# choderalab/pymbar

Hardware: AMD Instinct MI355X
Metric: mbar_adaptive_iterations_per_sec (higher is better)
Workload: dtype f64

## Files before the change

include/mbar_hip.h:

```cpp
#ifndef MBAR_HIP_H
#define MBAR_HIP_H

#include <stdint.h>

#ifdef __cplusplus
extern "C" {
#endif

typedef struct mbar_ctx mbar_ctx;

#define MBAR_OK 0
#define MBAR_ERR_ARG (-1)
#define MBAR_ERR_HIP (-2)
#define MBAR_ERR_NODEVICE (-3)
#define MBAR_ERR_STATE (-4)
#define MBAR_ERR_COMM (-5)
#define MBAR_ERR_NUMERIC (-6)

#define MBAR_EVAL_GRAM 1u
#define MBAR_EVAL_USE_OFFSET 2u

#define MBAR_TIMER_LSE 0
#define MBAR_TIMER_GRAM 1
#define MBAR_TIMER_REDUCE 2
// ... 10 lines not shown

int mbar_ctx_create(mbar_ctx** out, int device, int64_t K, int64_t N_local);
void mbar_ctx_destroy(mbar_ctx* ctx);
int mbar_ctx_synchronize(mbar_ctx* ctx);
int mbar_cache_trim(void);
int mbar_host_digest(const void* data, int64_t nbytes, int threads, uint64_t* out2);
int mbar_host_newton_direction(const double* H, const double* g, int m, int threads, double* x);
int mbar_device_synchronize(int device);
int mbar_ctx_set_option(mbar_ctx* ctx, const char* key, int64_t value);

int mbar_ctx_upload_u(mbar_ctx* ctx, const double* u_host, int64_t ld_host, int64_t col0_host,
                      int64_t ncols, int64_t col0_dev);
int mbar_ctx_download_u(mbar_ctx* ctx, double* out, int64_t ld_out);
int mbar_ctx_upload_rows(mbar_ctx* ctx, int64_t row0, int64_t nrows, const double* rows_host, int64_t ld_host);
int mbar_ctx_copy_rows(mbar_ctx* dst, int64_t dst_row0, mbar_ctx* src, int64_t src_row0, int64_t nrows);
int mbar_ctx_row_sub(mbar_ctx* ctx, int64_t row, const double* v_host);
int mbar_ctx_rows_sub(mbar_ctx* ctx, int64_t dst_row0, int64_t src_row0, int64_t nrows, const double* v_host);
int mbar_ctx_rows_rsub(mbar_ctx* ctx, int64_t dst_row0, int64_t src_row0, int64_t nrows);
int mbar_ctx_rows_logshift(mbar_ctx* ctx, int64_t row0, int64_t nrows, double* shift_out);
int mbar_ctx_vec_logshift(mbar_ctx* ctx, const double* A, double* shift_out);
int mbar_ctx_fill_masked_rows(mbar_ctx* ctx, int64_t row0, int64_t nrows, const double* v_host, const int32_t* label_host);
int mbar_ctx_generate_harmonic(mbar_ctx* ctx, uint64_t seed, const double* O_k, const double* K_k,
                               const int64_t* N_k_global, int64_t n_global0);
int mbar_ctx_set_Nk(mbar_ctx* ctx, const double* N_k);

int mbar_ctx_set_sample_weights(mbar_ctx* ctx, const double* c_n);

int mbar_ctx_draw_bootstrap_weights(mbar_ctx* ctx, uint64_t seed, int64_t replicate, const int64_t* cumN, int64_t K_states,
                                    const int64_t* order, int64_t n_global0);
int mbar_ctx_set_bootstrap_layout(mbar_ctx* ctx, const int64_t* cumN, int64_t K_states, const int64_t* order);
int mbar_bootstrap_draws(uint64_t seed, int64_t replicate, const int64_t* cumN, int64_t K_states, const int64_t* order,
                         int64_t* rints_out);

int mbar_ctx_weights_from_vec(mbar_ctx* ctx, double power);

int mbar_comm_unique_id(void* id128);
int mbar_ctx_comm_init(mbar_ctx* ctx, const void* id128, int rank, int nranks);
typedef int (*mbar_allreduce_fn)(double* buf, int64_t count, int op, void* user);
int mbar_ctx_set_host_allreduce(mbar_ctx* ctx, mbar_allreduce_fn fn, void* user, int rank, int nranks);
int mbar_ctx_comm_destroy(mbar_ctx* ctx);

typedef struct mbar_loopback mbar_loopback;
int mbar_loopback_create(mbar_loopback** out, int nranks);
void mbar_loopback_destroy(mbar_loopback* group);
int mbar_ctx_set_loopback(mbar_ctx* ctx, mbar_loopback* group, int rank);

int mbar_eval(mbar_ctx* ctx, const double* f, int nf, unsigned flags, double* psum,
              double* sumlogden, double* gram);
int mbar_ctx_set_objective_offset(mbar_ctx* ctx, const double* f0);
int mbar_lognum(mbar_ctx* ctx, const double* f, double* lognum);
int mbar_logden(mbar_ctx* ctx, const double* f, double* out_n);
int mbar_logw(mbar_ctx* ctx, const double* f, double* out_kn, int64_t ld_out);
int mbar_w(mbar_ctx* ctx, const double* f, double* out_kn, int64_t ld_out);
int mbar_gram_w(mbar_ctx* ctx, const double* f, double* gramW, double* wsum);

int mbar_ctx_create_ext(mbar_ctx** out, mbar_ctx* base, int64_t K_rows);
int mbar_ctx_rows_sub_from(mbar_ctx* dst, int64_t dst_row0, mbar_ctx* src, int64_t src_row0, int64_t nrows, const double* v_host);
int mbar_ctx_rows_rsub_from(mbar_ctx* dst, int64_t dst_row0, mbar_ctx* src, int64_t src_row0, int64_t nrows);
int mbar_ctx_rows_obs_from(mbar_ctx* dst, int64_t dst_row0, mbar_ctx* base, int64_t state_row0, int64_t obs_row0, int64_t nrows,
                           double* shift_out, const double* min_in, double* min_out);
int mbar_lognum_ext(mbar_ctx* ext, mbar_ctx* base, const double* f_base, double* lognum_ext);
int mbar_gram_w_ext(mbar_ctx* ext, mbar_ctx* base, const double* f_base, const double* f_ext, const double* gram_base, double* gramW,
                    double* wsum);

typedef struct mbar_solve_result {
    int64_t iterations;
    int64_t nr_iter;
    int64_t sci_iter;
    int32_t success;
    int32_t gram_sweeps;
    double max_delta;
    double gnorm;
    double wall_ms;
    int32_t warm_starts;
    int32_t builds;
    int32_t light_sweeps;
    int32_t fused_unit;
} mbar_solve_result;

int mbar_solve_adaptive(mbar_ctx* ctx, double* f_inout, double tol, int64_t maxiter,
                        int64_t min_sc_iter, double gamma, int check_convergence,
                        double* history, int64_t history_rows, mbar_solve_result* result);
int mbar_ctx_last_solve_psum(mbar_ctx* ctx, double* psum);
int mbar_solve_sci(mbar_ctx* ctx, double* f_inout, double tol, int64_t maxiter, int check_convergence,
                   mbar_solve_result* result);

int mbar_ctx_timing(mbar_ctx* ctx, int which, double* total_ms, int64_t* launches);
int mbar_ctx_timing_reset(mbar_ctx* ctx);
int mbar_mfma_f64_peak(mbar_ctx* ctx, double* tflops);

typedef struct mbar_kde mbar_kde;
#define MBAR_KDE_GAUSSIAN 0
#define MBAR_KDE_TOPHAT 1
#define MBAR_KDE_EPANECHNIKOV 2
#define MBAR_KDE_EXPONENTIAL 3
#define MBAR_KDE_LINEAR 4
#define MBAR_KDE_COSINE 5
int mbar_kde_create(mbar_kde** out, int device, int kernel, int d, int64_t N, const double* x, double bandwidth);
void mbar_kde_destroy(mbar_kde* kde);
int mbar_kde_set_weights(mbar_kde* kde, int64_t C, const double* v);
int mbar_kde_eval(mbar_kde* kde, int64_t M, const double* q, double* out);
int mbar_kde_log_norm(int kernel, int d, double bandwidth, double* out);

typedef struct mbar_acf mbar_acf;
int mbar_acf_create(mbar_acf** out, int device, int64_t T, const double* a, const double* b, int64_t K, const int64_t* seg,
                    double shift_a, double shift_b);
void mbar_acf_destroy(mbar_acf* acf);
int mbar_acf_suffix_g(mbar_acf* acf, int64_t nskip, int fast, int64_t mintime, int fft, double* g, int64_t* stop, int32_t* status);
int mbar_acf_multiple_g(mbar_acf* acf, int fast, int64_t mintime, double* g, int64_t* stop, int32_t* status, int64_t ct_cap,
                        double* ct);
int mbar_acf_schedule_length(int fast, int64_t tmax, int64_t* out);
int mbar_acf_lag_sums(mbar_acf* acf, int64_t nlags, const int64_t* lags, int64_t norig, const int64_t* origins, int segments,
                      double* xab, double* xba);

#define MBAR_BAR_CHUNK 4096
typedef struct mbar_bar_state {
    double DeltaF, DeltaF_old, DeltaF_initial, UpperB, LowerB, FUpperB, FLowerB, FNew, relative_change, relative_tolerance;
    double req[2];
    double moments[4];
    int64_t method, iterated, maximum_iterations, iteration, phase, status, nreq, nzero, want_moments, moments_pending;
} mbar_bar_state;
typedef struct mbar_bar mbar_bar;
int mbar_bar_create(mbar_bar** out, int device, int64_t P, const int64_t* n_f, const double* w_f, const int64_t* n_r,
                    const double* w_r);
void mbar_bar_destroy(mbar_bar* bar);
int mbar_bar_zero(mbar_bar* bar, const double* deltaf, double* out);
int mbar_bar_solve(mbar_bar* bar, mbar_bar_state* states, int64_t* passes);
int mbar_bar_moments(mbar_bar* bar, double* out);
int mbar_bar_step_host(mbar_bar_state* state, const double* F);

typedef struct mbar_bspline mbar_bspline;
int mbar_bspline_create(mbar_bspline** out, int device, int64_t N, const double* x);
void mbar_bspline_destroy(mbar_bspline* bs);
int mbar_bspline_set_groups(mbar_bspline* bs, int G, const int* g);
int mbar_bspline_set_weights(mbar_bspline* bs, int64_t C, const double* v);
int mbar_bspline_moments(mbar_bspline* bs, int k, int nbasis, const double* t, double* out);
int mbar_bspline_kernel_ms(mbar_bspline* bs, double* ms);

#define MBAR_BATCH_MAX_K 64
#define MBAR_BATCH_CHUNK 256
typedef struct mbar_batch_state {
    double f[MBAR_BATCH_MAX_K];
    double req[2][MBAR_BATCH_MAX_K];
    double lognum[MBAR_BATCH_MAX_K];
    double psum[MBAR_BATCH_MAX_K];
    double Nk[MBAR_BATCH_MAX_K];
    double x[MBAR_BATCH_MAX_K];
    double tol, gamma, max_delta, max_diff, gnorm_sci, gnorm_nr;
    int64_t K, maxiter, min_sc_iter, iterations, nr_iter, sci_iter, choices;
    int64_t phase, status, success, nreq, gram_req, gram_w, newton_bad;
} mbar_batch_state;
typedef struct mbar_batch mbar_batch;
int mbar_batch_create(mbar_batch** out, int device, int64_t P, const int64_t* K, const int64_t* N, const double* const* u);
void mbar_batch_destroy(mbar_batch* b);
int mbar_batch_solve(mbar_batch* b, mbar_batch_state* states, int64_t* passes);
int mbar_batch_gram_w(mbar_batch* b, const double* f, const int32_t* mask, double* gram, double* wsum);
int mbar_batch_step_host(mbar_batch_state* state, const double* lognum, const double* gram);

int mbar_batch_set_replicas(mbar_batch* b, int64_t R, const int64_t* base, const int64_t* Nk);
int mbar_batch_replica_set_weights(mbar_batch* b, int64_t slot, const double* c_n);
int mbar_batch_replicas_draw(mbar_batch* b, int64_t first, int64_t count, const uint64_t* seed, const int64_t* replicate);
int mbar_batch_replicas_solve(mbar_batch* b, mbar_batch_state* states, int64_t* passes);
int mbar_batch_replicas_gram_w(mbar_batch* b, const double* f, const int32_t* mask, double* gram, double* wsum);

#define MBAR_BATCH_MAX_AUG 128
int mbar_batch_set_ext(mbar_batch* b, const int64_t* R, const double* const* e);
// ... 10 lines not shown
```

pymbar_amd/_lib.py:

```python
import ctypes as C
import os

HERE = os.path.dirname(os.path.abspath(__file__))
LIB_PATH = os.environ.get("MBAR_HIP_LIBRARY") or os.path.join(HERE, "csrc", "libmbar_hip.so")

MBAR_OK = 0
EVAL_GRAM = 1
EVAL_USE_OFFSET = 2
TIMER_LSE, TIMER_GRAM, TIMER_REDUCE, TIMER_OTHER, TIMER_FUSED, TIMER_NEWTON, TIMER_COMM = 0, 1, 2, 3, 4, 5, 6


class BackendUnavailable(RuntimeError):
    """libmbar_hip.so is missing / not loadable, or there is no gfx950 device."""


class MbarHipError(RuntimeError):

    def __init__(self, code, message):
        super().__init__(f"libmbar_hip error {code}: {message}")
        self.code = code


class BarState(C.Structure):
    _fields_ = [(n, C.c_double) for n in ("DeltaF", "DeltaF_old", "DeltaF_initial", "UpperB", "LowerB", "FUpperB", "FLowerB", "FNew",
# ... 13 lines not shown
    _fields_ = [(n, C.c_double * MBAR_BATCH_MAX_K) for n in ("f",)] + [("req", (C.c_double * MBAR_BATCH_MAX_K) * 2)] + [
        (n, C.c_double * MBAR_BATCH_MAX_K) for n in ("lognum", "psum", "Nk", "x")] + [
        (n, C.c_double) for n in ("tol", "gamma", "max_delta", "max_diff", "gnorm_sci", "gnorm_nr")] + [
        (n, C.c_int64) for n in ("K", "maxiter", "min_sc_iter", "iterations", "nr_iter", "sci_iter", "choices", "phase", "status",
                                 "success", "nreq", "gram_req", "gram_w", "newton_bad")]


class SolveResult(C.Structure):
    _fields_ = [
        ("iterations", C.c_int64),
        ("nr_iter", C.c_int64),
        ("sci_iter", C.c_int64),
        ("success", C.c_int32),
        ("gram_sweeps", C.c_int32),
        ("max_delta", C.c_double),
        ("gnorm", C.c_double),
        ("wall_ms", C.c_double),
        ("warm_starts", C.c_int32),
        ("builds", C.c_int32),
        ("light_sweeps", C.c_int32),
        ("fused_unit", C.c_int32),
    ]


ALLREDUCE_FN = C.CFUNCTYPE(C.c_int, C.POINTER(C.c_double), C.c_int64, C.c_int, C.c_void_p)

_dp = C.POINTER(C.c_double)
_ip = C.POINTER(C.c_int64)
_ctx = C.c_void_p

SIGNATURES = {
    "mbar_version": (C.c_int, []),
    "mbar_last_error": (C.c_char_p, [_ctx]),
    "mbar_device_count": (C.c_int, [C.POINTER(C.c_int)]),
    "mbar_device_info": (C.c_int, [C.c_int, C.c_char_p, C.c_int, C.POINTER(C.c_int), _ip]),
    "mbar_ctx_create": (C.c_int, [C.POINTER(_ctx), C.c_int, C.c_int64, C.c_int64]),
    "mbar_ctx_destroy": (None, [_ctx]),
    "mbar_ctx_synchronize": (C.c_int, [_ctx]),
    "mbar_device_synchronize": (C.c_int, [C.c_int]),
    "mbar_cache_trim": (C.c_int, []),
    "mbar_host_digest": (C.c_int, [C.c_void_p, C.c_int64, C.c_int, C.POINTER(C.c_uint64)]),
    "mbar_host_newton_direction": (C.c_int, [_dp, _dp, C.c_int, C.c_int, _dp]),
    "mbar_ctx_set_option": (C.c_int, [_ctx, C.c_char_p, C.c_int64]),
    "mbar_ctx_upload_u": (C.c_int, [_ctx, _dp, C.c_int64, C.c_int64, C.c_int64, C.c_int64]),
    "mbar_ctx_download_u": (C.c_int, [_ctx, _dp, C.c_int64]),
    "mbar_ctx_upload_rows": (C.c_int, [_ctx, C.c_int64, C.c_int64, _dp, C.c_int64]),
    "mbar_ctx_copy_rows": (C.c_int, [_ctx, C.c_int64, _ctx, C.c_int64, C.c_int64]),
    "mbar_ctx_row_sub": (C.c_int, [_ctx, C.c_int64, _dp]),
    "mbar_ctx_rows_sub": (C.c_int, [_ctx, C.c_int64, C.c_int64, C.c_int64, _dp]),
    "mbar_ctx_rows_rsub": (C.c_int, [_ctx, C.c_int64, C.c_int64, C.c_int64]),
    "mbar_ctx_rows_logshift": (C.c_int, [_ctx, C.c_int64, C.c_int64, _dp]),
    "mbar_ctx_vec_logshift": (C.c_int, [_ctx, _dp, _dp]),
    "mbar_ctx_fill_masked_rows": (C.c_int, [_ctx, C.c_int64, C.c_int64, _dp, C.POINTER(C.c_int32)]),
    "mbar_ctx_generate_harmonic": (C.c_int, [_ctx, C.c_uint64, _dp, _dp, _ip, C.c_int64]),
    "mbar_ctx_set_Nk": (C.c_int, [_ctx, _dp]),
    "mbar_ctx_set_sample_weights": (C.c_int, [_ctx, _dp]),
    "mbar_ctx_weights_from_vec": (C.c_int, [_ctx, C.c_double]),
    "mbar_ctx_draw_bootstrap_weights": (C.c_int, [_ctx, C.c_uint64, C.c_int64, _ip, C.c_int64, _ip, C.c_int64]),
    "mbar_ctx_set_bootstrap_layout": (C.c_int, [_ctx, _ip, C.c_int64, _ip]),
    "mbar_bootstrap_draws": (C.c_int, [C.c_uint64, C.c_int64, _ip, C.c_int64, _ip, _ip]),
    "mbar_comm_unique_id": (C.c_int, [C.c_void_p]),
    "mbar_ctx_comm_init": (C.c_int, [_ctx, C.c_void_p, C.c_int, C.c_int]),
    "mbar_ctx_set_host_allreduce": (C.c_int, [_ctx, ALLREDUCE_FN, C.c_void_p, C.c_int, C.c_int]),
    "mbar_ctx_comm_destroy": (C.c_int, [_ctx]),
    "mbar_loopback_create": (C.c_int, [C.POINTER(C.c_void_p), C.c_int]),
    "mbar_loopback_destroy": (None, [C.c_void_p]),
    "mbar_ctx_set_loopback": (C.c_int, [_ctx, C.c_void_p, C.c_int]),
    "mbar_eval": (C.c_int, [_ctx, _dp, C.c_int, C.c_uint, _dp, _dp, _dp]),
    "mbar_ctx_set_objective_offset": (C.c_int, [_ctx, _dp]),
    "mbar_lognum": (C.c_int, [_ctx, _dp, _dp]),
    "mbar_logden": (C.c_int, [_ctx, _dp, _dp]),
    "mbar_logw": (C.c_int, [_ctx, _dp, _dp, C.c_int64]),
    "mbar_w": (C.c_int, [_ctx, _dp, _dp, C.c_int64]),
    "mbar_gram_w": (C.c_int, [_ctx, _dp, _dp, _dp]),
    "mbar_ctx_create_ext": (C.c_int, [C.POINTER(_ctx), _ctx, C.c_int64]),
    "mbar_ctx_rows_sub_from": (C.c_int, [_ctx, C.c_int64, _ctx, C.c_int64, C.c_int64, _dp]),
    "mbar_ctx_rows_rsub_from": (C.c_int, [_ctx, C.c_int64, _ctx, C.c_int64, C.c_int64]),
    "mbar_ctx_rows_obs_from": (C.c_int, [_ctx, C.c_int64, _ctx, C.c_int64, C.c_int64, C.c_int64, _dp, _dp, _dp]),
    "mbar_lognum_ext": (C.c_int, [_ctx, _ctx, _dp, _dp]),
    "mbar_gram_w_ext": (C.c_int, [_ctx, _ctx, _dp, _dp, _dp, _dp, _dp]),
    "mbar_solve_adaptive": (C.c_int, [_ctx, _dp, C.c_double, C.c_int64, C.c_int64, C.c_double, C.c_int,
                                      _dp, C.c_int64, C.POINTER(SolveResult)]),
    "mbar_ctx_last_solve_psum": (C.c_int, [_ctx, _dp]),
    "mbar_solve_sci": (C.c_int, [_ctx, _dp, C.c_double, C.c_int64, C.c_int, C.POINTER(SolveResult)]),
    "mbar_ctx_timing": (C.c_int, [_ctx, C.c_int, _dp, _ip]),
    "mbar_ctx_timing_reset": (C.c_int, [_ctx]),
    "mbar_mfma_f64_peak": (C.c_int, [_ctx, _dp]),
    "mbar_kde_create": (C.c_int, [C.POINTER(C.c_void_p), C.c_int, C.c_int, C.c_int, C.c_int64, _dp, C.c_double]),
    "mbar_kde_destroy": (None, [C.c_void_p]),
    "mbar_kde_set_weights": (C.c_int, [C.c_void_p, C.c_int64, _dp]),
    "mbar_kde_eval": (C.c_int, [C.c_void_p, C.c_int64, _dp, _dp]),
    "mbar_kde_log_norm": (C.c_int, [C.c_int, C.c_int, C.c_double, _dp]),
    "mbar_acf_create": (C.c_int, [C.POINTER(C.c_void_p), C.c_int, C.c_int64, _dp, _dp, C.c_int64, _ip, C.c_double, C.c_double]),
    "mbar_acf_destroy": (None, [C.c_void_p]),
    "mbar_acf_suffix_g": (C.c_int, [C.c_void_p, C.c_int64, C.c_int, C.c_int64, C.c_int, _dp, _ip, C.POINTER(C.c_int32)]),
    "mbar_acf_multiple_g": (C.c_int, [C.c_void_p, C.c_int, C.c_int64, _dp, _ip, C.POINTER(C.c_int32), C.c_int64, _dp]),
    "mbar_acf_schedule_length": (C.c_int, [C.c_int, C.c_int64, _ip]),
    "mbar_acf_lag_sums": (C.c_int, [C.c_void_p, C.c_int64, _ip, C.c_int64, _ip, C.c_int, _dp, _dp]),
    "mbar_bar_create": (C.c_int, [C.POINTER(C.c_void_p), C.c_int, C.c_int64, _ip, _dp, _ip, _dp]),
    "mbar_bar_destroy": (None, [C.c_void_p]),
    "mbar_bar_zero": (C.c_int, [C.c_void_p, _dp, _dp]),
    "mbar_bar_solve": (C.c_int, [C.c_void_p, C.POINTER(BarState), _ip]),
    "mbar_bar_moments": (C.c_int, [C.c_void_p, _dp]),
    "mbar_bar_step_host": (C.c_int, [C.POINTER(BarState), _dp]),
    "mbar_bspline_create": (C.c_int, [C.POINTER(C.c_void_p), C.c_int, C.c_int64, _dp]),
    "mbar_bspline_destroy": (None, [C.c_void_p]),
    "mbar_bspline_set_groups": (C.c_int, [C.c_void_p, C.c_int, C.POINTER(C.c_int32)]),
    "mbar_bspline_set_weights": (C.c_int, [C.c_void_p, C.c_int64, _dp]),
    "mbar_bspline_moments": (C.c_int, [C.c_void_p, C.c_int, C.c_int, _dp, _dp]),
    "mbar_bspline_kernel_ms": (C.c_int, [C.c_void_p, _dp]),
    "mbar_batch_create": (C.c_int, [C.POINTER(C.c_void_p), C.c_int, C.c_int64, _ip, _ip, C.POINTER(_dp)]),
    "mbar_batch_destroy": (None, [C.c_void_p]),
    "mbar_batch_solve": (C.c_int, [C.c_void_p, C.POINTER(BatchState), _ip]),
    "mbar_batch_gram_w": (C.c_int, [C.c_void_p, _dp, C.POINTER(C.c_int32), _dp, _dp]),
    "mbar_batch_step_host": (C.c_int, [C.POINTER(BatchState), _dp, _dp]),
    "mbar_batch_set_replicas": (C.c_int, [C.c_void_p, C.c_int64, _ip, _ip]),
    "mbar_batch_replica_set_weights": (C.c_int, [C.c_void_p, C.c_int64, _dp]),
    "mbar_batch_replicas_draw": (C.c_int, [C.c_void_p, C.c_int64, C.c_int64, C.POINTER(C.c_uint64), _ip]),
    "mbar_batch_replicas_solve": (C.c_int, [C.c_void_p, C.POINTER(BatchState), _ip]),
    "mbar_batch_replicas_gram_w": (C.c_int, [C.c_void_p, _dp, C.POINTER(C.c_int32), _dp, _dp]),
    "mbar_batch_set_ext": (C.c_int, [C.c_void_p, _ip, C.POINTER(_dp)]),
    "mbar_batch_ext_lognum": (C.c_int, [C.c_void_p, _dp, C.POINTER(C.c_int32), _dp]),
    "mbar_batch_ext_gram": (C.c_int, [C.c_void_p, _dp, _dp, C.POINTER(C.c_int32), C.c_int64, _dp, _dp]),
}

_lib = None


def load_library():
    global _lib
    if _lib is not None:
        return _lib
    if not os.path.exists(LIB_PATH):
        raise BackendUnavailable(
            f"{LIB_PATH} not found: build it with `python -c 'import __graft_entry__ as g; g.build()'` "
            "(hipcc --offload-arch=gfx950).  pymbar_amd has no CPU fallback.")
    try:
        lib = C.CDLL(LIB_PATH)
    except OSError as exc:
        raise BackendUnavailable(f"cannot load {LIB_PATH}: {exc}") from exc
    for name, (restype, argtypes) in SIGNATURES.items():
        fn = getattr(lib, name)
        fn.restype = restype
        fn.argtypes = argtypes
    _lib = lib
    return lib


def last_error(ctx=None):
    msg = load_library().mbar_last_error(ctx)
    return msg.decode("utf-8", "replace") if msg else ""


def check(code, ctx=None):
    if code != MBAR_OK:
        raise MbarHipError(code, last_error(ctx))


def host_digest(a, threads=0):
    out = (C.c_uint64 * 2)()
    check(load_library().mbar_host_digest(C.c_void_p(a.ctypes.data), a.nbytes, int(threads), out))
    return bytes(out)


def bootstrap_draws(seed, replicate, cumN, order=None):
    import numpy as np
# ... 77 lines not shown
```

pymbar_amd/csrc/mbar_capi.cpp:

```cpp
#include "mbar_ctx.h"

using namespace mbar;
using namespace mbar::host;

namespace mbar {
namespace host {

int fail(mbar_ctx* c, int code, const std::string& msg) {
    if (c) c->error = msg;
    g_last_error = msg;
    return code;
}
hipEvent_t get_event(mbar_ctx* c) {
    if (!c->pool.empty()) {
        hipEvent_t e = c->pool.back();
        c->pool.pop_back();
        return e;
    }
    hipEvent_t e;
    if (hipEventCreate(&e) != hipSuccess) return nullptr;
    return e;
}
void flush_timers(mbar_ctx* c) {
    for (auto& tp : c->pending) {
// ... 26 lines not shown
    }
    return MBAR_OK;
}
int ensure(mbar_ctx* c, double** p, size_t* have, size_t want) {
    if (*have >= want) return MBAR_OK;
    {
        int rc = drop_graphs(c);
        if (rc) return rc;
    }
    if (*p) HIPCHK(c, cache_free(*p));
    *p = nullptr;
    *have = 0;
    HIPCHK(c, cache_malloc((void**)p, want * sizeof(double)));
    *have = want;
    return MBAR_OK;
}
int refresh_poison(mbar_ctx* c) {
    if (c->u_checked) return MBAR_OK;
    c->ld0_valid = false;
    int* dflags = reinterpret_cast<int*>(d_delta(c) + 255);
    HIPCHK(c, hipMemsetAsync(dflags, 0, sizeof(int), c->stream));
    HIPCHK(c, launch_check_u(c->stream, c->u, c->ld, c->N, c->K, dflags));
    int h = 0;
    HIPCHK(c, hipMemcpyAsync(&h, dflags, sizeof(int), hipMemcpyDeviceToHost, c->stream));
    HIPCHK(c, hipStreamSynchronize(c->stream));
    if (c->nranks > 1) {
        double v[2] = {(h & 3) ? 1.0 : 0.0, (h & 4) ? 1.0 : 0.0};
        int rc = allreduce_host(c, v, 2, 1);
        if (rc) return rc;
        h = (v[0] > 0.0 ? 1 : 0) | (v[1] > 0.0 ? 4 : 0);
    }
    c->u_poison = (h & 3) != 0;
    c->u_posinf = (h & 4) != 0;
    c->u_checked = true;
    return MBAR_OK;
}
bool f_is_finite(const mbar_ctx* c, const double* f, int nf) {
    for (int i = 0; i < nf; ++i)
        for (int64_t k = 0; k < c->K; ++k)
            if (c->Nk[k] > 0.0 && !std::isfinite(f[(size_t)i * c->K + k])) return false;
    return true;
}

bool wide_pitch(const mbar_ctx* c) { return (uint64_t)c->ld * 56u + 128u >= (1ull << 32); }
int lse_variant_for(const mbar_ctx* c) {
    if (wide_pitch(c)) return 0;
    int v = 0;
    if (c->opt_small && c->Kp <= 32 && c->ld % 64 == 0) v |= 0x10;
    if (c->opt_wide && c->Kp > 128) v |= 0x20;
    return v;
}
bool use_fast(const mbar_ctx* c) { return c->K <= MAX_FAST_K && !c->opt_force_generic; }

void build_aden(const mbar_ctx* c, const double* f, double* out, int64_t rows) {
    const double ninf = -std::numeric_limits<double>::infinity();
    for (int64_t k = 0; k < rows; ++k) out[k] = (k < c->K && c->Nk[k] > 0.0) ? f[k] + c->lnNk[k] : ninf;
}

bool split_sweep_ok(const mbar_ctx* c, int64_t rows) {
    return !use_fast(c) && !c->opt_force_generic && !wide_pitch(c) && rows <= 1024 && rows % 64 == 0 && c->opt_wide;
}

int run_lse(mbar_ctx* c, int nf, int64_t rows, double* ld0, double* ld1, bool use_offset) {
    const double* dn = use_offset ? c->dn : nullptr;
    if (use_fast(c)) {
        const int nb = (int)(rows / 16);
        const int64_t ntiles = (c->N + TS - 1) / TS;
        LaunchGeom g = lse_geometry(nb, nf, c->num_cu, ntiles, c->opt_grid, lse_variant_for(c));
        g.balanced = c->opt_small_balanced ? 1 : 0;
        const size_t rec = (size_t)nf * rows;
        int rc = ensure(c, &c->part, &c->part_doubles, (size_t)g.nwaves * (rec + nf));
        if (rc) return rc;
        rc = ensure(c, &c->scratch, &c->scratch_doubles, ((size_t)g.nwaves / 32 + 1) * (rec + nf));
        if (rc) return rc;
        double* psum_part = c->part;
        double* obj_part = c->part + (size_t)g.nwaves * rec;
        {
            ScopedTimer t(c, MBAR_TIMER_LSE);
            HIPCHK(c, launch_lse(c->stream, nb, nf, g, c->u, c->ld, c->N, d_aden(c), c->cw, ld0,
                                 ld1, dn, psum_part, obj_part));
        }
        {
            ScopedTimer t(c, MBAR_TIMER_REDUCE);
            HIPCHK(c, launch_reduce2(c->stream, psum_part, (int64_t)rec, obj_part, nf, g.nwaves, c->scratch, c->red, c->red + rec));
        }
        return MBAR_OK;
    }
    if (split_sweep_ok(c, rows)) {
        int blocks = 0;
        int rc = ensure(c, &c->part, &c->part_doubles, (size_t)c->num_cu * nf * (rows + 1));
        if (rc) return rc;
        rc = ensure(c, &c->scratch, &c->scratch_doubles, (size_t)(c->num_cu / 32 + 2) * nf * (rows + 1));
        if (rc) return rc;
        double* obj_part = c->part + (size_t)c->num_cu * nf * rows;
        {
            ScopedTimer t(c, MBAR_TIMER_LSE);
            HIPCHK(c, launch_lse_split(c->stream, c->num_cu, nf, c->u, c->ld, c->N, rows, d_aden(c), c->cw, ld0, nf == 2 ? ld1 : nullptr, dn,
                                       c->part, obj_part, &blocks));
        }
        ScopedTimer t(c, MBAR_TIMER_REDUCE);
        HIPCHK(c, launch_reduce(c->stream, c->part, blocks, (int64_t)nf * rows, c->scratch, c->red));
        HIPCHK(c, launch_reduce(c->stream, obj_part, blocks, nf, c->scratch, c->red + (size_t)nf * rows));
        return MBAR_OK;
    }
    for (int i = 0; i < nf; ++i) {
        int blocks = 0, cblocks = 0;
        int rc = ensure(c, &c->part, &c->part_doubles, (size_t)c->num_cu * 8 + (size_t)512 * c->K);
        if (rc) return rc;
        rc = ensure(c, &c->scratch, &c->scratch_doubles, (size_t)64 * (c->K + 8));
        if (rc) return rc;
        double* ldst = i == 0 ? ld0 : ld1;
        if (!ldst) ldst = c->logden[i];
        {
            ScopedTimer t(c, MBAR_TIMER_LSE);
            HIPCHK(c, launch_lse_generic(c->stream, c->num_cu, c->u, c->ld, c->N, c->K, d_aden(c) + i * rows, c->cw,
                                         ldst, dn, c->part, &blocks));
        }
        {
            ScopedTimer t(c, MBAR_TIMER_REDUCE);
            HIPCHK(c, launch_reduce(c->stream, c->part, blocks, 1, c->scratch, c->red + nf * rows + i));
        }
        {
            ScopedTimer t(c, MBAR_TIMER_LSE);
            HIPCHK(c, launch_colsum_generic(c->stream, c->num_cu, c->u, c->ld, c->N, c->K, d_aden(c) + i * rows, c->cw,
                                            ldst, c->part, &cblocks));
        }
        {
            ScopedTimer t(c, MBAR_TIMER_REDUCE);
            HIPCHK(c, hipMemsetAsync(c->red + i * rows, 0, rows * sizeof(double), c->stream));
            HIPCHK(c, launch_reduce(c->stream, c->part, cblocks, c->K, c->scratch, c->red + i * rows));
        }
    }
    return MBAR_OK;
}

GramPlan gram_plan(int64_t Kp, bool quad) {
    GramPlan p;
    if (Kp <= 128 || quad) {
        int nb = (int)(Kp / 16);
        p.items.push_back({true, 0, 0, nb, nb, nb * (nb + 1) / 2, 0});
        p.total_blocks = (size_t)nb * (nb + 1) / 2;
        return p;
    }
    struct Panel { int64_t r0; int nb; };
    std::vector<Panel> panels;
    for (int64_t r = 0; r < Kp;) {
        const int nb = Kp - r >= 128 ? 8 : (int)((Kp - r) / 16);
        panels.push_back({r, nb});
        r += 16 * nb;
    }
    size_t off = 0;
    for (const auto& a : panels) {
        const int nblk = a.nb * (a.nb + 1) / 2;
        p.items.push_back({true, a.r0, a.r0, a.nb, a.nb, nblk, off});
        off += nblk;
    }
    for (size_t ia = 0; ia < panels.size(); ++ia)
        for (size_t ib = ia + 1; ib < panels.size(); ++ib) {
            const Panel &a = panels[ia], &b = panels[ib];
            if (b.nb == 8) {
                for (int h = 0; h < 2; ++h) {
                    p.items.push_back({false, a.r0 + 64 * h, b.r0, 4, 8, 32, off});
                    off += 32;
                }
            } else if (b.nb == 4) {
                p.items.push_back({false, b.r0, a.r0, 4, 8, 32, off});
                off += 32;
// ... 422 lines not shown
void mbar_ctx_destroy(mbar_ctx* c) {
    if (!c) return;
    (void)hipSetDevice(c->device);
    if (c->stream) (void)hipStreamSynchronize(c->stream);
    flush_timers(c);
    for (auto e : c->pool) (void)hipEventDestroy(e);
    if (c->comm && g_rccl.CommDestroy) g_rccl.CommDestroy(c->comm);
    if (c->u_alloc) (void)cache_free(c->u_alloc);
    else if (c->u) (void)cache_free(c->u);
    if (c->logden[0]) (void)cache_free(c->logden[0]);
    if (c->ad) (void)cache_free(c->ad);
    if (c->P) (void)cache_free(c->P);
    if (c->pm_vec) (void)cache_free(c->pm_vec);
    if (c->pm_ld0) (void)cache_free(c->pm_ld0);
    if (c->part_g) (void)cache_free(c->part_g);
    if (c->cwsq) (void)cache_free(c->cwsq);
    if (c->chol) (void)cache_free(c->chol);
    if (c->ad_ints) (void)cache_free(c->ad_ints);
    if (c->h_ctl) (void)cache_host_free(c->h_ctl);
    if (c->ad_graph) (void)hipGraphExecDestroy(c->ad_graph);
    if (c->dn) (void)cache_free(c->dn);
    if (c->cw) (void)cache_free(c->cw);
    if (c->lden_eff) (void)cache_free(c->lden_eff);
    if (c->small) (void)cache_free(c->small);
    if (c->part) (void)cache_free(c->part);
    if (c->scratch) (void)cache_free(c->scratch);
    if (c->red) (void)cache_free(c->red);
    if (c->hred) (void)cache_host_free(c->hred);
    if (c->lognum_part) (void)cache_free(c->lognum_part);
    if (c->f_hist) (void)cache_free(c->f_hist);
    if (c->hstage) (void)cache_host_free(c->hstage);
    if (c->vec_tmp) (void)cache_free(c->vec_tmp);
    if (c->boot_idx) (void)cache_free(c->boot_idx);
    if (c->stamps) (void)hipFree(c->stamps);
    if (c->sci_graph) (void)hipGraphExecDestroy(c->sci_graph);
    if (c->stream) {
        std::lock_guard<std::mutex> lock(g_dev_mu);
        auto& pool = g_stream_pool[c->device];
        if (pool.size() < 8)
            pool.push_back(c->stream);
        else
            (void)hipStreamDestroy(c->stream);
    }
    delete c;
    if (g_live_contexts.fetch_sub(1) == 1) g_mem.trim_to(g_mem.idle_limit());
}

int mbar_ctx_synchronize(mbar_ctx* c) {
    if (!c) return fail(nullptr, MBAR_ERR_ARG, "ctx is NULL");
    HIPCHK(c, hipSetDevice(c->device));
    return sync_stream(c);
}

int mbar_device_synchronize(int device) {
    hipError_t e = hipSetDevice(device);
    if (e == hipSuccess) e = hipDeviceSynchronize();
    if (e != hipSuccess) return fail(nullptr, MBAR_ERR_HIP, std::string("hipDeviceSynchronize: ") + hipGetErrorString(e));
    return MBAR_OK;
}

int mbar_ctx_set_option(mbar_ctx* c, const char* key, int64_t value) {
    if (!c || !key) return fail(c, MBAR_ERR_ARG, "NULL argument");
    const std::string k(key);
    if (k == "grid_blocks") c->opt_grid = value;
    else if (k == "force_generic") c->opt_force_generic = value;
    else if (k == "small_k_kernel") c->opt_small = value;
    else if (k == "wide_k_kernel") c->opt_wide = value;
    else if (k == "check_finite") c->opt_check_finite = value;
    else if (k == "timing") c->opt_timing = value;
    else if (k == "graph") c->opt_graph = value;
    else if (k == "sci_batch") c->opt_sci_batch = value < 1 ? 1 : (value > 256 ? 256 : value);
    else if (k == "device_loop") c->opt_device_loop = value;
    else if (k == "pmode") c->opt_pmode = value;
    else if (k == "fused") c->opt_fused = value;
    else if (k == "gram_quad") c->opt_quad = value;
    else if (k == "device_loop_wide") c->opt_device_loop_wide = value;
    else if (k == "pcache") c->opt_pcache = value;
    else if (k == "merge_select") c->opt_merge_select = value;
    else if (k == "light_last") c->opt_light_last = value;
    else if (k == "fused_general") {
        c->opt_fused_general = value ? 1 : 0;
        (void)drop_graphs(c);
    }
    else if (k == "debug_download_p") c->opt_debug_download_p = value;
    else if (k == "direct_results") c->opt_direct_results = value;
    else if (k == "sci_merged") c->opt_sci_merged = value;
    else if (k == "host_pmode") c->opt_host_pmode = value;
    else if (k == "rect_waves") c->opt_rect_waves = value == 8 ? 8 : 4;
    else if (k == "newton_ldlt") {
        c->opt_newton_ldlt = value ? 1 : 0;
        (void)drop_graphs(c);
    }
    else if (k == "sci_pingpong") {
        c->opt_sci_pingpong = value;
        (void)drop_graphs(c);
    }
    else if (k == "small_balanced") {
        c->opt_small_balanced = value;
        (void)drop_graphs(c);
    }
    else if (k == "wide_pmode") c->opt_wide_pmode = value;
    else if (k == "quad_trim") {
        c->opt_quad_trim = value;
        c->P_valid = false;
    }
    else if (k == "adapt_batch") c->opt_adapt_batch = value < 1 ? 1 : (value > 64 ? 64 : value);
    else return fail(c, MBAR_ERR_ARG, "unknown option: " + k);
    return MBAR_OK;
}

int mbar_ctx_upload_u(mbar_ctx* c, const double* u_host, int64_t ld_host, int64_t col0_host, int64_t ncols,
                      int64_t col0_dev) {
    if (!c || !u_host) return fail(c, MBAR_ERR_ARG, "NULL argument");
    if (ncols < 0 || col0_dev < 0 || col0_dev + ncols > c->N || col0_host < 0 || col0_host + ncols > ld_host)
        return fail(c, MBAR_ERR_ARG, "column range out of bounds");
    if (ncols == 0) return MBAR_OK;
    HIPCHK(c, hipSetDevice(c->device));
    HIPCHK(c, hipMemcpy2DAsync(c->u + col0_dev, (size_t)c->ld * sizeof(double), u_host + col0_host,
                               (size_t)ld_host * sizeof(double), (size_t)ncols * sizeof(double), (size_t)c->K,
                               hipMemcpyHostToDevice, c->stream));
    c->u_checked = false;
    c->P_valid = false;
    c->last_psum.clear();
    return sync_stream(c);
}

int mbar_ctx_upload_rows(mbar_ctx* c, int64_t row0, int64_t nrows, const double* rows_host, int64_t ld_host) {
    if (!c || !rows_host) return fail(c, MBAR_ERR_ARG, "NULL argument");
    if (row0 < 0 || nrows < 0 || row0 + nrows > c->K || ld_host < c->N) return fail(c, MBAR_ERR_ARG, "row range out of bounds");
    if (nrows == 0) return MBAR_OK;
    HIPCHK(c, hipSetDevice(c->device));
    HIPCHK(c, hipMemcpy2DAsync(c->u + row0 * c->ld, (size_t)c->ld * sizeof(double), rows_host,
                               (size_t)ld_host * sizeof(double), (size_t)c->N * sizeof(double), (size_t)nrows,
                               hipMemcpyHostToDevice, c->stream));
    c->u_checked = false;
    c->P_valid = false;
    c->last_psum.clear();
    return sync_stream(c);
}

int mbar_ctx_copy_rows(mbar_ctx* dst, int64_t dst_row0, mbar_ctx* src, int64_t src_row0, int64_t nrows) {
    if (!dst || !src) return fail(dst, MBAR_ERR_ARG, "NULL argument");
    if (dst->device != src->device || dst->N != src->N) return fail(dst, MBAR_ERR_ARG, "contexts must share device and N_local");
    if (nrows < 0 || dst_row0 < 0 || src_row0 < 0 || dst_row0 + nrows > dst->K || src_row0 + nrows > src->K)
        return fail(dst, MBAR_ERR_ARG, "row range out of bounds");
    if (nrows == 0) return MBAR_OK;
    HIPCHK(dst, hipSetDevice(dst->device));
    HIPCHK(dst, hipStreamSynchronize(src->stream));
    if (dst->ld == src->ld)
        HIPCHK(dst, hipMemcpyAsync(dst->u + dst_row0 * dst->ld, src->u + src_row0 * src->ld, (size_t)nrows * dst->ld * sizeof(double),
                                   hipMemcpyDeviceToDevice, dst->stream));
    else
        HIPCHK(dst, hipMemcpy2DAsync(dst->u + dst_row0 * dst->ld, (size_t)dst->ld * sizeof(double), src->u + src_row0 * src->ld,
                                     (size_t)src->ld * sizeof(double), (size_t)dst->N * sizeof(double), (size_t)nrows,
                                     hipMemcpyDeviceToDevice, dst->stream));
    dst->u_checked = false;
    dst->P_valid = false;
    dst->last_psum.clear();
    return sync_stream(dst);
}

int mbar_ctx_row_sub(mbar_ctx* c, int64_t row, const double* v_host) {
    if (!c) return fail(c, MBAR_ERR_ARG, "NULL argument");
    if (row < 0 || row >= c->K) return fail(c, MBAR_ERR_ARG, "row out of range");
    if (!v_host && !c->vec_tmp) return fail(c, MBAR_ERR_STATE, "mbar_ctx_row_sub: no vector has been uploaded yet");
    HIPCHK(c, hipSetDevice(c->device));
// ... 837 lines not shown
```

pymbar_amd/csrc/mbar_ctx.h:

```cpp
#pragma once
#include "../../include/mbar_hip.h"
#include "mbar_internal.h"

#include <dlfcn.h>
#include <sched.h>
#include <unistd.h>
#include <rccl/rccl.h>

#include <algorithm>
#include <chrono>
#include <condition_variable>
#include <cmath>
#include <cstdio>
#include <cstdlib>
#include <cstring>
#include <functional>
#include <limits>
#include <map>
#include <memory>
#include <mutex>
#include <string>
#include <atomic>
#include <thread>
#include <unordered_map>
// ... 184 lines not shown


}
}
using mbar::host::TimerPair;

struct mbar_loopback {
    int nranks = 0, device = -1;
    std::mutex mu;
    std::condition_variable cv;
    int arrived = 0;
    uint64_t gen = 0;
    bool broken = false;
    std::vector<const double*> src;
    std::vector<int64_t> cnt;
    std::vector<int> op;
    std::vector<hipEvent_t> ready, done;
    std::vector<double*> tmp;
    std::vector<size_t> tmp_doubles;
    std::vector<int> attached;
};

struct mbar_ctx {
    int device = 0;
    int num_cu = 256;
    hipStream_t stream = nullptr;
    int64_t K = 0, Kp = 0, N = 0, ld = 0;
    bool have_Nk = false;
    bool u_checked = false, u_poison = false;
    std::vector<double> ld0_f;
    bool ld0_valid = false;
    bool u_posinf = true;
    std::vector<double> Nk, lnNk;
    std::vector<int> sampled;
    double* u = nullptr;
    double* u_alloc = nullptr;
    mbar_ctx* ext_base = nullptr;
    double* logden[3] = {nullptr, nullptr, nullptr};
    double* dn = nullptr;
    double* cw = nullptr;
    double* lden_eff = nullptr;
    bool weighted = false;
    double* small = nullptr;
    double* part = nullptr;
    size_t part_doubles = 0;
    double* scratch = nullptr;
    size_t scratch_doubles = 0;
    double* red = nullptr;
    size_t red_doubles = 0;
    double* hred = nullptr;
    double* hstage = nullptr;
    double* lognum_part = nullptr;
    size_t lognum_part_doubles = 0;
    double* f_hist = nullptr;
    double* vec_tmp = nullptr;
    int64_t* boot_idx = nullptr;
    size_t boot_idx_words = 0;
    uint64_t boot_layout_digest[2] = {0, 0};
    int64_t boot_states = 0, boot_total = 0;
    bool boot_has_order = false;
    bool vec_holds_logshift = false;
    hipGraphExec_t sci_graph = nullptr;
    int64_t sci_graph_batch = 0, sci_graph_sig = 0;
    double sci_graph_tol = 0.0;
    double* ad = nullptr;
    int64_t ad_hist_cap = 0;
    int* ad_ints = nullptr;
    int* h_ctl = nullptr;
    hipGraphExec_t ad_graph = nullptr;
    int64_t ad_graph_batch = 0, ad_graph_sig = 0;
    double* P = nullptr;
    bool P_failed = false;
    double* pm_vec = nullptr;
    double* pm_ld0 = nullptr;
    double* part_g = nullptr;
    size_t part_g_doubles = 0;
    double* cwsq = nullptr;
    double* chol = nullptr;
    long long* stamps = nullptr;
    std::vector<double> last_psum;
    bool P_valid = false;
    std::vector<double> P_a0;
    int64_t opt_grid = 0, opt_force_generic = 0, opt_check_finite = 1, opt_sci_batch = 16, opt_timing = 0, opt_graph = 1, opt_small = 1, opt_wide = 1;
    int64_t opt_device_loop = 1, opt_adapt_batch = 8, opt_pmode = 1, opt_fused = 1, opt_quad = 1, opt_device_loop_wide = 1, opt_pcache = 1, opt_merge_select = 1, opt_sci_merged = 1, opt_wide_pmode = 1, opt_quad_trim = 1, opt_light_last = 1, opt_direct_results = 1, opt_debug_download_p = 0, opt_fused_general = 0;
    int64_t opt_small_balanced = 1, opt_sci_pingpong = 1, opt_host_pmode = 2, opt_rect_waves = 8, opt_newton_ldlt = 1;

    ncclComm_t comm = nullptr;
    mbar_loopback* loop = nullptr;
    mbar_allreduce_fn host_reduce = nullptr;
    void* host_reduce_user = nullptr;
    int rank = 0, nranks = 1;
    std::vector<TimerPair> pending;
    std::vector<hipEvent_t> pool;
    double t_ms[MBAR_TIMER_COUNT] = {0, 0, 0, 0, 0};
    int64_t t_n[MBAR_TIMER_COUNT] = {0, 0, 0, 0, 0};
    std::string error;
};


namespace mbar {
namespace host {

int fail(mbar_ctx* c, int code, const std::string& msg);
#define HIPCHK(ctx, expr)                                                                        \
    do {                                                                                         \
        hipError_t _e = (expr);                                                                  \
        if (_e != hipSuccess)                                                                    \
            return fail(ctx, MBAR_ERR_HIP, std::string(#expr) + ": " + hipGetErrorString(_e));   \
    } while (0)
inline int bad_arg(const std::string& msg) { return fail(nullptr, MBAR_ERR_ARG, msg); }


template <typename T>
struct DevBuf {
    T* p = nullptr;
    size_t n = 0;
    DevBuf() = default;
    DevBuf(const DevBuf&) = delete;
    DevBuf& operator=(const DevBuf&) = delete;
    DevBuf(DevBuf&& o) noexcept : p(o.p), n(o.n) {
        o.p = nullptr;
        o.n = 0;
    }
    DevBuf& operator=(DevBuf&& o) noexcept {
        std::swap(p, o.p);
        std::swap(n, o.n);
        return *this;
    }
    ~DevBuf() { reset(); }
    operator T*() const { return p; }
    void reset() {
        if (p) (void)cache_free(p);
        p = nullptr;
        n = 0;
    }
    auto grow(size_t want) -> hipError_t {
        if (n >= want) return hipSuccess;
        if (p) {
            hipError_t e = cache_free(p);
            if (e != hipSuccess) return e;
        }
        p = nullptr;
        n = 0;
        hipError_t e = cache_malloc((void**)&p, want * sizeof(T));
        if (e == hipSuccess) n = want;
        return e;
    }
    auto upload(const T* src, size_t count) -> hipError_t {
        hipError_t e = grow(count);
        return e != hipSuccess ? e : hipMemcpy(p, src, count * sizeof(T), hipMemcpyHostToDevice);
    }
};

int open_device(int device, DevInfo* out);

struct Handle {
    int device = 0;
    hipStream_t stream = nullptr;
    Handle() { g_live_contexts.fetch_add(1); }
    Handle(const Handle&) = delete;
    Handle& operator=(const Handle&) = delete;
    ~Handle() {
        if (stream) (void)hipStreamDestroy(stream);
        if (g_live_contexts.fetch_sub(1) == 1) g_mem.trim_to(g_mem.idle_limit());
    }
};

// ... 199 lines not shown
```

pymbar_amd/csrc/mbar_device.h:

```cpp
#ifndef MBAR_DEVICE_H
#define MBAR_DEVICE_H
#include "mbar_internal.h"

#include <hip/hip_ext.h>
#include <math.h>
#include <type_traits>

namespace mbar {

typedef double v4d __attribute__((ext_vector_type(4)));

template <int CTRL>
__device__ __forceinline__ double dpp_move(double x) {
    int lo = __double2loint(x), hi = __double2hiint(x);
    lo = __builtin_amdgcn_update_dpp(0, lo, CTRL, 0xF, 0xF, true);
    hi = __builtin_amdgcn_update_dpp(0, hi, CTRL, 0xF, 0xF, true);
    return __hiloint2double(hi, lo);
}
__device__ __forceinline__ double row16_max(double x) {
    x = fmax(x, dpp_move<0xB1>(x));
    x = fmax(x, dpp_move<0x4E>(x));
    x = fmax(x, dpp_move<0x141>(x));
    x = fmax(x, dpp_move<0x140>(x));
    return x;
// ... 434 lines not shown
}
template <bool DMA>
__device__ __forceinline__ void stage_piece(const double* __restrict__ ubase , uint32_t voff,
                                            char* dst , int lane) {
    uint64_t ub = reinterpret_cast<uint64_t>(ubase);
    asm("" : "+s"(ub));
    asm("" : "+v"(voff));
    const char* src = reinterpret_cast<const char*>(ub) + voff;
    if constexpr (DMA) {
        __builtin_amdgcn_global_load_lds((const __attribute__((address_space(1))) void*)src,
                                         (__attribute__((address_space(3))) void*)dst, 16, 0, MBAR_DMA_AUX);
    } else {
        *reinterpret_cast<double2*>(dst + lane * 16) = *reinterpret_cast<const double2*>(src);
    }
}
template <int ROWS, bool DMA, int J0, int JSTEP, typename RowMap, typename SO>
__device__ __forceinline__ void stage_tile(const double* __restrict__ u, int64_t ld, int64_t n0, char* dst, int lane,
                                           const SO& so, RowMap rowmap) {
    constexpr int NDMA = ROWS / 8;
#pragma unroll
    for (int j = J0; j < NDMA; j += JSTEP)
        stage_piece<DMA>(u + rowmap(8 * j) * ld + rowmap.cols(j, n0), so.off[j & 1], dst + j * 1024, lane);
}

template <bool DMA>
__device__ __forceinline__ void stage_vec16(const double* __restrict__ v, int64_t n0, char* dst, int lane) {
    if (lane < 8) stage_piece<DMA>(v + n0, (uint32_t)(lane * 16), dst, lane);
}

__device__ __forceinline__ void settle(double& x) { asm volatile("" : "+v"(x)); }

__device__ __forceinline__ double load_untracked(const double* p) {
    double v;
    asm volatile("global_load_dwordx2 %0, %1, off" : "=v"(v) : "v"(p) : "memory");
    return v;
}
template <int N>
__device__ __forceinline__ void wait_vm_for(double& a, double& b, double& c, double& d, double& e, double (&r)[16]) {
    asm volatile("s_waitcnt vmcnt(%21)"
                 : "+v"(a), "+v"(b), "+v"(c), "+v"(d), "+v"(e), "+v"(r[0]), "+v"(r[1]), "+v"(r[2]), "+v"(r[3]), "+v"(r[4]), "+v"(r[5]),
                   "+v"(r[6]), "+v"(r[7]), "+v"(r[8]), "+v"(r[9]), "+v"(r[10]), "+v"(r[11]), "+v"(r[12]), "+v"(r[13]), "+v"(r[14]), "+v"(r[15])
                 : "n"(N)
                 : "memory");
}
__device__ __forceinline__ void lds_barrier() { asm volatile("s_waitcnt lgkmcnt(0)\n\ts_barrier" ::: "memory"); }
template <int N>
__device__ __forceinline__ void wait_vm() {
    asm volatile("s_waitcnt vmcnt(%0)" ::"n"(N) : "memory");
}

struct RowIdentity {
    int64_t row0;
    uint32_t live = 0xffffffffu;
    __device__ __forceinline__ int64_t operator()(int tr) const { return row0 + tr; }
    __device__ __forceinline__ int64_t cols(int j, int64_t n0) const { return ((live >> j) & 1u) ? n0 : 0; }
};
struct RowTwoPanels {
    int64_t row_i0, row_j0;
    int split;
    uint32_t live = 0xffffffffu;
    __device__ __forceinline__ int64_t operator()(int tr) const {
        return tr < split ? row_i0 + tr : row_j0 + (tr - split);
    }
    __device__ __forceinline__ int64_t cols(int j, int64_t n0) const { return ((live >> j) & 1u) ? n0 : 0; }
};
template <int NB>
__device__ __forceinline__ uint32_t live_piece_mask(const double (&a)[NB], double dead) {
    uint32_t m = 0;
#pragma unroll
    for (int I = 0; I < NB; ++I) {
        const unsigned long long b = __ballot(a[I] != dead);
        m |= ((b & 0xffull) ? 1u : 0u) << (2 * I);
        m |= ((b & 0xff00ull) ? 1u : 0u) << (2 * I + 1);
    }
    return m;
}

constexpr int lse_waves(int nb) { return nb <= 2 ? 16 : (nb <= 4 ? 8 : (nb <= 8 ? 4 : 2)); }
constexpr int TSS = 64;
constexpr int GRAM_AGPR_BLOCKS = 31;
constexpr double GRAM_NEG_HUGE = -2.9e303, LOGDEN_HUGE = 1e300;
constexpr int FUSED_PSUM1_FROM_GRAM_NB = 8;

static inline int blocks_per_cu_for(size_t lds_bytes) {
    int b = (int)((160 * 1024) / lds_bytes);
    if (b < 1) b = 1;
    if (b > 4) b = 4;
    return b;
}

static inline bool stage_offsets_wide(int64_t ld) { return (uint64_t)ld * 56u + 128u >= (1ull << 32); }

hipError_t launch_fused_quad(hipStream_t s, int nbt, const LaunchGeom& g, const double* P, int64_t ld, int64_t N, const double* cmul,
                             const double* cw, const double* wsq, double* rinv0, double* gp, double* pp, const LoopCtl& lc);

}
#endif
```

pymbar_amd/csrc/mbar_internal.h:

```cpp
#pragma once
#include <hip/hip_runtime.h>
#include <stdint.h>

#include "../../include/mbar_hip.h"

namespace mbar {

constexpr int TS = 16;
constexpr int GROUPS = 4;
constexpr int MAX_FAST_K = 256;
constexpr int PANEL = 64;

inline int64_t padded_K(int64_t K) {
    if (K <= 128) return (K + 15) / 16 * 16;
    return (K + PANEL - 1) / PANEL * PANEL;
}
inline int lse_nb_for(int64_t Kp) {
    static const int nbs[] = {1, 2, 3, 4, 5, 6, 7, 8, 12, 16};
    int need = (int)(Kp / 16);
    for (int nb : nbs) if (nb >= need) return nb;
    return 0;
}

#if defined(__HIPCC__)
#define MBAR_HD __host__ __device__
#else
#define MBAR_HD
#endif
MBAR_HD inline uint64_t bootstrap_mix64(uint64_t z) {
    z = (z ^ (z >> 30)) * 0xBF58476D1CE4E5B9ull;
    z = (z ^ (z >> 27)) * 0x94D049BB133111EBull;
    return z ^ (z >> 31);
}
MBAR_HD inline int64_t bootstrap_draw(uint64_t seed, uint64_t replicate, uint64_t slot, uint64_t n) {
    const uint64_t key = bootstrap_mix64(seed + 0x9E3779B97F4A7C15ull * (replicate + 1));
    const uint64_t z = bootstrap_mix64(bootstrap_mix64(key ^ (slot * 0xD1342543DE82EF95ull)) + slot);
    return (int64_t)(((unsigned __int128)z * (unsigned __int128)n) >> 64);
}

enum : int {
    CTL_SLOT = 0,
    CTL_DONE = 1,
    CTL_ITER = 2,
    CTL_SCI = 3,
    CTL_NR = 4,
    CTL_REASON = 5,
    CTL_NEEDGRAM = 6,
    CTL_GRAMSWEEPS = 7,
    CTL_SPEC = 8,
    CTL_LIGHT = 9,
    CTL_LIGHTS = 10,
    CTL_WORDS = 12
};
struct LoopCtl {
    const int* ctl = nullptr;
    int64_t slot_stride = 0;
    hipEvent_t ev_start = nullptr, ev_stop = nullptr;
    bool unclamped = false;
    bool pmode = false;
    bool cond_needgram = false;
    bool light_only = false;
};

struct LaunchGeom {
    int blocks;
    int waves;
    int nwaves;
    int psum_records;
    int variant;
    size_t lds_bytes;
    int live_blocks = 0;
    int balanced = 0;
};

LaunchGeom lse_geometry(int nb, int nf, int num_cu, int64_t ntiles, int64_t grid_override, int variant);
hipError_t launch_lse(hipStream_t s, int nb, int nf, const LaunchGeom& g,
                      const double* u, int64_t ld, int64_t N, const double* aden ,
                      const double* cw, double* logden0, double* logden1, const double* dn,
                      double* psum_part, double* obj_part, const LoopCtl& lc = LoopCtl());

LaunchGeom gram_geometry(int tile_rows, bool diag, int num_cu, int64_t ntiles, int64_t grid_override);
hipError_t launch_row_sub(hipStream_t s, double* row, const double* v, int64_t n);
hipError_t launch_rows_sub(hipStream_t s, double* dst, const double* src, int64_t ld, int64_t nrows, const double* v, int64_t n);
hipError_t launch_rows_obs(hipStream_t s, double* dst, const double* obs, const double* state, int64_t ld, int64_t nrows, int64_t n,
                           double* part, double* shift_out, bool have_min = false);
hipError_t launch_rows_rsub(hipStream_t s, double* dst, const double* src, int64_t ld, int64_t nrows, int64_t n);
hipError_t launch_rows_logshift(hipStream_t s, double* base, int64_t ld, int64_t nrows, int64_t n, double* part, double* shift_out);
hipError_t launch_fill_masked_rows(hipStream_t s, double* rows, int64_t ld, int64_t n, int64_t nrows, const double* v,
                                   const int* label);
hipError_t launch_gram_diag(hipStream_t s, int nb, const LaunchGeom& g, const double* u,
                            int64_t ld, int64_t N, const double* anum ,
                            const double* logden, int64_t row0, double* gram_part, double* psum_part,
                            const LoopCtl& lc = LoopCtl());
hipError_t launch_gram_thin(hipStream_t s, const LaunchGeom& g, const double* u, int64_t ld, int64_t N, const double* ai,
                            const double* aj, const double* logden, int64_t ri, int64_t rj, double* gp);
hipError_t launch_gram_off(hipStream_t s, int nbj , const LaunchGeom& g, const double* u, int64_t ld,
                           int64_t N, const double* anum_i, const double* anum_j, const double* logden,
                           int64_t row_i0, int64_t row_j0, double* gram_part, bool pmode = false);

LaunchGeom gram_quad_geometry(int nbt, int num_cu, int64_t ntiles, int64_t grid_override);
hipError_t launch_gram_rect(hipStream_t s, int nbi, const LaunchGeom& g, const double* P, int64_t ld, int64_t N, int64_t ri, int64_t rj,
                            const double* rinv, double* gram_part);
hipError_t launch_gram_quad(hipStream_t s, int nbt, const LaunchGeom& g, const double* u, int64_t ld, int64_t N,
                            const double* anum, const double* logden, double* gram_part, const LoopCtl& lc = LoopCtl(),
                            double* Pout = nullptr);
hipError_t launch_gram_quad_split(hipStream_t s, int nbt, const LaunchGeom& g, const double* u, int64_t ld, int64_t N, const double* anum,
                                  const double* logden, double* gram_part, int64_t split_rows, int64_t row_j0);

hipError_t launch_lse_split(hipStream_t s, int num_cu, int nf, const double* u, int64_t ld, int64_t N, int64_t rows, const double* aden,
                            const double* cw, double* logden, double* logden1, const double* dn, double* psum_part, double* obj_part,
                            int* blocks_out, const double* ld_anchor = nullptr );
hipError_t launch_lse_generic(hipStream_t s, int num_cu, const double* u, int64_t ld, int64_t N, int64_t K,
                              const double* aden, const double* cw, double* logden, const double* dn,
                              double* obj_part , int* blocks_out);
hipError_t launch_colsum_generic(hipStream_t s, int num_cu, const double* u, int64_t ld, int64_t N, int64_t K,
                                 const double* anum, const double* cw, const double* logden,
                                 double* psum_part , int* blocks_out);
hipError_t launch_shift_logden(hipStream_t s, const double* logden, const double* cw, double alpha, int64_t N,
                               double* out, const LoopCtl& lc = LoopCtl());

hipError_t launch_reduce(hipStream_t s, const double* part, int64_t nparts, int64_t count,
                         double* scratch, double* out);
hipError_t launch_lognum(hipStream_t s, const double* u, int64_t ld, int64_t N, int64_t K,
                         const double* anum, const double* logden,
                         double* pmax , double* psum , int64_t nchunks);
int64_t lognum_chunks(int64_t N, int64_t K);
hipError_t launch_lognum_merge(hipStream_t s, const double* pmax, const double* psum, int64_t K,
                               int64_t nchunks, double* out_max , double* out_sum );
hipError_t launch_logw(hipStream_t s, const double* u, int64_t ld, int64_t N, int64_t K,
                       const double* f, const double* logden, double* out, int64_t ld_out, bool exponentiate = false);
hipError_t launch_check_u(hipStream_t s, const double* u, int64_t ld, int64_t N, int64_t K, int* flags);
hipError_t launch_generate_harmonic(hipStream_t s, double* u, int64_t ld, int64_t N, int64_t K,
                                    uint64_t seed, const double* O_k, const double* K_k,
                                    const int64_t* cumN , int64_t n_global0);
hipError_t launch_sci_update(hipStream_t s, const double* part, int64_t nparts, int64_t rows, const double* Nk,
                             const double* lnNk, int64_t K, int64_t Kp, int first_state, double tol, double* f,
                             double* aden, double* f_hist, double* delta_out);
struct SciLoopArgs {
    const double* Nk;
    const double* lnNk;
    int K;
    int first;
    double tol;
    double* state;
    double* rec;
    int64_t nrec;
    double* f_hist;
    double* delta_out;
    int parity;
    uint32_t live;
    int balanced;
    int pingpong;
    long long* stamps;
};
hipError_t launch_sci_small(hipStream_t s, int nb, const LaunchGeom& g, const double* u, int64_t ld, int64_t N, const double* cw,
                            const SciLoopArgs& q);
hipError_t launch_bootstrap_counts(hipStream_t s, uint64_t seed, int64_t replicate, const int64_t* cum, int64_t K, int64_t total,
                                   const int64_t* order, int64_t n0, int64_t N, double* cw);
hipError_t launch_weights_from_log(hipStream_t s, const double* v, double p, int64_t n, double* cw, double* cwsq, int* overflow);
hipError_t launch_reduce_level1(hipStream_t s, const double* part, int64_t nparts, int64_t count, double* out,
                                int64_t* nchunks);
hipError_t launch_mfma_peak(hipStream_t s, int blocks, int iters, double* sink);
hipError_t launch_reduce2(hipStream_t s, const double* partA, int64_t countA, const double* partB, int64_t countB,
                          int64_t nparts, double* scratch, double* outA, double* outB);

struct LoopSrc {
    const double* p[8];
    int n;
};
hipError_t launch_loop_reduce(hipStream_t s, const LoopSrc& src, int64_t count, int op , double* out);

struct AdaptArgs {
    const double* gram_red;
    const double* lse_red;
    double* f;
    double* psum;
    double* cand;
    double* ratio;
    double* aden;
    double* anum;
    const double* Nk;
    const double* lnNk;
    const int* sampled;
    int m, K, Kp;
    int* ctl;
    const double* prm;
    double* state;
    double* hist;
    int64_t hist_cap;
    int pmode;
    const double* a0;
    double* ccur;
    int fused;
    double* cgram;
    int light_ok;
    long long* stamps;
    int newton_ldlt;
};
LaunchGeom psweep_geometry(int nb, int num_cu, int64_t ntiles, int64_t grid_override);
hipError_t launch_psweep(hipStream_t s, int nb, int nf, const LaunchGeom& g, const double* P, int64_t ld, int64_t N,
                         const double* cmul, const double* cw, double* rinv0, double* rinv1, double* psum_part,
                         const LoopCtl& lc = LoopCtl());
LaunchGeom fused_geometry(int nb, int num_cu, int64_t ntiles, int64_t grid_override, bool unit = false);
hipError_t launch_fused(hipStream_t s, int nb, const LaunchGeom& g, const double* P, int64_t ld, int64_t N, const double* cmul,
                        const double* cw, const double* wsq, bool unit, double* rinv_base, double* gram_part, double* psum_part,
                        const LoopCtl& lc);
LaunchGeom build_sweep_geometry(int nb, int num_cu, int64_t ntiles, int64_t grid_override);
hipError_t launch_build_sweep(hipStream_t s, int nb, const LaunchGeom& g, const double* u, int64_t ld, int64_t N,
                              const double* aden, const double* cw, double* P, double* rinv_slot, double* psum_part);
LaunchGeom build_gram_geometry(int nb, int num_cu, int64_t ntiles, int64_t grid_override);
hipError_t launch_build_gram(hipStream_t s, int nb, const LaunchGeom& g, const double* u, int64_t ld, int64_t N,
                             const double* aden, const double* wsq, bool general, double* P, double* rinv_slot, double* gram_part);

hipError_t launch_make_p(hipStream_t s, int num_cu, const double* u, int64_t ld, int64_t N, int64_t rows, const double* aden,
                         const double* logden, double* P);
hipError_t launch_fill(hipStream_t s, double* v, double value, int64_t n);
hipError_t launch_zero(hipStream_t s, void* p, size_t bytes);
hipError_t launch_sqrt_vec(hipStream_t s, double* dst, const double* src, int64_t n);
hipError_t launch_rinv_from_logden(hipStream_t s, const double* ld0, const double* ldv, const double* cw, bool weighted, int64_t N,
                                   double* out);
hipError_t launch_rinv_weighted(hipStream_t s, const double* rinv, const double* cw, int64_t N, double* out,
                                const LoopCtl& lc = LoopCtl());
hipError_t launch_newton(hipStream_t s, const AdaptArgs& a);
constexpr size_t NEWTON_CHOL_WORK = (size_t)256 * 256 + 8;
hipError_t launch_newton_chol(hipStream_t s, const AdaptArgs& a, double* work);
hipError_t launch_select(hipStream_t s, const AdaptArgs& a);
hipError_t launch_select_newton(hipStream_t s, const AdaptArgs& a);
hipError_t launch_ctl_resume(hipStream_t s, int* ctl);


enum : int { KDE_GAUSSIAN = 0, KDE_TOPHAT = 1, KDE_EPANECHNIKOV = 2, KDE_EXPONENTIAL = 3, KDE_LINEAR = 4, KDE_COSINE = 5 };
constexpr int KDE_MAX_D = 8;
constexpr int KDE_TILE = 64;
constexpr int KDE_MAX_CB = 32;
struct KdeLaunch {
    int kernel, d, cb;
    const double* X;
    int64_t ldx;
    const double* V;
    const double* Q;
    int64_t ldq, M;
    double coef;
    double h, inv_h, inv_h2;
    int64_t qblocks, nchunks, chunk;
    double* part;
};
size_t kde_lds_bytes(int kernel, int d, int cb);
hipError_t launch_kde(hipStream_t s, const KdeLaunch& a);
hipError_t launch_kde_combine(hipStream_t s, const KdeLaunch& a, int cv, const double* logW, double lognorm, double* out, int* flag);
hipError_t launch_kde_exact(hipStream_t s, const KdeLaunch& a, int64_t N, int64_t npairs, const int64_t* pq, const double* logW,
                            double lognorm, double* out);

constexpr int BSP_MAX_K = 7;
constexpr int BSP_MAX_BASIS = 1024;
constexpr int BSP_MAX_GROUPS = 1024;
constexpr int BSP_MAX_CB = 32;
constexpr int BSP_SLAB_ENTRIES = 768;
struct BsplineLaunch {
    int k, nbasis, cb;
    const double* X;
    const int* G;
    const double* V;
    int64_t N;
    const double* t;
    int64_t nchunks, chunk;
    int cells, tile_cells, ntiles;
    double* part;
};
size_t bspline_lds_bytes(int k, int nbasis, int tile_cells, int cb);
hipError_t launch_bspline(hipStream_t s, const BsplineLaunch& a);
hipError_t launch_bspline_combine(hipStream_t s, const BsplineLaunch& a, double* out);

constexpr int ACF_WG = 256;
constexpr int ACF_R = 8;
constexpr int ACF_TILE = ACF_WG * ACF_R;
constexpr int ACF_MAX_LAGS = 64;
enum : int { ACF_AUTO = 0, ACF_CROSS = 1, ACF_PLAIN = 2 };
enum : int { ACF_RULE_SUFFIX = 0, ACF_RULE_MULTIPLE = 1 };
enum : int { ACF_RUNNING = 0, ACF_STOPPED = 1, ACF_ZERO_VARIANCE = 2, ACF_END = 3 };
struct AcfLaunch {
    int kind, nacc;
    const double2* A;
    const double2* B;
    const int* rem;
    int64_t T, ldx, ntiles;
    int nl;
    int64_t lag[ACF_MAX_LAGS];
    int64_t inc[ACF_MAX_LAGS];
    double den[ACF_MAX_LAGS];
    int64_t kbase;
    int64_t tile_lo, atile_hi;
    double2* tot;
    double2* off;
// ... 394 lines not shown
```

pymbar_amd/csrc/mbar_k_fused.hip:

```cpp
#include "mbar_device.h"

namespace mbar {

template <int NB>
__host__ __device__ constexpr int fused_steps_done(int I) {
    if (I < 0) return 0;
    if (I >= NB - 2) return 2 * NB;
    if (NB < 4) return 2 * (I + 1) < 2 * NB ? 2 * (I + 1) : 2 * NB;
    const int r1 = (NB + 1) / 2 - 1;
    if (I <= r1) return 2 * (I + 1) < NB ? 2 * (I + 1) : NB;
    const int rows = NB - 2 - r1;
    return NB + (NB * (I - r1) + rows - 1) / rows;
}
template <int NB, bool WIDE, bool UNIT>
__global__ void __launch_bounds__(256, 1)
k_fused(const double* __restrict__ P, int64_t ld, int64_t N, int64_t ntiles, const double* __restrict__ cmul,
        const double* __restrict__ cw, const double* __restrict__ wsq, double* __restrict__ rinv0,
        double* __restrict__ rinv1, double* __restrict__ gram_part, double* __restrict__ psum_part,
        const int* __restrict__ ctl, int64_t slot_stride) {
    extern __shared__ __attribute__((aligned(16))) char smem[];
    if (ctl) {
        if (ctl[CTL_DONE] != 0 || ctl[CTL_LIGHT] != 0) return;
        const int s = ctl[CTL_SLOT];
        rinv1 = rinv0 + (int64_t)((s + 2) % 3) * slot_stride;
        rinv0 = rinv0 + (int64_t)((s + 1) % 3) * slot_stride;
    }
    constexpr int ROWS = NB * 16;
    constexpr int NDMA = ROWS / 8 + (UNIT ? 0 : 1);
    constexpr int U_BYTES = ROWS * TS * 8;
    constexpr int TILE_BYTES = U_BYTES + (UNIT ? 0 : 1024);
    constexpr int NBLK = NB * (NB + 1) / 2;
    constexpr bool PINNED = NBLK > GRAM_AGPR_BLOCKS;
    constexpr bool ACC1 = NB < FUSED_PSUM1_FROM_GRAM_NB;
    const int lane = threadIdx.x & 63;
    const int wave = __builtin_amdgcn_readfirstlane(threadIdx.x >> 6);
    const int nwv = blockDim.x >> 6;
    const int ks = lane & 15, ns = lane >> 4;
    char* buf = smem + wave * (2 * TILE_BYTES);
    const int64_t gw = (int64_t)blockIdx.x * nwv + wave;
    const int64_t W = (int64_t)gridDim.x * nwv;
    RowIdentity rows{0};
    const StageOffsetsT<WIDE> so = make_stage_offsets<WIDE>(ld, lane);

    double acc[2][NB];
#pragma unroll
    for (int f = 0; f < 2; ++f)
#pragma unroll
        for (int I = 0; I < NB; ++I) acc[f][I] = 0.0;
    {
        double cany[NB];
#pragma unroll
        for (int I = 0; I < NB; ++I) cany[I] = fabs(cmul[16 * I + ks]) + fabs(cmul[ROWS + 16 * I + ks]);
        if constexpr (NB <= 2) rows.live = live_piece_mask<NB>(cany, 0.0);
    }
    constexpr int NSTEP = ROWS / 4;
    double cb[UNIT ? NSTEP : 1];
    if constexpr (UNIT) {
#pragma unroll
        for (int st = 0; st < NSTEP; ++st) {
            const double cv = cmul[(lane & 1) * ROWS + 4 * st + (lane >> 4)];
            cb[st] = (lane & 3) < 2 ? cv : 0.0;
            asm volatile("" : "+v"(cb[st]));
        }
    } else {
        double* ctab = reinterpret_cast<double*>(smem + nwv * (2 * TILE_BYTES));
        for (int e = threadIdx.x; e < NSTEP * 16; e += blockDim.x) ctab[e] = (e & 3) < 2 ? cmul[(e & 3) * ROWS + (e >> 2)] : 0.0;
        __syncthreads();
    }
    int apos[4];
#pragma unroll
    for (int q = 0; q < 4; ++q) apos[q] = ns * (TS * 8) + (((lane & 15) + (ns & 2) + 4 * q) & 15) * 8;
    v4d G[NBLK];
#pragma unroll
    for (int b = 0; b < NBLK; ++b) G[b] = v4d{0.0, 0.0, 0.0, 0.0};

    const int rd_base = ks * (TS * 8);
    int pos[GROUPS];
#pragma unroll
    for (int g = 0; g < GROUPS; ++g) pos[g] = ((4 * g + ns + (ks & 14)) & 15) * 8;
    const int sq = ns + 4 * ((lane >> 2) & 3);
    const int fq = lane & 3;

    const char* wsrc = reinterpret_cast<const char*>(((lane >> 3) & 1) ? wsq : cw) + (lane & 7) * 16;
    auto stage_w = [&](int64_t tile, char* dst) {
        __builtin_amdgcn_global_load_lds((const __attribute__((address_space(1))) void*)(wsrc + tile * (TS * 8)),
                                         (__attribute__((address_space(3))) void*)(dst + U_BYTES), 16, 0, 0);
    };
    auto stage = [&](int64_t tile, char* dst) {
        stage_tile<ROWS, true, 0, 1>(P, ld, tile * TS, dst, lane, so, rows);
        if constexpr (!UNIT) stage_w(tile, dst);
    };
    auto read_group = [&](const char* tb, int g, double (&x)[NB], double& wg, double& swg) {
        if constexpr (!UNIT) {
            wg = *reinterpret_cast<const double*>(tb + U_BYTES + (4 * g + ns) * 8);
            swg = *reinterpret_cast<const double*>(tb + U_BYTES + TS * 8 + (4 * g + ns) * 8);
        }
#pragma unroll
// ... 90 lines not shown
#pragma unroll
                    for (int q = 0; q < B1; ++q) read_step(nbuf, (g - 2) * 2 * NB + q, opa[q], opb[q]);
                }
            };
            if constexpr (!PINNED) {
                request_next();
                request_steps();
            }
            auto mfma = [&](int b, double x, double y) {
                if constexpr (PINNED) {
                    if (b < GRAM_AGPR_BLOCKS)
                        asm volatile("v_mfma_f64_16x16x4_f64 %0, %1, %2, %0" : "+a"(G[b]) : "v"(x), "v"(y));
                    else
                        asm volatile("v_mfma_f64_16x16x4_f64 %0, %1, %2, %0" : "+v"(G[b]) : "v"(x), "v"(y));
                } else {
                    G[b] = __builtin_amdgcn_mfma_f64_16x16x4f64(x, y, G[b], 0, 0, 0);
                }
            };
            if constexpr (PINNED) {
                __builtin_amdgcn_sched_barrier(0);
                asm volatile("s_nop 7");
            }
            constexpr int NM = NBLK;
            int b = 0, nm = 0;
#pragma unroll
            for (int I = 0; I < NB; ++I) {
                if (NB == 1 && g >= 2) {
                    mfma4(sacc[2 * (g & 1)], opa[0], opb[0], true);
                    mfma4(sacc[2 * (g & 1) + 1], opa[1], opb[1], true);
                }
#pragma unroll
                for (int J = I; J < NB; ++J) {
                    mfma(b, p[I], p[J]);
                    if constexpr (PINNED) {
                        if (nm == 0 || nm == 1) {
                            __builtin_amdgcn_sched_barrier(0);
                            if (nm == 0) request_next(); else request_steps();
                            __builtin_amdgcn_sched_barrier(0);
                        }
                    }
                    if (g == GROUPS - 1) {
#pragma unroll
                        for (int j = nm * NDMA / NM; j < (nm + 1) * NDMA / NM; ++j) {
                            if constexpr (PINNED) __builtin_amdgcn_sched_barrier(0);
                            if (j < ROWS / 8)
                                stage_piece<true>(P + rows(8 * j) * ld + rows.cols(j, tstage * TS), so.off[j & 1], cbuf + j * 1024, lane);
                            else if constexpr (!UNIT)
                                stage_w(tstage, cbuf);
                            if constexpr (PINNED) __builtin_amdgcn_sched_barrier(0);
                        }
                    }
                    ++b;
                    ++nm;
                }
                if (g >= 2 && NB > 1 && I < NB - 1) {
#pragma unroll
                    for (int q = fused_steps_done<NB>(I - 1); q < fused_steps_done<NB>(I); ++q)
                        mfma4(sacc[q & 3], opa[q % B1], opb[q % B1], g == 2 && q < 4);
                    if (B1 < 2 * NB && fused_steps_done<NB>(I - 1) < B1 && fused_steps_done<NB>(I) >= B1) {
#pragma unroll
                        for (int q = 0; q < B1; ++q) read_step(nbuf, (g - 2) * 2 * NB + B1 + q, opa[q], opb[q]);
                    }
                }
            }
            if constexpr (PINNED) __builtin_amdgcn_sched_barrier(0);
        }
        if constexpr (PINNED)
            asm volatile("s_nop 7\n\ts_nop 7" : "+v"(sacc[0]), "+v"(sacc[1]), "+v"(sacc[2]), "+v"(sacc[3]));
        rcur = recip_fast(fmax((sacc[0] + sacc[1]) + (sacc[2] + sacc[3]), 1e-300));
        store_rinv(tn, rcur);
        cur ^= 1;
    }
    if constexpr (PINNED) asm volatile("s_nop 15\n\ts_nop 15" ::: "memory");
#pragma unroll
    for (int f = 0; f < 2; ++f) {
#pragma unroll
        for (int I = 0; I < NB; ++I) {
            double v = acc[f][I];
            v += __shfl_xor(v, 16);
            v += __shfl_xor(v, 32);
            if (lane < 16) psum_part[(gw * 2 + f) * ROWS + 16 * I + lane] = v;
        }
    }
    {
        int b = 0;
#pragma unroll
        for (int I = 0; I < NB; ++I)
#pragma unroll
            for (int J = I; J < NB; ++J, ++b) {
#pragma unroll
                for (int r = 0; r < 4; ++r) {
#if defined(MBAR_GRAM_STORE_NT)
                    __builtin_nontemporal_store(G[b][r], &gram_part[((gw * NBLK + b) * 4 + r) * 64 + lane]);
#else
                    gram_part[((gw * NBLK + b) * 4 + r) * 64 + lane] = G[b][r];
#endif
                }
            }
    }
}



LaunchGeom fused_geometry(int nb, int num_cu, int64_t ntiles, int64_t grid_override, bool unit) {
    LaunchGeom g;
    g.waves = 4;
    g.variant = 1;
    if (nb > 8) {
        g.variant = 6;
        g.lds_bytes = (size_t)2 * ((size_t)nb * 16 * TS * 8 + 4 * 1024) + 1024;
        int64_t capq = grid_override > 0 ? grid_override : num_cu;
        int64_t wantq = ntiles < 1 ? 1 : ntiles;
        g.blocks = (int)(wantq < capq ? wantq : capq);
        g.nwaves = g.blocks;
        g.psum_records = g.nwaves;
        return g;
    }
    const size_t tile = (size_t)nb * 16 * TS * 8 + 1024;
    const size_t lds_general = (size_t)4 * 2 * tile + (size_t)nb * 512;
    g.lds_bytes = unit ? (size_t)4 * 2 * (tile - 1024) : lds_general;
    int64_t want = (ntiles + 3) / 4;
    int64_t cap = num_cu;
    if (nb <= 5) {
        static const int occ[6] = {1, 4, 4, 3, 2, 2};
        const int by_lds = blocks_per_cu_for(lds_general);
        cap = (int64_t)num_cu * (by_lds < occ[nb] ? by_lds : occ[nb]);
        int64_t by_work = (ntiles + 127) / 128;
        if (by_work < num_cu) by_work = num_cu;
        if (cap > by_work) cap = by_work;
    }
    if (grid_override > 0) cap = grid_override;
    if (want < 1) want = 1;
    g.blocks = (int)(want < cap ? want : cap);
    g.nwaves = g.blocks * 4;
    g.psum_records = g.nwaves;
    return g;
}
template <int NB>
static hipError_t launch_fused_nb(hipStream_t s, const LaunchGeom& g, const double* P, int64_t ld, int64_t N, const double* cmul,
                                  const double* cw, const double* wsq, bool unit, double* rinv0, double* gp, double* pp, const LoopCtl& lc) {
    auto go = [&](auto kern) -> hipError_t {
        if (g.lds_bytes > 64 * 1024) {
            hipError_t e = hipFuncSetAttribute(reinterpret_cast<const void*>(kern),
                                               hipFuncAttributeMaxDynamicSharedMemorySize, (int)g.lds_bytes);
            if (e != hipSuccess) return e;
        }
        const int64_t ntiles = (N + TS - 1) / TS;
        double* r1 = nullptr;
        if (lc.ev_start && lc.ev_stop)
            hipExtLaunchKernelGGL(kern, dim3(g.blocks), dim3(256), g.lds_bytes, s, lc.ev_start, lc.ev_stop, 0, P, ld, N, ntiles, cmul,
                                  cw, wsq, rinv0, r1, gp, pp, lc.ctl, lc.slot_stride);
        else
            hipLaunchKernelGGL(kern, dim3(g.blocks), dim3(256), g.lds_bytes, s, P, ld, N, ntiles, cmul, cw, wsq, rinv0, r1, gp, pp,
                               lc.ctl, lc.slot_stride);
        return hipGetLastError();
    };
    if (unit) return stage_offsets_wide(ld) ? go(k_fused<NB, true, true>) : go(k_fused<NB, false, true>);
    return stage_offsets_wide(ld) ? go(k_fused<NB, true, false>) : go(k_fused<NB, false, false>);
}
hipError_t launch_fused(hipStream_t s, int nb, const LaunchGeom& g, const double* P, int64_t ld, int64_t N, const double* cmul,
                        const double* cw, const double* wsq, bool unit, double* rinv_base, double* gram_part, double* psum_part,
                        const LoopCtl& lc) {
    if (!lc.ctl) return hipErrorInvalidValue;
    if (nb == 12 || nb == 16) return launch_fused_quad(s, nb, g, P, ld, N, cmul, cw, wsq, rinv_base, gram_part, psum_part, lc);
    switch (nb) {
#define MBAR_CASE(NB_) \
    case NB_: return launch_fused_nb<NB_>(s, g, P, ld, N, cmul, cw, wsq, unit, rinv_base, gram_part, psum_part, lc);
        MBAR_CASE(1) MBAR_CASE(2) MBAR_CASE(3) MBAR_CASE(4) MBAR_CASE(5) MBAR_CASE(6) MBAR_CASE(7) MBAR_CASE(8)
#undef MBAR_CASE
        default: return hipErrorInvalidValue;
    }
}

}
```

pymbar_amd/csrc/mbar_k_pmode.hip:

```cpp
#include "mbar_device.h"

namespace mbar {

__global__ void __launch_bounds__(256)
k_rinv_weighted(const double* __restrict__ rinv, const double* __restrict__ cw, int64_t N, double* __restrict__ out,
                const int* __restrict__ ctl, int64_t slot_stride) {
    if (ctl) {
        if (ctl[CTL_DONE] != 0) return;
        rinv += (int64_t)ctl[CTL_SLOT] * slot_stride;
    }
    for (int64_t n = (int64_t)blockIdx.x * blockDim.x + threadIdx.x; n < N; n += (int64_t)gridDim.x * blockDim.x)
        out[n] = rinv[n] * sqrt(cw[n]);
}

__global__ void __launch_bounds__(256)
k_rinv_from_logden(const double* __restrict__ ld0, const double* __restrict__ ldv, const double* __restrict__ cw, int weighted,
                   int64_t N, double* __restrict__ out) {
    for (int64_t n = (int64_t)blockIdx.x * blockDim.x + threadIdx.x; n < N; n += (int64_t)gridDim.x * blockDim.x) {
        double r = exp(ld0[n] - ldv[n]);
        if (weighted) r *= sqrt(cw[n]);
        out[n] = r;
    }
}
hipError_t launch_rinv_from_logden(hipStream_t s, const double* ld0, const double* ldv, const double* cw, bool weighted, int64_t N,
// ... 54 lines not shown
k_build_sweep(const double* __restrict__ u, int64_t ld, int64_t N, int64_t ntiles, const double* __restrict__ aden,
              const double* __restrict__ cw, double* __restrict__ P, double* __restrict__ rinv_slot,
              double* __restrict__ psum_part) {
    extern __shared__ __attribute__((aligned(16))) char smem[];
    constexpr int ROWS = NB * 16;
    constexpr int NDMA = ROWS / 8;
    constexpr int U_BYTES = ROWS * TS * 8;
    constexpr int TILE_BYTES = U_BYTES + TS * 8;
    const int lane = threadIdx.x & 63;
    const int wave = __builtin_amdgcn_readfirstlane(threadIdx.x >> 6);
    const int nwv = blockDim.x >> 6;
    const int ks = lane & 15, ns = lane >> 4;
    exp_table_init(smem);
    __syncthreads();
    char* buf = smem + EXP_TABLE_BYTES + wave * (2 * TILE_BYTES);
    const int64_t gw = (int64_t)blockIdx.x * nwv + wave;
    const int64_t W = (int64_t)gridDim.x * nwv;
    RowIdentity rows{0};
    const StageOffsetsT<WIDE> so = make_stage_offsets<WIDE>(ld, lane);

    double a[NB], acc[NB];
#pragma unroll
    for (int I = 0; I < NB; ++I) {
        a[I] = aden[16 * I + ks];
        acc[I] = 0.0;
    }
#pragma unroll
    for (int I = 0; I < NB; ++I) settle(a[I]);
    rows.live = live_piece_mask<NB>(a, -INFINITY);
    const int rd_base = ks * (TS * 8);
    int pos[GROUPS];
#pragma unroll
    for (int g = 0; g < GROUPS; ++g) pos[g] = rd_base + ((4 * g + ns + (ks & 14)) & 15) * 8;

    int64_t t = gw;
    int cur = 0;
    if (t < ntiles) {
        stage_tile<ROWS, true, 0, 1>(u, ld, t * TS, buf, lane, so, rows);
        stage_vec16<true>(cw, t * TS, buf + U_BYTES, lane);
    }
    for (; t < ntiles; t += W) {
        char* cbuf = buf + cur * TILE_BYTES;
        const char* wslot = cbuf + U_BYTES;
        const int64_t tn = t + W;
        if (tn < ntiles) {
            char* nbuf = buf + (cur ^ 1) * TILE_BYTES;
            stage_tile<ROWS, true, 0, 1>(u, ld, tn * TS, nbuf, lane, so, rows);
            stage_vec16<true>(cw, tn * TS, nbuf + U_BYTES, lane);
            if (t != gw)
                wait_vm<2 * (NDMA + 1)>();
            else
                wait_vm<NDMA + 1>();
        } else {
            wait_vm<0>();
        }
        double w[GROUPS];
#pragma unroll
        for (int g = 0; g < GROUPS; ++g) w[g] = *reinterpret_cast<const double*>(wslot + (4 * g + ns) * 8);
        build_two_groups<NB>(cbuf, pos[0], pos[1], a, acc, w[0], w[1]);
        build_two_groups<NB>(cbuf, pos[2], pos[3], a, acc, w[2], w[3]);
        __builtin_amdgcn_fence(__ATOMIC_RELEASE, "wavefront");
        __builtin_amdgcn_wave_barrier();
#pragma unroll
        for (int j = 0; j < NDMA; ++j) {
            const double2 v = *reinterpret_cast<const double2*>(cbuf + j * 1024 + lane * 16);
            char* dst = reinterpret_cast<char*>(P + (int64_t)(8 * j) * ld + t * TS) + so.off[j & 1];
            store_p16(dst, v);
        }
        {
            const int64_t n = t * TS + lane;
            if (lane < TS && n < N) rinv_slot[n] = 1.0;
        }
        cur ^= 1;
    }
#pragma unroll
    for (int I = 0; I < NB; ++I) {
        double v = acc[I];
        v += __shfl_xor(v, 16);
        v += __shfl_xor(v, 32);
        if (lane < 16) psum_part[gw * ROWS + 16 * I + lane] = v;
    }
}

template <int NB, bool WIDE, bool GENERAL>
__global__ void __launch_bounds__(256, 1)
k_build_gram(const double* __restrict__ u, int64_t ld, int64_t N, int64_t ntiles, const double* __restrict__ aden,
             const double* __restrict__ wsq, double* __restrict__ P, double* __restrict__ rinv_slot, double* __restrict__ gram_part) {
    extern __shared__ __attribute__((aligned(16))) char smem[];
    constexpr int ROWS = NB * 16;
    constexpr int NDMA = ROWS / 8;
    constexpr int U_BYTES = ROWS * TS * 8;
    constexpr int TILE_BYTES = U_BYTES + TS * 8;
    constexpr int NBLK = NB * (NB + 1) / 2;
    constexpr bool PINNED = NBLK > GRAM_AGPR_BLOCKS;
    const int lane = threadIdx.x & 63;
    const int wave = __builtin_amdgcn_readfirstlane(threadIdx.x >> 6);
    const int nwv = blockDim.x >> 6;
    const int ks = lane & 15, ns = lane >> 4;
    exp_table_init(smem);
    __syncthreads();
    char* buf = smem + EXP_TABLE_BYTES + wave * (2 * TILE_BYTES);
    const int64_t gw = (int64_t)blockIdx.x * nwv + wave;
    const int64_t W = (int64_t)gridDim.x * nwv;
    RowIdentity rows{0};
    const StageOffsetsT<WIDE> so = make_stage_offsets<WIDE>(ld, lane);

    double aL[NB];
    {
        double a[NB];
#pragma unroll
        for (int I = 0; I < NB; ++I) a[I] = aden[16 * I + ks];
        if constexpr (NB <= 2) rows.live = live_piece_mask<NB>(a, -INFINITY);
#pragma unroll
        for (int I = 0; I < NB; ++I) aL[I] = a[I] > -INFINITY ? a[I] * LOG2E_S : -1.0e9;
    }
#pragma unroll
    for (int I = 0; I < NB; ++I) settle(aL[I]);
    v4d G[NBLK];
#pragma unroll
    for (int b = 0; b < NBLK; ++b) G[b] = v4d{0.0, 0.0, 0.0, 0.0};
    const int rd_base = ks * (TS * 8);
    int pos[GROUPS];
#pragma unroll
    for (int g = 0; g < GROUPS; ++g) pos[g] = rd_base + ((4 * g + ns + (ks & 14)) & 15) * 8;

    auto stage = [&](int64_t tile, char* dst) {
        stage_tile<ROWS, true, 0, 1>(u, ld, tile * TS, dst, lane, so, rows);
        stage_vec16<true>(wsq, tile * TS, dst + U_BYTES, lane);
    };
    int64_t t = gw;
    int cur = 0;
    if (t < ntiles) stage(t, buf);
    for (; t < ntiles; t += W) {
        char* cbuf = buf + cur * TILE_BYTES;
        const int64_t tn = t + W;
        if (tn < ntiles) {
            stage(tn, buf + (cur ^ 1) * TILE_BYTES);
            if (t != gw)
                wait_vm<2 * (NDMA + 1)>();
            else
                wait_vm<NDMA + 1>();
        } else {
            wait_vm<0>();
        }
        const int nvalid = (int)(N - t * TS < TS ? N - t * TS : TS);
        auto mfma = [&](int b, double xx, double yy) {
            if constexpr (PINNED) {
                if (b < GRAM_AGPR_BLOCKS)
                    asm("v_mfma_f64_16x16x4_f64 %0, %1, %2, %0" : "+a"(G[b]) : "v"(xx), "v"(yy));
                else
                    asm("v_mfma_f64_16x16x4_f64 %0, %1, %2, %0" : "+v"(G[b]) : "v"(xx), "v"(yy));
            } else {
                G[b] = __builtin_amdgcn_mfma_f64_16x16x4f64(xx, yy, G[b], 0, 0, 0);
            }
        };
#pragma unroll
        for (int g = 0; g < GROUPS; g += 2) {
            double x0[NB], x1[NB];
#pragma unroll
            for (int I = 0; I < NB; ++I) {
                x0[I] = *reinterpret_cast<const double*>(cbuf + I * (16 * TS * 8) + pos[g]);
                x1[I] = *reinterpret_cast<const double*>(cbuf + I * (16 * TS * 8) + pos[g + 1]);
            }
            __builtin_amdgcn_sched_barrier(0);
#pragma unroll
            for (int I = 0; I < NB; ++I) {
                x0[I] = fma(x0[I], -LOG2E_S, aL[I]);
                x1[I] = fma(x1[I], -LOG2E_S, aL[I]);
            }
            double m0 = tree_max<NB>(x0), m1 = tree_max<NB>(x1);
            row16_max2(m0, m1);
#pragma unroll
            for (int I = 0; I < NB; ++I) {
                x0[I] = m0 - x0[I];
                x1[I] = m1 - x1[I];
            }
            exp2s_neg_batch2<NB, GENERAL>(x0, x1);
            double s0 = tree_sum<NB>(x0), s1 = tree_sum<NB>(x1);
            row16_sum2(s0, s1);
            double ri0 = recip_fast(s0), ri1 = recip_fast(s1);
            if (4 * g + ns >= nvalid) ri0 = 0.0;
            if (4 * g + 4 + ns >= nvalid) ri1 = 0.0;
            double p0[NB], p1[NB];
            if constexpr (GENERAL) {
                const double sw0 = *reinterpret_cast<const double*>(cbuf + U_BYTES + (4 * g + ns) * 8);
                const double sw1 = *reinterpret_cast<const double*>(cbuf + U_BYTES + (4 * g + 4 + ns) * 8);
#pragma unroll
                for (int I = 0; I < NB; ++I) {
                    x0[I] *= ri0;
                    x1[I] *= ri1;
                    *reinterpret_cast<double*>(cbuf + I * (16 * TS * 8) + pos[g]) = x0[I];
                    *reinterpret_cast<double*>(cbuf + I * (16 * TS * 8) + pos[g + 1]) = x1[I];
                    p0[I] = x0[I] * sw0;
                    p1[I] = x1[I] * sw1;
                }
            } else {
#pragma unroll
                for (int I = 0; I < NB; ++I) {
                    p0[I] = x0[I] * ri0;
                    p1[I] = x1[I] * ri1;
                    *reinterpret_cast<double*>(cbuf + I * (16 * TS * 8) + pos[g]) = p0[I];
                    *reinterpret_cast<double*>(cbuf + I * (16 * TS * 8) + pos[g + 1]) = p1[I];
                }
            }
            if constexpr (PINNED) {
                __builtin_amdgcn_sched_barrier(0);
                asm volatile("s_nop 7");
            }
            {
                int b = 0;
#pragma unroll
                for (int I = 0; I < NB; ++I)
#pragma unroll
                    for (int J = I; J < NB; ++J) mfma(b++, p0[I], p0[J]);
            }
            {
                int b = 0;
#pragma unroll
                for (int I = 0; I < NB; ++I)
#pragma unroll
                    for (int J = I; J < NB; ++J) mfma(b++, p1[I], p1[J]);
            }
            if constexpr (PINNED) __builtin_amdgcn_sched_barrier(0);
        }
        __builtin_amdgcn_fence(__ATOMIC_RELEASE, "wavefront");
        __builtin_amdgcn_wave_barrier();
#pragma unroll
        for (int j = 0; j < NDMA; ++j) {
            const double2 v = *reinterpret_cast<const double2*>(cbuf + j * 1024 + lane * 16);
            char* dst = reinterpret_cast<char*>(P + (int64_t)(8 * j) * ld + t * TS) + so.off[j & 1];
            store_p16(dst, v);
        }
        {
            const int64_t n = t * TS + lane;
            if (lane < TS && n < N) rinv_slot[n] = 1.0;
        }
        cur ^= 1;
    }
    if constexpr (PINNED) asm volatile("s_nop 15\n\ts_nop 15" ::: "memory");
#pragma unroll
    for (int b = 0; b < NBLK; ++b)
#pragma unroll
        for (int r = 0; r < 4; ++r) gram_part[((gw * NBLK + b) * 4 + r) * 64 + lane] = G[b][r];
}

template <int NB, int NF>
__device__ __forceinline__ void psweep_two_groups(const char* cbuf, int rd0, int rd1, const double (&c)[NF][NB],
                                                  double (&acc)[NF][NB], double w0, double w1, double (&r0)[NF],
                                                  double (&r1)[NF]) {
    double x0[NB], x1[NB];
#pragma unroll
    for (int I = 0; I < NB; ++I) {
        x0[I] = *reinterpret_cast<const double*>(cbuf + I * (16 * TS * 8) + rd0);
        x1[I] = *reinterpret_cast<const double*>(cbuf + I * (16 * TS * 8) + rd1);
    }
    __builtin_amdgcn_sched_barrier(0);
#pragma unroll
    for (int f = 0; f < NF; ++f) {
        double s0 = dot_sum<NB>(x0, c[f]), s1 = dot_sum<NB>(x1, c[f]);
        row16_sum2(s0, s1);
        r0[f] = recip_fast(fmax(s0, 1e-300));
        r1[f] = recip_fast(fmax(s1, 1e-300));
        const double q0 = w0 * r0[f], q1 = w1 * r1[f];
#pragma unroll
        for (int I = 0; I < NB; ++I) acc[f][I] = fma(x1[I], q1, fma(x0[I], q0, acc[f][I]));
    }
}

template <int NB, int NF, bool WIDE>
__global__ void __launch_bounds__(64 * lse_waves(NB))
k_psweep(const double* __restrict__ P, int64_t ld, int64_t N, int64_t ntiles, const double* __restrict__ cmul,
         const double* __restrict__ cw, double* __restrict__ rinv0, double* __restrict__ rinv1,
         double* __restrict__ psum_part, const int* __restrict__ ctl, int64_t slot_stride, int light_only) {
    extern __shared__ __attribute__((aligned(16))) char smem[];
    if (ctl) {
        if (ctl[CTL_DONE] != 0) return;
        if (light_only && ctl[CTL_LIGHT] == 0) return;
        const int s = ctl[CTL_SLOT];
        rinv1 = rinv0 + (int64_t)((s + 2) % 3) * slot_stride;
        rinv0 = rinv0 + (int64_t)((s + 1) % 3) * slot_stride;
    }
    constexpr int ROWS = NB * 16;
    constexpr int U_BYTES = ROWS * TS * 8;
    constexpr int TILE_BYTES = U_BYTES + TS * 8;
    const int lane = threadIdx.x & 63;
    const int wave = __builtin_amdgcn_readfirstlane(threadIdx.x >> 6);
    const int nwv = blockDim.x >> 6;
    const int ks = lane & 15, ns = lane >> 4;
    char* buf = smem + wave * (2 * TILE_BYTES);
    const int64_t gw = (int64_t)blockIdx.x * nwv + wave;
    const int64_t W = (int64_t)gridDim.x * nwv;
    RowIdentity rows{0};
    const StageOffsetsT<WIDE> so = make_stage_offsets<WIDE>(ld, lane);

    double c[NF][NB], acc[NF][NB];
#pragma unroll
    for (int f = 0; f < NF; ++f)
#pragma unroll
        for (int I = 0; I < NB; ++I) {
            c[f][I] = cmul[f * ROWS + 16 * I + ks];
            acc[f][I] = 0.0;
        }
#pragma unroll
    for (int f = 0; f < NF; ++f)
#pragma unroll
        for (int I = 0; I < NB; ++I) settle(c[f][I]);
    {
        double cany[NB];
#pragma unroll
        for (int I = 0; I < NB; ++I) cany[I] = NF == 2 ? fabs(c[0][I]) + fabs(c[NF - 1][I]) : c[0][I];
        rows.live = live_piece_mask<NB>(cany, 0.0);
    }
    const int rd_base = ks * (TS * 8);
    int pos[GROUPS];
#pragma unroll
    for (int g = 0; g < GROUPS; ++g) pos[g] = rd_base + ((4 * g + ns + (ks & 14)) & 15) * 8;
    const int gq = ks & 3;
    const int fq = (NF == 2 && (ks & 4)) ? 1 : 0;

    int64_t t = gw;
    int cur = 0;
    if (t < ntiles) {
        stage_tile<ROWS, true, 0, 1>(P, ld, t * TS, buf, lane, so, rows);
        stage_vec16<true>(cw, t * TS, buf + U_BYTES, lane);
    }
    for (; t < ntiles; t += W) {
// ... 55 lines not shown
    int64_t want = (ntiles + g.waves - 1) / g.waves;
    int64_t cap = (int64_t)num_cu * blocks_per_cu_for(g.lds_bytes);
    if (grid_override > 0) cap = grid_override;
    if (want < 1) want = 1;
    g.blocks = (int)(want < cap ? want : cap);
    g.nwaves = g.blocks * g.waves;
    g.psum_records = g.nwaves;
    return g;
}

template <int NB>
static hipError_t launch_psweep_nb(hipStream_t s, int nf, const LaunchGeom& g, const double* P, int64_t ld, int64_t N,
                                   const double* cmul, const double* cw, double* rinv0, double* rinv1, double* pp,
                                   const LoopCtl& lc) {
    auto go = [&](auto kern) -> hipError_t {
        if (g.lds_bytes > 64 * 1024) {
            hipError_t e = hipFuncSetAttribute(reinterpret_cast<const void*>(kern),
                                               hipFuncAttributeMaxDynamicSharedMemorySize, (int)g.lds_bytes);
            if (e != hipSuccess) return e;
        }
        const int64_t ntiles = (N + TS - 1) / TS;
        if (lc.ev_start && lc.ev_stop)
            hipExtLaunchKernelGGL(kern, dim3(g.blocks), dim3(g.waves * 64), g.lds_bytes, s, lc.ev_start, lc.ev_stop, 0, P, ld, N,
                                  ntiles, cmul, cw, rinv0, rinv1, pp, lc.ctl, lc.slot_stride, lc.light_only ? 1 : 0);
        else
            hipLaunchKernelGGL(kern, dim3(g.blocks), dim3(g.waves * 64), g.lds_bytes, s, P, ld, N, ntiles, cmul, cw, rinv0,
                               rinv1, pp, lc.ctl, lc.slot_stride, lc.light_only ? 1 : 0);
        return hipGetLastError();
    };
    const bool wide = stage_offsets_wide(ld);
    if (nf == 1) return wide ? go(k_psweep<NB, 1, true>) : go(k_psweep<NB, 1, false>);
    return wide ? go(k_psweep<NB, 2, true>) : go(k_psweep<NB, 2, false>);
}

hipError_t launch_psweep(hipStream_t s, int nb, int nf, const LaunchGeom& g, const double* P, int64_t ld, int64_t N,
                         const double* cmul, const double* cw, double* rinv0, double* rinv1, double* pp, const LoopCtl& lc) {
    switch (nb) {
#define MBAR_CASE(NB_) \
    case NB_: return launch_psweep_nb<NB_>(s, nf, g, P, ld, N, cmul, cw, rinv0, rinv1, pp, lc);
        MBAR_CASE(1) MBAR_CASE(2) MBAR_CASE(3) MBAR_CASE(4) MBAR_CASE(5) MBAR_CASE(6) MBAR_CASE(7) MBAR_CASE(8)
#undef MBAR_CASE
        default: return hipErrorInvalidValue;
    }
}

hipError_t launch_rinv_weighted(hipStream_t s, const double* rinv, const double* cw, int64_t N, double* out,
                                const LoopCtl& lc) {
    int64_t bx = (N + 255) / 256;
    if (bx > 2048) bx = 2048;
    if (bx < 1) bx = 1;
    hipLaunchKernelGGL(k_rinv_weighted, dim3((unsigned)bx), dim3(256), 0, s, rinv, cw, N, out, lc.ctl, lc.slot_stride);
    return hipGetLastError();
}

template <int NB>
static hipError_t launch_build_sweep_nb(hipStream_t s, const LaunchGeom& g, const double* u, int64_t ld, int64_t N,
                                        const double* aden, const double* cw, double* P, double* rinv_slot, double* pp) {
    auto go = [&](auto kern) -> hipError_t {
        if (g.lds_bytes > 64 * 1024) {
            hipError_t e = hipFuncSetAttribute(reinterpret_cast<const void*>(kern),
                                               hipFuncAttributeMaxDynamicSharedMemorySize, (int)g.lds_bytes);
            if (e != hipSuccess) return e;
        }
        const int64_t ntiles = (N + TS - 1) / TS;
        hipLaunchKernelGGL(kern, dim3(g.blocks), dim3(g.waves * 64), g.lds_bytes, s, u, ld, N, ntiles, aden, cw, P, rinv_slot, pp);
        return hipGetLastError();
    };
    return stage_offsets_wide(ld) ? go(k_build_sweep<NB, true>) : go(k_build_sweep<NB, false>);
}
LaunchGeom build_sweep_geometry(int nb, int num_cu, int64_t ntiles, int64_t grid_override) {
    return lse_geometry(nb, 1, num_cu, ntiles, grid_override, 1);
}
hipError_t launch_build_sweep(hipStream_t s, int nb, const LaunchGeom& g, const double* u, int64_t ld, int64_t N,
                              const double* aden, const double* cw, double* P, double* rinv_slot, double* pp) {
    switch (nb) {
#define MBAR_CASE(NB_) \
    case NB_: return launch_build_sweep_nb<NB_>(s, g, u, ld, N, aden, cw, P, rinv_slot, pp);
        MBAR_CASE(1) MBAR_CASE(2) MBAR_CASE(3) MBAR_CASE(4) MBAR_CASE(5) MBAR_CASE(6) MBAR_CASE(7) MBAR_CASE(8)
#undef MBAR_CASE
        default: return hipErrorInvalidValue;
    }
}

LaunchGeom build_gram_geometry(int nb, int num_cu, int64_t ntiles, int64_t grid_override) {
    LaunchGeom g = fused_geometry(nb, num_cu, ntiles, grid_override);
    g.lds_bytes = (size_t)4 * 2 * ((size_t)nb * 16 * TS * 8 + TS * 8) + EXP_TABLE_BYTES;
    return g;
}
template <int NB>
static hipError_t launch_build_gram_nb(hipStream_t s, const LaunchGeom& g, const double* u, int64_t ld, int64_t N,
                                       const double* aden, const double* wsq, bool general, double* P, double* rinv_slot, double* gp) {
    auto go = [&](auto kern) -> hipError_t {
        if (g.lds_bytes > 64 * 1024) {
            hipError_t e = hipFuncSetAttribute(reinterpret_cast<const void*>(kern),
                                               hipFuncAttributeMaxDynamicSharedMemorySize, (int)g.lds_bytes);
            if (e != hipSuccess) return e;
        }
        const int64_t ntiles = (N + TS - 1) / TS;
        hipLaunchKernelGGL(kern, dim3(g.blocks), dim3(256), g.lds_bytes, s, u, ld, N, ntiles, aden, wsq, P, rinv_slot, gp);
        return hipGetLastError();
    };
    if (general) return stage_offsets_wide(ld) ? go(k_build_gram<NB, true, true>) : go(k_build_gram<NB, false, true>);
    return stage_offsets_wide(ld) ? go(k_build_gram<NB, true, false>) : go(k_build_gram<NB, false, false>);
}
hipError_t launch_build_gram(hipStream_t s, int nb, const LaunchGeom& g, const double* u, int64_t ld, int64_t N,
                             const double* aden, const double* wsq, bool general, double* P, double* rinv_slot, double* gram_part) {
    switch (nb) {
#define MBAR_CASE(NB_) \
    case NB_: return launch_build_gram_nb<NB_>(s, g, u, ld, N, aden, wsq, general, P, rinv_slot, gram_part);
        MBAR_CASE(1) MBAR_CASE(2) MBAR_CASE(3) MBAR_CASE(4) MBAR_CASE(5) MBAR_CASE(6) MBAR_CASE(7) MBAR_CASE(8)
#undef MBAR_CASE
        default: return hipErrorInvalidValue;
    }
}

}
```

pymbar_amd/csrc/mbar_k_solver.hip:

```cpp
#include "mbar_device.h"

namespace mbar {

__global__ void __launch_bounds__(256)
k_reduce(const double* __restrict__ part, int64_t nparts, int64_t count, int64_t chunk,
         double* __restrict__ out) {
    const int64_t i = (int64_t)blockIdx.x * blockDim.x + threadIdx.x;
    if (i >= count) return;
    const int64_t p0 = (int64_t)blockIdx.y * chunk;
    const int64_t p1 = p0 + chunk < nparts ? p0 + chunk : nparts;
    double s = 0.0;
#pragma unroll 8
    for (int64_t p = p0; p < p1; ++p) s += part[p * count + i];
    out[(int64_t)blockIdx.y * count + i] = s;
}

constexpr int LN_ROWS = 8;
constexpr int LN_TILE = 64;
template <bool MASKED>
__device__ __forceinline__ void lognum_tile(const double* __restrict__ u, int64_t ld, int64_t N, int64_t K, int64_t k0,
                                            int64_t n, const double* __restrict__ logden, const double (&a)[LN_ROWS],
                                            double (&m)[LN_ROWS], double (&s)[LN_ROWS]) {
    const bool ok = !MASKED || n < N;
    const int64_t nn = ok ? n : 0;
    double v[LN_ROWS];
#pragma unroll
    for (int i = 0; i < LN_ROWS; ++i) v[i] = (k0 + i < K) ? u[(k0 + i) * ld + nn] : 0.0;
    const double nl = -logden[nn];
#pragma unroll
    for (int i = 0; i < LN_ROWS; ++i) {
        double x = (a[i] + nl) - v[i];
        if (MASKED && !ok) x = -INFINITY;
        const double d = x - m[i];
        const double e = exp2s_fast(-fabs(d) * LOG2E_S);
        s[i] = d > 0.0 ? fma(s[i], e, 1.0) : s[i] + e;
        m[i] = fmax(m[i], x);
    }
}
__global__ void __launch_bounds__(256)
k_lognum(const double* __restrict__ u, int64_t ld, int64_t N, int64_t K,
         const double* __restrict__ anum, const double* __restrict__ logden,
         double* __restrict__ pmax, double* __restrict__ psum, int64_t nchunks, int64_t tiles_per_chunk) {
    extern __shared__ __attribute__((aligned(16))) char smem[];
    exp_table_init(smem);
    __syncthreads();
    const int wave = threadIdx.x >> 6, lane = threadIdx.x & 63;
    const int64_t nsb = (K + LN_ROWS - 1) / LN_ROWS;
    const int64_t w = (int64_t)blockIdx.x * 4 + wave;
    const int64_t c = w / nsb, k0 = (w % nsb) * LN_ROWS;
    if (c >= nchunks) return;
    double a[LN_ROWS], m[LN_ROWS], s[LN_ROWS];
#pragma unroll
    for (int i = 0; i < LN_ROWS; ++i) {
        a[i] = (k0 + i < K) ? anum[k0 + i] : 0.0;
        m[i] = -INFINITY;
        s[i] = 0.0;
    }
    const int64_t ntiles = (N + LN_TILE - 1) / LN_TILE;
    const int64_t t0 = c * tiles_per_chunk;
    int64_t t1 = t0 + tiles_per_chunk;
    if (t1 > ntiles) t1 = ntiles;
    const int64_t tfull = (t1 * LN_TILE <= N) ? t1 : t1 - 1;
    int64_t t = t0;
    for (; t + 1 < tfull; t += 2) {
        lognum_tile<false>(u, ld, N, K, k0, t * LN_TILE + lane, logden, a, m, s);
        lognum_tile<false>(u, ld, N, K, k0, (t + 1) * LN_TILE + lane, logden, a, m, s);
    }
    for (; t < tfull; ++t) lognum_tile<false>(u, ld, N, K, k0, t * LN_TILE + lane, logden, a, m, s);
    for (; t < t1; ++t) lognum_tile<true>(u, ld, N, K, k0, t * LN_TILE + lane, logden, a, m, s);
#pragma unroll
    for (int i = 0; i < LN_ROWS; ++i) {
        const double mw = wave_max(m[i]);
        const double sc = (m[i] > -INFINITY) ? s[i] * exp(m[i] - mw) : 0.0;
        const double sw = wave_sum(sc);
        if (lane == 0 && k0 + i < K) {
            pmax[(k0 + i) * nchunks + c] = mw;
            psum[(k0 + i) * nchunks + c] = sw;
        }
    }
}

__global__ void __launch_bounds__(256)
k_lognum_merge(const double* __restrict__ pmax, const double* __restrict__ psum, int64_t nchunks,
               double* __restrict__ out_max, double* __restrict__ out_sum) {
    __shared__ double red[8];
    const int64_t k = blockIdx.x;
// ... 136 lines not shown
            if (k < K && q.Nk[k] > 0.0) {
                const double fo = q.f[k];
                const double fn = fo - log(psum[k] / q.Nk[k]) - f0new;
                q.f[k] = fn;
                q.f_hist[k] = fn;
                q.aden[k] = fn + q.lnNk[k];
                if (k != q.first) {
                    const double div = fabs(fn) < small ? 1.0 : fabs(fn);
                    const double d = fabs(fn - fo) / div;
                    dmax = (d > dmax || d != d) ? d : dmax;
                }
            } else {
                q.aden[k] = -INFINITY;
                q.f_hist[k] = k < K ? q.f[k] : 0.0;
            }
        }
    double m = dmax;
#pragma unroll
    for (int sft = 32; sft >= 1; sft >>= 1) {
        const double o = __shfl_xor(m, sft);
        m = (o > m || o != o) ? o : m;
    }
    if (act && (tid & 63) == 0) red[tid >> 6] = m;
    __syncthreads();
    if (tid == 0) {
        double r = red[0];
        for (int w = 1; w < 4; ++w) r = (red[w] > r || red[w] != red[w]) ? red[w] : r;
        *q.delta_out = r;
    }
}

__global__ void __launch_bounds__(256)
k_sci_update(const double* __restrict__ part, int64_t nparts, int64_t rows, SciArgs q) {
    __shared__ double red[5];
    extern __shared__ double psum[];
    sci_update_block(part, nparts, rows, q, psum, red);
}

__global__ void k_mfma_peak(int iters, double* sink) {
    v4d c[4];
#pragma unroll
    for (int i = 0; i < 4; ++i) c[i] = v4d{0.0, 0.0, 0.0, 0.0};
    const double a = 1.0 + threadIdx.x * 1e-9, b = 1.0 - threadIdx.x * 1e-9;
    for (int it = 0; it < iters; ++it) {
#pragma unroll
        for (int i = 0; i < 4; ++i) c[i] = __builtin_amdgcn_mfma_f64_16x16x4f64(a, b, c[i], 0, 0, 0);
    }
    double v = 0.0;
#pragma unroll
    for (int i = 0; i < 4; ++i) v += c[i][0] + c[i][3];
    if (v == 12345.678) sink[threadIdx.x] = v;
}


__global__ void __launch_bounds__(256)
k_make_p(const double* __restrict__ u, int64_t ld, int64_t N, int64_t rows, const double* __restrict__ aden,
         const double* __restrict__ logden, double* __restrict__ P) {
    const int64_t per_row = ld / 2;
    const int64_t total = rows * per_row;
    for (int64_t e = (int64_t)blockIdx.x * blockDim.x + threadIdx.x; e < total; e += (int64_t)gridDim.x * blockDim.x) {
        const int64_t k = e / per_row, n = (e - k * per_row) * 2;
        const double a = aden[k];
        const double2 uv = *reinterpret_cast<const double2*>(u + k * ld + n);
        double2 pv;
        pv.x = (n < N) ? exp(a - uv.x - logden[n]) : 0.0;
        pv.y = (n + 1 < N) ? exp(a - uv.y - logden[n + 1]) : 0.0;
        if (!(pv.x >= 0x1p-1022)) pv.x = 0.0;
        if (!(pv.y >= 0x1p-1022)) pv.y = 0.0;
        *reinterpret_cast<double2*>(P + k * ld + n) = pv;
    }
}
__global__ void __launch_bounds__(256) k_fill(double* __restrict__ v, double value, int64_t n) {
    for (int64_t i = (int64_t)blockIdx.x * blockDim.x + threadIdx.x; i < n; i += (int64_t)gridDim.x * blockDim.x) v[i] = value;
}
__global__ void __launch_bounds__(256) k_zero16(uint4* __restrict__ p, size_t n16) {
    const uint4 z = make_uint4(0u, 0u, 0u, 0u);
    for (size_t i = (size_t)blockIdx.x * blockDim.x + threadIdx.x; i < n16; i += (size_t)gridDim.x * blockDim.x) p[i] = z;
}
__global__ void __launch_bounds__(256) k_sqrt_vec(double* __restrict__ dst, const double* __restrict__ src, int64_t n) {
    for (int64_t i = (int64_t)blockIdx.x * blockDim.x + threadIdx.x; i < n; i += (int64_t)gridDim.x * blockDim.x) dst[i] = sqrt(src[i]);
}


__global__ void __launch_bounds__(256)
k_reduce2(const double* __restrict__ partA, int64_t countA, const double* __restrict__ partB, int64_t countB,
          int64_t nparts, int64_t chunk, double* __restrict__ outA, double* __restrict__ outB) {
    const int64_t gxA = (countA + 255) / 256;
    const bool isB = (int64_t)blockIdx.x >= gxA;
    const double* part = isB ? partB : partA;
    const int64_t count = isB ? countB : countA;
    double* out = isB ? outB : outA;
    const int64_t i = ((int64_t)blockIdx.x - (isB ? gxA : 0)) * blockDim.x + threadIdx.x;
    if (i >= count) return;
    const int64_t p0 = (int64_t)blockIdx.y * chunk;
    const int64_t p1 = p0 + chunk < nparts ? p0 + chunk : nparts;
    double s = 0.0;
#pragma unroll 8
    for (int64_t p = p0; p < p1; ++p) s += part[p * count + i];
    out[(int64_t)blockIdx.y * count + i] = s;
}


__device__ __forceinline__ double gram_elem(const double* __restrict__ g, int nb, int ki, int kj) {
    if (ki > kj) {
        const int t = ki;
        ki = kj;
        kj = t;
    }
    const int I = ki >> 4, J = kj >> 4;
    const int b = I * nb - (I * (I - 1)) / 2 + (J - I);
    return g[(int64_t)b * 256 + (ki & 15) * 16 + (kj & 15)];
}

__device__ __forceinline__ double block256_sum(double v, double* red ) {
    v = wave_sum(v);
    __syncthreads();
    if ((threadIdx.x & 63) == 0) red[threadIdx.x >> 6] = v;
    __syncthreads();
    return (red[0] + red[1]) + (red[2] + red[3]);
}
__device__ __forceinline__ double block256_max(double v, double* red ) {
    v = wave_max(v);
    __syncthreads();
    if ((threadIdx.x & 63) == 0) red[threadIdx.x >> 6] = v;
    __syncthreads();
    return fmax(fmax(red[0], red[1]), fmax(red[2], red[3]));
}

template <int NT>
__device__ __forceinline__ void newton_tail(const AdaptArgs& q, const double* xs, bool bad, const double* s_f, const double* s_ps,
                                            const double* s_nk, const double* s_ln, const double* s_a0, const int* smp,
                                            const int* pos, int tid) {
    const double gamma = q.prm[0];
    const int first = smp[0];
    const double shift = s_f[first] - log(s_ps[first] / s_nk[first]);
    int flags = bad ? 1 : 0;
    const bool swap = q.fused && q.ctl[CTL_SCI] < (int)q.prm[2];
    const int o_sci = swap ? q.Kp : 0, o_nr = swap ? 0 : q.Kp;
    if (tid == 0) q.ctl[CTL_SPEC] = swap ? 0 : 1;
    const double tol = q.prm[1], tol_small = tol < 1e-8 ? tol : 1e-8, tol_diff = sqrt(tol);
    for (int k = tid; k < q.Kp; k += NT) {
        const bool sampled = k < q.K && s_nk[k] > 0.0;
        const double fk = s_f[k];
        double fs = fk, fn = fk, a0 = -INFINITY, rt = 1.0;
        if (sampled) {
            fn = fk - gamma * xs[pos[k]];
            fs = (fk - log(s_ps[k] / s_nk[k])) - shift;
            a0 = fs + s_ln[k];
            const double a1 = fn + s_ln[k];
            if (q.pmode) {
                const double d0 = a0 - s_a0[k], d1 = a1 - s_a0[k];
                if (!(fabs(d0) < 250.0) || !(fabs(d1) < 250.0)) flags |= 2;
                a0 = exp(d0);
                rt = exp(d1);
            } else {
                const double d = a1 - a0;
                rt = exp(d);
                if (!(fabs(d) < 300.0)) flags |= 2;
            }
            if (!isfinite(fs) || !isfinite(fn)) flags |= 4;
            if (k != first) {
                const double ds = fabs(fs) < tol_small ? 1.0 : fabs(fs), dn = fabs(fn) < tol_small ? 1.0 : fabs(fn);
                const double gap = fabs(fs - fn);
                if (!(fabs(fs - fk) / ds < tol) || !(fabs(fn - fk) / dn < tol) || !(gap / ds < tol_diff) || !(gap / dn < tol_diff)) flags |= 8;
            }
        } else if (q.pmode) {
            a0 = 0.0;
            rt = 0.0;
        }
        q.cand[k] = fs;
        q.cand[q.Kp + k] = fn;
        q.ratio[k] = rt;
        q.aden[o_sci + k] = a0;
        q.aden[o_nr + k] = rt;
    }
    {
        __shared__ int s_flags;
        if (tid == 0) s_flags = 0;
        __syncthreads();
        if (flags) atomicOr(&s_flags, flags);
        __syncthreads();
        flags = s_flags;
// ... 757 lines not shown
                }
            }
#pragma unroll
            for (int b = 0; b < 4; ++b) {
                if (4 * w2 + b < nb) {
#pragma unroll
                    for (int r = 0; r < 16; ++r) xv = fma(wt[b][r], readlane_f64(xv, 16 * b + r), xv);
                }
            }
            s_x[64 * w2 + lane] = xv;
        }
        __syncthreads();
    }
    if (tid == 0) {
        s_x[0] = 0.0;
        s_x[first] = 0.0;
    }
    __syncthreads();
    bool bad = false;
    if (tid < 128 && tid < q.Kp && s_live[tid]) {
        const double pvv = s_pv[tid];
        bad = !(pvv > piv_thr) || !isfinite(pvv);
    }
    if (st && tid == 0) st[4] = clock64();
    newton_tail<256>(q, s_x, bad, s_f, s_ps, s_nk, s_ln, s_a0, s_first, s_pos, tid);
}
template <int NB>
__global__ void __launch_bounds__(256) __attribute__((amdgpu_waves_per_eu(2, 2)))
k_newton_ldlt(AdaptArgs q) {
    extern __shared__ __attribute__((aligned(16))) double select_dyn_lds[];
    newton_body_ldlt<NB>(q, select_dyn_lds, nullptr);
}

template <int R>
__global__ void __launch_bounds__(256)
k_select_newton(AdaptArgs q, int gram_in_lds) {
    extern __shared__ __attribute__((aligned(16))) double select_dyn_lds[];
    long long* st = q.stamps ? q.stamps + 16 * (q.ctl[CTL_ITER] & 63) : nullptr;
    if (st && threadIdx.x == 0) st[0] = clock64();
    select_body(q, gram_in_lds ? select_dyn_lds : nullptr);
    __syncthreads();
    if (st && threadIdx.x == 0) st[1] = clock64();
    newton_body<16, R>(q, st);
    if (st && threadIdx.x == 0) st[5] = clock64();
}
template <int NB>
__global__ void __launch_bounds__(256) __attribute__((amdgpu_waves_per_eu(2, 2)))
k_select_newton_ldlt(AdaptArgs q, int gram_in_lds) {
    extern __shared__ __attribute__((aligned(16))) double select_dyn_lds[];
    long long* st = q.stamps ? q.stamps + 16 * (q.ctl[CTL_ITER] & 63) : nullptr;
    if (st && threadIdx.x == 0) st[0] = clock64();
    select_body(q, gram_in_lds ? select_dyn_lds : nullptr, st);
    __syncthreads();
    if (st && threadIdx.x == 0) st[1] = clock64();
    newton_body_ldlt<NB>(q, select_dyn_lds, gram_in_lds ? select_dyn_lds : nullptr, st);
    if (st && threadIdx.x == 0) st[5] = clock64();
}

__global__ void __launch_bounds__(256)
k_loop_reduce(LoopSrc src, int64_t count, int op, double* __restrict__ out) {
    const int64_t i = (int64_t)blockIdx.x * blockDim.x + threadIdx.x;
    if (i >= count) return;
    double v = src.p[0][i];
    for (int r = 1; r < src.n; ++r) v = op == 0 ? v + src.p[r][i] : fmax(v, src.p[r][i]);
    out[i] = v;
}

__global__ void k_ctl_resume(int* ctl) {
    if (threadIdx.x == 0 && ctl[CTL_DONE] == 3) {
        ctl[CTL_DONE] = 0;
        ctl[CTL_NEEDGRAM] = 0;
    }
}



hipError_t launch_reduce(hipStream_t s, const double* part, int64_t nparts, int64_t count, double* scratch,
                         double* out) {
    const unsigned gx = (unsigned)((count + 255) / 256);
    if (nparts <= 32) {
        hipLaunchKernelGGL(k_reduce, dim3(gx, 1), dim3(256), 0, s, part, nparts, count, nparts, out);
        return hipGetLastError();
    }
    const int64_t chunk = 32;
    const int64_t n1 = (nparts + chunk - 1) / chunk;
    hipLaunchKernelGGL(k_reduce, dim3(gx, (unsigned)n1), dim3(256), 0, s, part, nparts, count, chunk, scratch);
    hipLaunchKernelGGL(k_reduce, dim3(gx, 1), dim3(256), 0, s, (const double*)scratch, n1, count, n1, out);
    return hipGetLastError();
}

static int64_t lognum_tiles_per_chunk(int64_t N, int64_t K) {
    const int64_t ntiles = (N + LN_TILE - 1) / LN_TILE;
    const int64_t nsb = (K + LN_ROWS - 1) / LN_ROWS;
    int64_t target = 16384 / nsb;
    if (target < 1) target = 1;
    int64_t tpc = (ntiles + target - 1) / target;
    return tpc < 1 ? 1 : tpc;
}
int64_t lognum_chunks(int64_t N, int64_t K) {
    const int64_t ntiles = (N + LN_TILE - 1) / LN_TILE;
    const int64_t tpc = lognum_tiles_per_chunk(N, K);
    const int64_t n = (ntiles + tpc - 1) / tpc;
    return n < 1 ? 1 : n;
}

hipError_t launch_lognum(hipStream_t s, const double* u, int64_t ld, int64_t N, int64_t K, const double* anum,
                         const double* logden, double* pmax, double* psum, int64_t nchunks) {
    const int64_t nsb = (K + LN_ROWS - 1) / LN_ROWS;
    const int64_t waves = nsb * nchunks;
    hipLaunchKernelGGL(k_lognum, dim3((unsigned)((waves + 3) / 4)), dim3(256), EXP_TABLE_BYTES, s, u, ld, N, K, anum, logden, pmax,
                       psum, nchunks, lognum_tiles_per_chunk(N, K));
    return hipGetLastError();
}

hipError_t launch_lognum_merge(hipStream_t s, const double* pmax, const double* psum, int64_t K, int64_t nchunks,
                               double* out_max, double* out_sum) {
    hipLaunchKernelGGL(k_lognum_merge, dim3((unsigned)K), dim3(256), 0, s, pmax, psum, nchunks, out_max, out_sum);
    return hipGetLastError();
}

hipError_t launch_logw(hipStream_t s, const double* u, int64_t ld, int64_t N, int64_t K, const double* f,
                       const double* logden, double* out, int64_t ld_out, bool exponentiate) {
    int64_t bx = (N + 255) / 256;
    if (bx > 2048) bx = 2048;
    if (bx < 1) bx = 1;
    if (exponentiate)
        hipLaunchKernelGGL(k_logw<true>, dim3((unsigned)bx, (unsigned)K), dim3(256), 0, s, u, ld, N, f, logden, out, ld_out);
    else
        hipLaunchKernelGGL(k_logw<false>, dim3((unsigned)bx, (unsigned)K), dim3(256), 0, s, u, ld, N, f, logden, out, ld_out);
    return hipGetLastError();
}

hipError_t launch_check_u(hipStream_t s, const double* u, int64_t ld, int64_t N, int64_t K, int* flags) {
    int64_t bx = (N + 255) / 256;
    if (bx > 1024) bx = 1024;
    if (bx < 1) bx = 1;
    hipLaunchKernelGGL(k_check_u, dim3((unsigned)bx, (unsigned)K), dim3(256), 0, s, u, ld, N, flags);
    return hipGetLastError();
}

hipError_t launch_shift_logden(hipStream_t s, const double* logden, const double* cw, double alpha, int64_t N,
                               double* out, const LoopCtl& lc) {
    int64_t bx = (N + 255) / 256;
    if (bx > 2048) bx = 2048;
    if (bx < 1) bx = 1;
    hipLaunchKernelGGL(k_shift_logden, dim3((unsigned)bx), dim3(256), 0, s, logden, cw, alpha, N, out, lc.ctl, lc.slot_stride);
    return hipGetLastError();
}

hipError_t launch_generate_harmonic(hipStream_t s, double* u, int64_t ld, int64_t N, int64_t K, uint64_t seed,
                                    const double* O_k, const double* K_k, const int64_t* cumN,
                                    int64_t n_global0) {
    int64_t bx = (N + 255) / 256;
    if (bx > 4096) bx = 4096;
    if (bx < 1) bx = 1;
    hipLaunchKernelGGL(k_generate_harmonic, dim3((unsigned)bx), dim3(256), 0, s, u, ld, N, K, seed, O_k, K_k, cumN,
                       n_global0);
    return hipGetLastError();
}

__global__ void __launch_bounds__(256)
k_fill_masked_rows(double* __restrict__ rows, int64_t ld, int64_t n, const double* __restrict__ v,
                   const int* __restrict__ label) {
    const int i = blockIdx.y;
    double* row = rows + (int64_t)i * ld;
    for (int64_t k = (int64_t)blockIdx.x * blockDim.x + threadIdx.x; k < n; k += (int64_t)gridDim.x * blockDim.x)
        row[k] = label[k] == i ? v[k] : INFINITY;
// ... 44 lines not shown
    __shared__ double red[4];
    for (int64_t r = blockIdx.y; r < nrows; r += gridDim.y) {
        double m = INFINITY;
        for (int i = threadIdx.x; i < nparts; i += blockDim.x) m = fmin(m, part[r * nparts + i]);
        m = -block256_max(-m, red);
        const double shift = m - fabs(8.881784197001252e-16 * m);
        if (blockIdx.x == 0 && threadIdx.x == 0) shift_out[r] = shift;
        for (int64_t i = (int64_t)blockIdx.x * blockDim.x + threadIdx.x; i < n; i += (int64_t)gridDim.x * blockDim.x)
            base[r * ld + i] = log(base[r * ld + i] - shift);
        __syncthreads();
    }
}
hipError_t launch_rows_logshift(hipStream_t s, double* base, int64_t ld, int64_t nrows, int64_t n, double* part, double* shift_out) {
    const int64_t want = (n + 2047) / 2048;
    const unsigned gx = (unsigned)(want < 256 ? (want < 1 ? 1 : want) : 256);
    const unsigned gy = (unsigned)(nrows < 1024 ? (nrows < 1 ? 1 : nrows) : 1024);
    hipLaunchKernelGGL(k_rows_min_partial, dim3(gx, gy), dim3(256), 0, s, base, ld, nrows, n, part);
    hipLaunchKernelGGL(k_rows_logshift, dim3(gx, gy), dim3(256), 0, s, base, ld, nrows, n, part, (int)gx, shift_out);
    return hipGetLastError();
}
__global__ void __launch_bounds__(256) k_rows_obs(double* __restrict__ dst, const double* __restrict__ obs, const double* __restrict__ state,
                                                  int64_t ld, int64_t nrows, int64_t n, const double* __restrict__ part, int nparts,
                                                  double* __restrict__ shift_out) {
    __shared__ double red[4];
    for (int64_t r = blockIdx.y; r < nrows; r += gridDim.y) {
        double m = INFINITY;
        for (int i = threadIdx.x; i < nparts; i += blockDim.x) m = fmin(m, part[r * nparts + i]);
        m = -block256_max(-m, red);
        const double shift = m - fabs(8.881784197001252e-16 * m);
        if (blockIdx.x == 0 && threadIdx.x == 0) shift_out[r] = shift;
        for (int64_t i = (int64_t)blockIdx.x * blockDim.x + threadIdx.x; i < n; i += (int64_t)gridDim.x * blockDim.x)
            dst[r * ld + i] = state[r * ld + i] - log(obs[r * ld + i] - shift);
        __syncthreads();
    }
}
hipError_t launch_rows_obs(hipStream_t s, double* dst, const double* obs, const double* state, int64_t ld, int64_t nrows, int64_t n,
                           double* part, double* shift_out, bool have_min) {
    const int64_t want = (n + 2047) / 2048;
    const unsigned gx = (unsigned)(want < 256 ? (want < 1 ? 1 : want) : 256);
    const unsigned gy = (unsigned)(nrows < 1024 ? (nrows < 1 ? 1 : nrows) : 1024);
    if (!have_min) hipLaunchKernelGGL(k_rows_min_partial, dim3(gx, gy), dim3(256), 0, s, obs, ld, nrows, n, part);
    hipLaunchKernelGGL(k_rows_obs, dim3(gx, gy), dim3(256), 0, s, dst, obs, state, ld, nrows, n, (const double*)part, have_min ? 1 : (int)gx,
                       shift_out);
    return hipGetLastError();
}
hipError_t launch_rows_rsub(hipStream_t s, double* dst, const double* src, int64_t ld, int64_t nrows, int64_t n) {
    const int64_t want = (n + 255) / 256;
    const unsigned gx = (unsigned)(want < 2048 ? (want < 1 ? 1 : want) : 2048);
    const unsigned gy = (unsigned)(nrows < 1024 ? (nrows < 1 ? 1 : nrows) : 1024);
    hipLaunchKernelGGL(k_rows_rsub, dim3(gx, gy), dim3(256), 0, s, dst, src, ld, nrows, n);
    return hipGetLastError();
}
hipError_t launch_rows_sub(hipStream_t s, double* dst, const double* src, int64_t ld, int64_t nrows, const double* v, int64_t n) {
    const int64_t want = (n + 255) / 256;
    const unsigned gx = (unsigned)(want < 2048 ? (want < 1 ? 1 : want) : 2048);
    const unsigned gy = (unsigned)(nrows < 1024 ? (nrows < 1 ? 1 : nrows) : 1024);
    hipLaunchKernelGGL(k_rows_sub, dim3(gx, gy), dim3(256), 0, s, dst, src, ld, nrows, v, n);
    return hipGetLastError();
}

hipError_t launch_sci_update(hipStream_t s, const double* part, int64_t nparts, int64_t rows, const double* Nk,
                             const double* lnNk, int64_t K, int64_t Kp, int first_state, double tol, double* f,
                             double* aden, double* f_hist, double* delta_out) {
    const SciArgs q{Nk, lnNk, K, Kp, first_state, tol, f, aden, f_hist, delta_out};
    hipLaunchKernelGGL(k_sci_update, dim3(1), dim3(256), (size_t)(Kp + 256) * sizeof(double), s, part, nparts, rows, q);
    return hipGetLastError();
}

hipError_t launch_reduce_level1(hipStream_t s, const double* part, int64_t nparts, int64_t count, double* out,
                                int64_t* nchunks) {
    const int64_t chunk = 32;
    const int64_t n1 = (nparts + chunk - 1) / chunk;
    const unsigned gx = (unsigned)((count + 255) / 256);
    hipLaunchKernelGGL(k_reduce, dim3(gx, (unsigned)n1), dim3(256), 0, s, part, nparts, count, chunk, out);
    *nchunks = n1;
    return hipGetLastError();
}

hipError_t launch_mfma_peak(hipStream_t s, int blocks, int iters, double* sink) {
    hipLaunchKernelGGL(k_mfma_peak, dim3(blocks), dim3(256), 0, s, iters, sink);
    return hipGetLastError();
}

hipError_t launch_reduce2(hipStream_t s, const double* partA, int64_t countA, const double* partB, int64_t countB,
                          int64_t nparts, double* scratch, double* outA, double* outB) {
    const unsigned gx = (unsigned)((countA + 255) / 256 + (countB + 255) / 256);
    if (nparts <= 32) {
        hipLaunchKernelGGL(k_reduce2, dim3(gx, 1), dim3(256), 0, s, partA, countA, partB, countB, nparts, nparts, outA, outB);
        return hipGetLastError();
    }
    const int64_t chunk = 32;
    const int64_t n1 = (nparts + chunk - 1) / chunk;
    double* sA = scratch;
    double* sB = scratch + n1 * countA;
    hipLaunchKernelGGL(k_reduce2, dim3(gx, (unsigned)n1), dim3(256), 0, s, partA, countA, partB, countB, nparts, chunk, sA, sB);
    hipLaunchKernelGGL(k_reduce2, dim3(gx, 1), dim3(256), 0, s, (const double*)sA, countA, (const double*)sB, countB, n1, n1,
                       outA, outB);
    return hipGetLastError();
}

hipError_t launch_newton(hipStream_t s, const AdaptArgs& a) {
    const int M = a.m - 1;
    if (M > 127 || a.Kp > 128) return hipErrorInvalidValue;
    if (a.newton_ldlt) {
        const size_t lds = (size_t)LDLT_LDS_DOUBLES * sizeof(double);
        auto go = [&](auto kern) -> hipError_t {
            hipError_t e = hipFuncSetAttribute(reinterpret_cast<const void*>(kern), hipFuncAttributeMaxDynamicSharedMemorySize, (int)lds);
            if (e != hipSuccess) return e;
            hipLaunchKernelGGL(kern, dim3(1), dim3(256), lds, s, a);
            return hipGetLastError();
        };
        return a.Kp <= 64 ? go(k_newton_ldlt<4>) : go(k_newton_ldlt<8>);
    }
    if (M <= 31)
        hipLaunchKernelGGL((k_newton<8, 4>), dim3(1), dim3(64), 0, s, a);
    else if (M <= 63)
        hipLaunchKernelGGL((k_newton<16, 4>), dim3(1), dim3(256), 0, s, a);
    else
        hipLaunchKernelGGL((k_newton<16, 8>), dim3(1), dim3(256), 0, s, a);
    return hipGetLastError();
}

hipError_t launch_loop_reduce(hipStream_t s, const LoopSrc& src, int64_t count, int op, double* out) {
    if (count < 1 || src.n < 1 || src.n > 8) return hipErrorInvalidValue;
    hipLaunchKernelGGL(k_loop_reduce, dim3((unsigned)((count + 255) / 256)), dim3(256), 0, s, src, count, op, out);
    return hipGetLastError();
}

hipError_t launch_newton_chol(hipStream_t s, const AdaptArgs& a, double* work) {
    const int M = a.m - 1;
    if (M < 0 || M > CHOL_NP - 1 || a.Kp > 256) return hipErrorInvalidValue;
    double* Aw = work;
    double* thr = work + (size_t)CHOL_NP * CHOL_NP;
    hipLaunchKernelGGL(k_chol_setup, dim3(CHOL_NP / 16, CHOL_NP / 16), dim3(256), 0, s, a, Aw, thr);
    for (int j0 = 0; j0 < M; j0 += CB) {
        hipLaunchKernelGGL(k_chol_panel, dim3(1), dim3(256), 0, s, a, Aw, (const double*)thr, j0);
        const int rows_below = M + 1 - (j0 + CB);
        if (rows_below > 0) {
            const int nt = (rows_below + CB - 1) / CB;
            hipLaunchKernelGGL(k_chol_update, dim3((unsigned)(nt * (nt + 1) / 2)), dim3(256), 0, s, a, Aw, j0);
        }
    }
    hipLaunchKernelGGL(k_chol_finish, dim3(1), dim3(256), 0, s, a, (const double*)Aw);
    return hipGetLastError();
}

hipError_t launch_ctl_resume(hipStream_t s, int* ctl) {
    hipLaunchKernelGGL(k_ctl_resume, dim3(1), dim3(64), 0, s, ctl);
    return hipGetLastError();
}

hipError_t launch_select_newton(hipStream_t s, const AdaptArgs& a) {
    const int M = a.m - 1;
    if (M > 127 || a.Kp > 128) return hipErrorInvalidValue;
    const int stage = (a.fused && a.Kp == 128) ? 1 : 0;
    const size_t lds = a.newton_ldlt ? (size_t)LDLT_LDS_DOUBLES * sizeof(double) : stage ? (size_t)SELECT_GRAM_LDS_DOUBLES * sizeof(double) : 0;
    auto go = [&](auto kern) -> hipError_t {
        if (lds > 48 * 1024) {
            hipError_t e = hipFuncSetAttribute(reinterpret_cast<const void*>(kern), hipFuncAttributeMaxDynamicSharedMemorySize, (int)lds);
            if (e != hipSuccess) return e;
        }
        hipLaunchKernelGGL(kern, dim3(1), dim3(256), lds, s, a, stage);
        return hipGetLastError();
    };
    if (a.newton_ldlt) return a.Kp <= 64 ? go(k_select_newton_ldlt<4>) : go(k_select_newton_ldlt<8>);
    if (M <= 63) return go(k_select_newton<4>);
    return go(k_select_newton<8>);
}

hipError_t launch_select(hipStream_t s, const AdaptArgs& a) {
    if (a.Kp > 256) return hipErrorInvalidValue;
    const int stage = (a.fused && a.Kp == 128) ? 1 : 0;
    const size_t lds = stage ? (size_t)SELECT_GRAM_LDS_DOUBLES * sizeof(double) : 0;
    if (lds > 48 * 1024) {
        hipError_t e = hipFuncSetAttribute(reinterpret_cast<const void*>(k_select), hipFuncAttributeMaxDynamicSharedMemorySize, (int)lds);
        if (e != hipSuccess) return e;
    }
    hipLaunchKernelGGL(k_select, dim3(1), dim3(256), lds, s, a, stage);
    return hipGetLastError();
// ... 71 lines not shown
```

pymbar_amd/csrc/mbar_loops.cpp:

```cpp
#include "mbar_ctx.h"

using namespace mbar;
using namespace mbar::host;

namespace mbar {
namespace host {

int adaptive_host_loop(mbar_ctx* c, std::vector<double>& f, double tol, int64_t maxiter, int64_t min_sc_iter, double gamma,
                       int check_convergence, double* history, int64_t history_rows, mbar_solve_result& res,
                       std::vector<double>& psum, double& max_delta) {
    const int64_t K = c->K;
    const int m = (int)c->sampled.size();
    const int first = c->sampled[0];
    std::vector<double> f_old(K), cand(2 * (size_t)K), psum2(2 * (size_t)K);
    std::vector<double> H((size_t)m * m), g(m), x;
    std::vector<int> pos((size_t)K, -1);
    for (int i = 0; i < m; ++i) pos[(size_t)c->sampled[i]] = i;
    psum.assign(K, 0.0);
    int cur = 0;
    int rc = eval_core(c, f.data(), 1, 0, c->logden[cur], nullptr, psum.data(), nullptr, nullptr);
    if (rc) return rc;
    bool done = false;
    const GramPlan plan = plan_for(c);
    const bool dbg = std::getenv("MBAR_DEBUG_TIMING") != nullptr;
// ... 267 lines not shown
    int rc = allreduce_host(c, &v, 1, 1);
    if (rc) return rc;
    ok = !(v > 0.0);
    return MBAR_OK;
}

template <class Enqueue>
int capture_batch(mbar_ctx* c, hipGraphExec_t* exec, int64_t batch, Enqueue&& enqueue) {
    hipGraph_t graph = nullptr;
    HIPCHK(c, hipStreamBeginCapture(c->stream, hipStreamCaptureModeThreadLocal));
    int crc = MBAR_OK;
    for (int64_t b = 0; b < batch && crc == MBAR_OK; ++b) crc = enqueue(b);
    hipError_t ee = hipStreamEndCapture(c->stream, &graph);
    if (crc) return crc;
    if (ee != hipSuccess) return fail(c, MBAR_ERR_HIP, std::string("hipStreamEndCapture: ") + hipGetErrorString(ee));
    ee = hipGraphInstantiate(exec, graph, nullptr, nullptr, 0);
    (void)hipGraphDestroy(graph);
    if (ee != hipSuccess) return fail(c, MBAR_ERR_HIP, std::string("hipGraphInstantiate: ") + hipGetErrorString(ee));
    return MBAR_OK;
}

struct DeviceLoopPlan {
    int m = 0, nb = 0;
    bool wide = false;
    bool pmode = false;
    bool fused = false;
    bool light = false;
    bool unit = false;
    bool merged = false;
    bool warm = false;
    bool use_graph = false;
    LaunchGeom gg, gl, gp, gb;
    size_t rec_g = 0, rec_l = 0, off_gram = 0;
    LoopCtl lc_slot, lc_flat;
    int64_t batch = 0, graph_sig = 0;
    std::vector<double> an0, cm0;
};

int plan_device_loop(mbar_ctx* c, const std::vector<double>& f, int check_convergence, const double* history, int64_t history_rows,
                     DeviceLoopPlan& p) {
    const int64_t Kp = c->Kp;
    const int64_t ntiles = (c->N + TS - 1) / TS;
    const int nb = p.nb = (int)(Kp / 16);
    p.m = (int)c->sampled.size();
    const bool wide = p.wide = Kp > 128;
    bool pmode = c->opt_pmode && !c->P_failed && (!wide || (c->opt_wide_pmode && c->opt_fused));
    int arc = ensure_ad(c, history ? history_rows : 0);
    if (!arc && wide && !c->chol && cache_malloc((void**)&c->chol, NEWTON_CHOL_WORK * sizeof(double)) != hipSuccess)
        arc = fail(c, MBAR_ERR_HIP, "allocation of the Newton workspace failed");
    if (!arc && pmode && !c->P) {
        arc = drop_graphs(c);
        if (!arc) {
            if (cache_malloc((void**)&c->P, (size_t)Kp * c->ld * sizeof(double)) != hipSuccess) {
                (void)hipGetLastError();
                c->P = nullptr;
                c->P_failed = true;
                pmode = false;
            } else if (launch_zero(c->stream, c->P, (size_t)Kp * c->ld * sizeof(double)) != hipSuccess) {
                arc = fail(c, MBAR_ERR_HIP, "zero fill of P failed");
            }
        }
    }
    {
        bool p_ok = pmode;
        int rc = agree_all_ok(c, p_ok);
        if (rc) return rc;
        if (pmode && !p_ok) {
            pmode = false;
            c->error = "resident probability matrix does not fit on every rank: classic sweeps";
        }
    }
    p.pmode = pmode;
    if (!arc && pmode && !c->pm_vec && cache_malloc((void**)&c->pm_vec, (size_t)3 * Kp * sizeof(double)) != hipSuccess)
        arc = fail(c, MBAR_ERR_HIP, "allocation of the P-mode vectors failed");
    const bool fused = p.fused = pmode && c->opt_fused;
    p.merged = fused && !wide && c->opt_merge_select;
    bool light = fused && check_convergence && c->opt_light_last != 0 &&
                 (c->opt_light_last >= 2 || (nb >= 5 && (double)Kp * (double)c->N >= 5.0e7));
    LaunchGeom& gg = p.gg;
    LaunchGeom& gl = p.gl;
    LaunchGeom& gp = p.gp;
    gg = wide ? gram_quad_geometry(nb, c->num_cu, ntiles, c->opt_grid) : gram_geometry(nb * 16, true, c->num_cu, ntiles, c->opt_grid);
    p.unit = !c->weighted && !c->opt_fused_general;
    gl = fused ? fused_geometry(nb, c->num_cu, ntiles, c->opt_grid, p.unit)
         : pmode ? psweep_geometry(nb, c->num_cu, ntiles, c->opt_grid)
                 : lse_geometry(nb, 2, c->num_cu, ntiles, c->opt_grid, lse_variant_for(c));
    if (wide) gg.live_blocks = gl.live_blocks = quad_live_blocks(c);
    if (fused) {
        gg.blocks = gl.blocks;
        gg.nwaves = gl.nwaves;
    }
    gp = psweep_geometry(wide ? 8 : nb, c->num_cu, ntiles, 0);
    if (light && !wide && gl.nwaves % gp.waves != 0) light = false;
    if (light && !wide) {
        gp.blocks = gl.nwaves / gp.waves;
        gp.nwaves = gp.psum_records = gl.nwaves;
    }
    {
        bool l_ok = light;
        int rcl = agree_all_ok(c, l_ok);
        if (rcl) return rcl;
        light = light && l_ok;
    }
    p.light = light;
    const LaunchGeom& gb = p.gb = fused ? build_gram_geometry(nb, c->num_cu, ntiles, c->opt_grid)
                                        : build_sweep_geometry(nb, c->num_cu, ntiles, c->opt_grid);
    const size_t rec_g = p.rec_g = (size_t)nb * (nb + 1) / 2 * 256;
    const size_t rec_l = p.rec_l = (size_t)2 * Kp;
    const size_t off_gram = p.off_gram = rec_l + 2;
    if (!arc) arc = ensure_red(c, off_gram + rec_g);
    if (!arc)
        arc = ensure(c, &c->part, &c->part_doubles,
                     std::max(std::max((size_t)gg.nwaves * rec_g, (size_t)gl.nwaves * (rec_l + 2)), (size_t)gb.nwaves * Kp));
    if (!arc)
        arc = ensure(c, &c->scratch, &c->scratch_doubles,
                     std::max(((size_t)std::max(gg.nwaves, gl.nwaves) / 32 + 1) * (rec_g + rec_l + 2), ((size_t)gb.nwaves / 32 + 1) * (Kp + rec_g)));
    if (!arc && c->weighted && !c->lden_eff) arc = fail(c, MBAR_ERR_STATE, "weighted context without its logden buffer");
    if (!arc && fused) arc = ensure(c, &c->part_g, &c->part_g_doubles, (size_t)gl.nwaves * rec_g);
    {
        bool ok = arc == MBAR_OK;
        const std::string local_err = c->error;
        int rc = agree_all_ok(c, ok);
        if (rc) return rc;
        if (arc) return arc;
        if (!ok) return fail(c, MBAR_ERR_STATE, "a peer rank could not allocate its solver buffers");
        c->error = local_err;
    }
    p.lc_slot.ctl = p.lc_flat.ctl = c->ad_ints;
    p.lc_slot.slot_stride = c->ld;
    p.lc_slot.unclamped = p.lc_flat.unclamped = c->u_checked && !c->u_posinf;
    p.lc_slot.pmode = p.lc_flat.pmode = pmode;
    p.batch = c->opt_adapt_batch;
    p.use_graph = c->opt_graph && !stream_transport(c);
    p.graph_sig = ((int64_t)gg.blocks << 40) ^ ((int64_t)gl.blocks << 20) ^ ((int64_t)p.m << 12) ^ (pmode ? 128 : 0) ^ (fused ? 256 : 0) ^
                  (c->weighted ? 64 : 0) ^ (p.lc_slot.unclamped ? 512 : 0) ^ (p.merged ? 1024 : 0) ^ (light ? 2048 : 0) ^ (int64_t)nb;
    p.an0.assign((size_t)Kp, 0.0);
    p.cm0.assign((size_t)Kp, 0.0);
    build_aden(c, f.data(), p.an0.data(), Kp);
    bool warm = fused && c->opt_pcache && c->P_valid && (int64_t)c->P_a0.size() == Kp;
    for (int64_t k = 0; warm && k < Kp; ++k) {
        const bool live = !std::isinf(p.an0[k]), was = !std::isinf(c->P_a0[k]);
        if (live != was) warm = false;
        else if (live) {
            const double d = p.an0[k] - c->P_a0[k];
            if (!(std::fabs(d) < 200.0)) warm = false;
            p.cm0[k] = std::exp(d);
        }
    }
    int rc = agree_all_ok(c, warm);
    if (rc) return rc;
    p.warm = warm;
    return MBAR_OK;
}


int start_classic(mbar_ctx* c, const DeviceLoopPlan&, const std::vector<double>& f, std::vector<double>& psum, mbar_solve_result&) {
    return eval_core(c, f.data(), 1, 0, c->logden[0], nullptr, psum.data(), nullptr, nullptr);
}

int start_warm(mbar_ctx* c, const DeviceLoopPlan& p, const std::vector<double>&, std::vector<double>& psum, mbar_solve_result& res) {
    const int64_t K = c->K, Kp = c->Kp;
    std::vector<int> z((size_t)CTL_WORDS, 0);
    HIPCHK(c, hipMemcpyAsync(c->ad_ints, z.data(), z.size() * sizeof(int), hipMemcpyHostToDevice, c->stream));
    std::copy(p.cm0.begin(), p.cm0.end(), c->hstage);
    std::copy(p.cm0.begin(), p.cm0.end(), c->hstage + Kp);
    HIPCHK(c, hipMemcpyAsync(d_aden(c), c->hstage, (size_t)2 * Kp * sizeof(double), hipMemcpyHostToDevice, c->stream));
    HIPCHK(c, hipMemsetAsync(c->red, 0, p.off_gram * sizeof(double), c->stream));
    {
        ScopedTimer t(c, MBAR_TIMER_OTHER);
        HIPCHK(c, launch_fused(c->stream, p.nb, p.gl, c->P, c->ld, c->N, d_aden(c), c->cw, c->weighted ? c->cwsq : c->cw, p.unit,
                               c->logden[0], c->part_g, c->part, p.lc_slot));
    }
    HIPCHK(c, launch_reduce2(c->stream, c->part, (int64_t)p.rec_l, c->part_g, (int64_t)p.rec_g, p.gl.nwaves, c->scratch, c->red,
                             c->red + p.off_gram));
    int rc = allreduce_dev(c, c->red, (int64_t)(p.off_gram + p.rec_g), 0);
    if (rc) return rc;
    HIPCHK(c, hipMemcpyAsync(c->hred, c->red, (size_t)Kp * sizeof(double), hipMemcpyDeviceToHost, c->stream));
    rc = sync_stream(c);
    if (rc) return rc;
    for (int64_t k = 0; k < K; ++k) psum[k] = c->hred[k] * p.cm0[k];
    res.warm_starts += 1;
    return MBAR_OK;
}

int start_build_wide(mbar_ctx* c, const DeviceLoopPlan& p, const std::vector<double>& f, std::vector<double>& psum, mbar_solve_result& res) {
    c->P_valid = false;
    int rc = eval_core(c, f.data(), 1, 0, c->logden[1], nullptr, psum.data(), nullptr, nullptr);
    if (rc) return rc;
    if (!c->weighted) {
        ScopedTimer t(c, MBAR_TIMER_OTHER);
        HIPCHK(c, launch_gram_quad(c->stream, p.nb, p.gg, c->u, c->ld, c->N, d_aden(c), c->logden[1], c->part_g, LoopCtl(), c->P));
        HIPCHK(c, launch_reduce(c->stream, c->part_g, p.gg.nwaves, (int64_t)p.rec_g, c->scratch, c->red + p.off_gram));
        rc = allreduce_dev(c, c->red + p.off_gram, (int64_t)p.rec_g, 0);
        if (rc) return rc;
        HIPCHK(c, launch_fill(c->stream, c->logden[0], 1.0, c->ld));
    } else {
        {
            ScopedTimer t(c, MBAR_TIMER_OTHER);
            HIPCHK(c, launch_make_p(c->stream, c->num_cu, c->u, c->ld, c->N, c->Kp, d_aden(c), c->logden[1], c->P));
            HIPCHK(c, launch_fill(c->stream, c->logden[0], 1.0, c->ld));
        }
        HIPCHK(c, launch_rinv_weighted(c->stream, c->logden[0], c->cw, c->N, c->lden_eff));
        LoopCtl lp;
        lp.pmode = true;
        {
            ScopedTimer t(c, MBAR_TIMER_GRAM);
            HIPCHK(c, launch_gram_quad(c->stream, p.nb, p.gg, c->P, c->ld, c->N, d_anum(c), c->lden_eff, c->part_g, lp));
        }
        HIPCHK(c, launch_reduce(c->stream, c->part_g, p.gg.nwaves, (int64_t)p.rec_g, c->scratch, c->red + p.off_gram));
        rc = allreduce_dev(c, c->red + p.off_gram, (int64_t)p.rec_g, 0);
        if (rc) return rc;
    }
    rc = sync_stream(c);
    if (rc) return rc;
    c->P_a0 = p.an0;
    c->P_valid = true;
    res.builds += 1;
    return MBAR_OK;
}

int reduce_to_host(mbar_ctx* c, const double* part, int64_t nrec, int64_t len, size_t off) {
    HIPCHK(c, launch_reduce(c->stream, part, nrec, len, c->scratch, c->red + off));
    int rc = allreduce_dev(c, c->red + off, len, 0);
    if (rc) return rc;
    HIPCHK(c, hipMemcpyAsync(c->hred + off, c->red + off, (size_t)len * sizeof(double), hipMemcpyDeviceToHost, c->stream));
    return sync_stream(c);
}

int start_build_narrow(mbar_ctx* c, const DeviceLoopPlan& p, const std::vector<double>& f, std::vector<double>& psum, mbar_solve_result& res) {
    const int64_t K = c->K, Kp = c->Kp;
    c->P_valid = false;
    build_aden(c, f.data(), c->hstage, Kp);
    HIPCHK(c, hipMemcpyAsync(d_aden(c), c->hstage, (size_t)Kp * sizeof(double), hipMemcpyHostToDevice, c->stream));
    HIPCHK(c, hipMemsetAsync(c->red, 0, p.off_gram * sizeof(double), c->stream));
    {
        ScopedTimer t(c, MBAR_TIMER_OTHER);
        if (p.fused)
            HIPCHK(c, launch_build_gram(c->stream, p.nb, p.gb, c->u, c->ld, c->N, d_aden(c), c->weighted ? c->cwsq : c->cw,
                                        c->weighted || !p.lc_slot.unclamped, c->P, c->logden[0], c->part_g));
        else
            HIPCHK(c, launch_build_sweep(c->stream, p.nb, p.gb, c->u, c->ld, c->N, d_aden(c), c->cw, c->P, c->logden[0], c->part));
    }
    if (p.fused) {
        int rc = reduce_to_host(c, c->part_g, p.gb.nwaves, (int64_t)p.rec_g, p.off_gram);
        if (rc) return rc;
        gram_row_sums(c->hred + p.off_gram, p.nb, K, psum.data());
    } else {
        int rc = reduce_to_host(c, c->part, p.gb.nwaves, Kp, 0);
        if (rc) return rc;
        for (int64_t k = 0; k < K; ++k) psum[k] = c->hred[k];
    }
    c->P_a0 = p.an0;
    c->P_valid = true;
    res.builds += 1;
    return MBAR_OK;
}

int upload_state(mbar_ctx* c, const DeviceLoopPlan& p, const std::vector<double>& f, const std::vector<double>& psum, double tol,
                 int64_t min_sc_iter, double gamma, int check_convergence, const mbar_solve_result& res) {
    const int64_t K = c->K, Kp = c->Kp;
    std::vector<double> h(ad_off_hist(c), 0.0);
    for (int64_t k = 0; k < K; ++k) {
        h[ad_off_f() + k] = f[k];
        h[ad_off_psum(c) + k] = psum[k];
    }
    h[ad_off_prm(c) + 0] = gamma;
    h[ad_off_prm(c) + 1] = tol;
    h[ad_off_prm(c) + 2] = (double)std::min<int64_t>(min_sc_iter, 1 << 30);
    h[ad_off_prm(c) + 3] = check_convergence ? 1.0 : 0.0;
    h[ad_off_state(c)] = std::numeric_limits<double>::quiet_NaN();
    std::vector<int> hi((size_t)CTL_WORDS + Kp, 0);
    hi[CTL_NEEDGRAM] = p.fused ? 0 : 1;
    hi[CTL_GRAMSWEEPS] = 0;
    hi[CTL_SPEC] = 1;
    hi[CTL_SLOT] = p.warm ? 1 : 0;
    hi[CTL_ITER] = (int)res.iterations;
    hi[CTL_SCI] = (int)res.sci_iter;
    hi[CTL_NR] = (int)res.nr_iter;
    for (int i = 0; i < p.m; ++i) hi[CTL_WORDS + i] = c->sampled[i];
    HIPCHK(c, hipMemcpyAsync(c->ad, h.data(), h.size() * sizeof(double), hipMemcpyHostToDevice, c->stream));
    HIPCHK(c, hipMemcpyAsync(c->ad_ints, hi.data(), hi.size() * sizeof(int), hipMemcpyHostToDevice, c->stream));
    HIPCHK(c, hipMemcpyAsync(d_anum(c), p.an0.data(), p.an0.size() * sizeof(double), hipMemcpyHostToDevice, c->stream));
    std::vector<double> pv;
    if (p.pmode) {
        pv.assign((size_t)3 * Kp, 1.0);
        std::copy(c->P_a0.begin(), c->P_a0.end(), pv.begin());
        for (int64_t k = 0; k < Kp; ++k) {
            if (p.warm) pv[(size_t)Kp + k] = pv[(size_t)2 * Kp + k] = p.cm0[k];
            if (!(k < K && c->Nk[k] > 0.0)) pv[(size_t)Kp + k] = pv[(size_t)2 * Kp + k] = 0.0;
        }
        HIPCHK(c, hipMemcpyAsync(c->pm_vec, pv.data(), pv.size() * sizeof(double), hipMemcpyHostToDevice, c->stream));
    }
    HIPCHK(c, hipStreamSynchronize(c->stream));
    return MBAR_OK;
}

int make_adapt_args(mbar_ctx* c, const DeviceLoopPlan& p, AdaptArgs& q) {
    const int64_t Kp = c->Kp;
    q.gram_red = c->red + p.off_gram;
    q.lse_red = c->red;
    q.f = c->ad + ad_off_f();
    q.psum = c->ad + ad_off_psum(c);
    q.cand = c->ad + ad_off_cand(c);
    q.ratio = c->ad + ad_off_ratio(c);
    q.aden = d_aden(c);
    q.anum = d_anum(c);
    q.Nk = d_Nk(c);
    q.lnNk = d_lnNk(c);
    q.sampled = c->ad_ints + CTL_WORDS;
    q.m = p.m;
    q.K = (int)c->K;
    q.Kp = (int)Kp;
    q.ctl = c->ad_ints;
    q.prm = c->ad + ad_off_prm(c);
    q.state = c->ad + ad_off_state(c);
    q.hist = c->ad + ad_off_hist(c);
    q.hist_cap = c->ad_hist_cap;
    q.pmode = p.pmode ? 1 : 0;
    q.a0 = c->pm_vec;
    q.ccur = p.pmode ? c->pm_vec + Kp : nullptr;
    q.fused = p.fused ? 1 : 0;
    q.cgram = p.fused ? c->pm_vec + 2 * Kp : nullptr;
    q.light_ok = p.light ? 1 : 0;
    q.newton_ldlt = c->opt_newton_ldlt ? 1 : 0;
    if (const char* e = std::getenv("MBAR_NEWTON_LDLT")) q.newton_ldlt = std::atoi(e) != 0 ? 1 : 0;
    q.stamps = nullptr;
    if (std::getenv("MBAR_DEBUG_STAMPS")) {
// ... 37 lines not shown
    mbar_ctx* c;
    const DeviceLoopPlan& p;
    AdaptArgs q;
    double* gram_part;
    bool need_newton = true;
    int64_t it, it_start;
    int32_t gram_sweeps = 0;
    bool converged = false, handed_back = false;

    DeviceLoop(mbar_ctx* c_, const DeviceLoopPlan& p_, int64_t it0)
        : c(c_), p(p_), gram_part(p_.fused ? c_->part_g : c_->part), it(it0), it_start(it0) {}
    bool take_need_newton() {
        const bool n = need_newton;
        need_newton = false;
        return n;
    }

    int enqueue_gram(bool timed) {
        const double* lden = c->logden[0];
        LoopCtl lca = p.lc_slot;
        if (p.fused) HIPCHK(c, launch_ctl_resume(c->stream, c->ad_ints));
        if (c->weighted) {
            if (p.pmode)
                HIPCHK(c, launch_rinv_weighted(c->stream, c->logden[0], c->cw, c->N, c->lden_eff, p.lc_slot));
            else
                HIPCHK(c, launch_shift_logden(c->stream, c->logden[0], c->cw, 0.5, c->N, c->lden_eff, p.lc_slot));
            lden = c->lden_eff;
            lca = p.lc_flat;
        }
        {
            LaunchTimer t(c, MBAR_TIMER_GRAM, timed, lca);
            if (p.wide)
                HIPCHK(c, launch_gram_quad(c->stream, p.nb, p.gg, p.pmode ? c->P : c->u, c->ld, c->N, d_anum(c), lden, gram_part, lca));
            else
                HIPCHK(c, launch_gram_diag(c->stream, p.nb, p.gg, p.pmode ? c->P : c->u, c->ld, c->N, d_anum(c), lden, 0, gram_part,
                                           nullptr, lca));
        }
        HIPCHK(c, launch_reduce(c->stream, gram_part, p.gg.nwaves, (int64_t)p.rec_g, c->scratch, c->red + p.off_gram));
        if (stream_transport(c)) {
            int r2 = allreduce_dev(c, c->red + p.off_gram, (int64_t)p.rec_g, 0);
            if (r2) return r2;
        }
        return MBAR_OK;
    }

    int enqueue_iteration(bool timed, bool own_newton) {
        const bool split = timed && c->opt_timing == 3;
        const bool solve = p.wide || !p.merged || own_newton;
        if (!p.fused) {
            int r2 = enqueue_gram(timed);
            if (r2) return r2;
        }
        {
            ScopedTimer sec(c, MBAR_TIMER_NEWTON, split && solve);
            if (p.wide)
                HIPCHK(c, launch_newton_chol(c->stream, q, c->chol));
            else if (solve)
                HIPCHK(c, launch_newton(c->stream, q));
        }
        double* psum_part = c->part;
        double* obj_part = c->part + (size_t)p.gl.nwaves * p.rec_l;
        {
            LoopCtl lcb = p.lc_slot;
            LaunchTimer t(c, p.fused ? MBAR_TIMER_FUSED : MBAR_TIMER_LSE, timed, lcb);
            if (p.fused) {
                HIPCHK(c, launch_fused(c->stream, p.nb, p.gl, c->P, c->ld, c->N, d_aden(c), c->cw, c->weighted ? c->cwsq : c->cw, p.unit,
                                       c->logden[0], gram_part, psum_part, lcb));
                if (p.light && !p.wide) {
                    LoopCtl lcl = p.lc_slot;
                    lcl.light_only = true;
                    HIPCHK(c, launch_psweep(c->stream, p.nb, 2, p.gp, c->P, c->ld, c->N, d_aden(c), c->cw, c->logden[0], nullptr, psum_part, lcl));
                }
            } else if (p.pmode)
                HIPCHK(c, launch_psweep(c->stream, p.nb, 2, p.gl, c->P, c->ld, c->N, d_aden(c), c->cw, c->logden[0], nullptr, psum_part,
                                        lcb));
            else
                HIPCHK(c, launch_lse(c->stream, p.nb, 2, p.gl, c->u, c->ld, c->N, d_aden(c), c->cw, c->logden[0], nullptr,
                                     nullptr, psum_part, obj_part, lcb));
        }
        int64_t ar_count = (int64_t)(p.rec_l + 2);
        {
            ScopedTimer sec(c, MBAR_TIMER_REDUCE, split);
            if (p.fused) {
                HIPCHK(c, launch_reduce2(c->stream, psum_part, (int64_t)p.rec_l, gram_part, (int64_t)p.rec_g, p.gl.nwaves, c->scratch, c->red,
                                         c->red + p.off_gram));
                ar_count = (int64_t)(p.off_gram + p.rec_g);
            } else if (p.pmode) {
                HIPCHK(c, launch_reduce(c->stream, psum_part, p.gl.nwaves, (int64_t)p.rec_l, c->scratch, c->red));
            } else {
                HIPCHK(c, launch_reduce2(c->stream, psum_part, (int64_t)p.rec_l, obj_part, 2, p.gl.nwaves, c->scratch, c->red, c->red + p.rec_l));
            }
        }
        if (stream_transport(c)) {
            ScopedTimer sec(c, MBAR_TIMER_COMM, split);
            int r2 = allreduce_dev(c, c->red, ar_count, 0);
            if (r2) return r2;
        }
        {
            ScopedTimer sec(c, MBAR_TIMER_NEWTON, split);
            if (p.merged)
                HIPCHK(c, launch_select_newton(c->stream, q));
            else
                HIPCHK(c, launch_select(c->stream, q));
        }
        return MBAR_OK;
    }

    int prepare_graph() {
        if (c->ad_graph && c->ad_graph_batch == p.batch && c->ad_graph_sig == p.graph_sig) return MBAR_OK;
        if (c->ad_graph) HIPCHK(c, hipGraphExecDestroy(c->ad_graph));
        c->ad_graph = nullptr;
        int one = 1;
        HIPCHK(c, hipMemcpyAsync(c->ad_ints + CTL_DONE, &one, sizeof(int), hipMemcpyHostToDevice, c->stream));
        int rc = enqueue_iteration(false, false);
        if (rc) return rc;
        int zero = 0;
        HIPCHK(c, hipMemcpyAsync(c->ad_ints + CTL_DONE, &zero, sizeof(int), hipMemcpyHostToDevice, c->stream));
        HIPCHK(c, hipStreamSynchronize(c->stream));
        rc = capture_batch(c, &c->ad_graph, p.batch, [&](int64_t) { return enqueue_iteration(false, false); });
        if (rc) return rc;
        c->ad_graph_batch = p.batch;
        c->ad_graph_sig = p.graph_sig;
        return MBAR_OK;
    }

    int run(int64_t maxiter, int check_convergence) {
        BatchSchedule sched(p.batch, !check_convergence);
        const bool timed = c->opt_timing != 0;
        bool done = false;
        int rc = MBAR_OK;
        while (it < maxiter && !done) {
            const BatchSchedule::Round round = sched.next();
            int64_t nbat = 0;
            for (int rep = 0; rep < round.reps && it + nbat < maxiter; ++rep) {
                const int64_t nb1 = std::min(round.want, maxiter - it - nbat);
                if (p.use_graph && nb1 == p.batch) {
                    rc = prepare_graph();
                    if (rc) return rc;
                    if (take_need_newton() && p.merged) HIPCHK(c, launch_newton(c->stream, q));
                    HIPCHK(c, hipGraphLaunch(c->ad_graph, c->stream));
                } else {
                    for (int64_t b = 0; b < nb1; ++b) {
                        rc = enqueue_iteration(timed, take_need_newton());
                        if (rc) return rc;
                    }
                }
                nbat += nb1;
            }
            HIPCHK(c, hipMemcpyAsync(c->h_ctl, c->ad_ints, CTL_WORDS * sizeof(int), hipMemcpyDeviceToHost, c->stream));
            rc = sync_stream(c);
            if (rc) return rc;
            const int64_t it_new = c->h_ctl[CTL_ITER];
            if (c->h_ctl[CTL_DONE] == 1) {
                converged = true;
                done = true;
            } else if (c->h_ctl[CTL_DONE] == 2) {
                handed_back = true;
                done = true;
            } else if (c->h_ctl[CTL_DONE] == 3) {
                if (it_new <= it || it_new > it + nbat) return fail(c, MBAR_ERR_STATE, "device-resident adaptive loop lost count of its iterations");
                if (it_new < maxiter) {
                    rc = enqueue_gram(timed);
                    if (rc) return rc;
                    ++gram_sweeps;
                    sched.paused();
                    need_newton = true;
                }
            } else if (it_new != it + nbat) {
                return fail(c, MBAR_ERR_STATE, "device-resident adaptive loop lost count of its iterations");
            }
            it = it_new;
        }
        return MBAR_OK;
// ... 64 lines not shown
int dump_sci_small_stamps(mbar_ctx* c) {
    long long st[24];
    HIPCHK(c, hipMemcpy(st, c->stamps, sizeof(st), hipMemcpyDeviceToHost));
    std::fprintf(stderr, "[mbar] k_sci_small workgroup 0, end of the tile loop per wave (us):");
    for (int w = 0; w < 8; ++w) std::fprintf(stderr, " %.2f", (st[16 + w] - st[0]) * 0.01);
    std::fprintf(stderr, "\n");
    for (int w = 0; w < 2; ++w) {
        const long long* p = st + 8 * w;
        std::fprintf(stderr, "[mbar] k_sci_small workgroup %s (us since its start; start offset to workgroup 0: %.2f): tables %.2f, update done %.2f, first tile in %.2f, "
                     "sweep done %.2f, barrier %.2f, record written %.2f\n", w ? "mid" : "0", (p[0] - st[0]) * 0.01, (p[1] - p[0]) * 0.01, (p[2] - p[0]) * 0.01,
                     (p[3] - p[0]) * 0.01, (p[4] - p[0]) * 0.01, (p[5] - p[0]) * 0.01, (p[6] - p[0]) * 0.01);
    }
    return MBAR_OK;
}


}
}

extern "C" {

int mbar_solve_adaptive(mbar_ctx* c, double* f_inout, double tol, int64_t maxiter, int64_t min_sc_iter, double gamma,
                        int check_convergence, double* history, int64_t history_rows, mbar_solve_result* result) {
    if (c && c->ext_base) return fail(c, MBAR_ERR_STATE, "mbar_solve_adaptive: an extension context holds rows only (mbar_lognum_ext / mbar_gram_w_ext sweep them)");
    if (!c || !f_inout) return fail(c, MBAR_ERR_ARG, "NULL argument");
    if (!c->have_Nk) return fail(c, MBAR_ERR_STATE, "mbar_ctx_set_Nk has not been called");
    HIPCHK(c, hipSetDevice(c->device));
    const double t0 = now_ms();
    const int64_t K = c->K;
    std::vector<double> f(f_inout, f_inout + K), psum;
    mbar_solve_result res;
    std::memset(&res, 0, sizeof(res));
    struct Ld0Guard {
        mbar_ctx* c;
        ~Ld0Guard() { c->ld0_valid = false; }
    } ld0_guard{c};
    c->ld0_valid = false;
    double max_delta = std::numeric_limits<double>::quiet_NaN();
    int rc = refresh_poison(c);
    if (rc) return rc;
    bool on_device = device_loop_eligible(c) && !c->u_poison && f_is_finite(c, f.data(), 1) && maxiter > 0;
    int handbacks = 0;
    while (on_device) {
        bool handed_back = false;
        rc = adaptive_device_loop(c, f, tol, maxiter, min_sc_iter, gamma, check_convergence, history, history_rows, res, psum,
                                  max_delta, handed_back);
        if (rc) return rc;
        if (!handed_back) break;
        const int reason = c->h_ctl[CTL_REASON];
        const bool one_off = (reason == 2 || reason == 3) && ++handbacks <= 6 && res.iterations + 1 < maxiter;
        if (!one_off) {
            on_device = false;
            break;
        }
        rc = adaptive_host_loop(c, f, tol, res.iterations + 1, min_sc_iter, gamma, check_convergence, history, history_rows, res,
                                psum, max_delta);
        if (rc) return rc;
        if (res.success || !f_is_finite(c, f.data(), 1)) break;
    }
    if (!on_device && !res.success && res.iterations < maxiter) {
        rc = adaptive_host_loop(c, f, tol, maxiter, min_sc_iter, gamma, check_convergence, history, history_rows, res, psum,
                                max_delta);
        if (rc) return rc;
    }
    const int m = (int)c->sampled.size();
    double gn = 0.0;
    for (int i = 0; i < m && (int64_t)psum.size() == K; ++i) {
        const int k = c->sampled[i];
        gn += (psum[k] - c->Nk[k]) * (psum[k] - c->Nk[k]);
    }
    res.gnorm = std::sqrt(gn);
    c->ld0_valid = false;
    c->last_psum = (int64_t)psum.size() == K ? psum : std::vector<double>();
    res.max_delta = max_delta;
    res.wall_ms = now_ms() - t0;
    if (std::getenv("MBAR_DEBUG_TIMING") && res.iterations > 0)
        std::fprintf(stderr, "[mbar] adaptive: %lld iterations, %.3f ms per iteration (%s loop)\n", (long long)res.iterations,
                     res.wall_ms / res.iterations, on_device ? "device-resident" : "host-driven");
    std::copy(f.begin(), f.end(), f_inout);
    if (result) *result = res;
    return MBAR_OK;
}

int mbar_ctx_last_solve_psum(mbar_ctx* c, double* psum_out) {
    if (!c || !psum_out) return fail(c, MBAR_ERR_ARG, "NULL argument");
    if ((int64_t)c->last_psum.size() != c->K) return fail(c, MBAR_ERR_STATE, "no adaptive solve has left its per-state sums on this context");
    std::copy(c->last_psum.begin(), c->last_psum.end(), psum_out);
    return MBAR_OK;
}

int mbar_solve_sci(mbar_ctx* c, double* f_inout, double tol, int64_t maxiter, int check_convergence,
                   mbar_solve_result* result) {
    if (c && c->ext_base) return fail(c, MBAR_ERR_STATE, "mbar_solve_sci: an extension context holds rows only (mbar_lognum_ext / mbar_gram_w_ext sweep them)");
    if (!c || !f_inout) return fail(c, MBAR_ERR_ARG, "NULL argument");
    if (!c->have_Nk) return fail(c, MBAR_ERR_STATE, "mbar_ctx_set_Nk has not been called");
    HIPCHK(c, hipSetDevice(c->device));
    const double t0 = now_ms();
    const int64_t K = c->K, Kp = c->Kp;
    const int first = c->sampled[0];
    mbar_solve_result res;
    std::memset(&res, 0, sizeof(res));
    struct Ld0Guard {
        mbar_ctx* c;
        ~Ld0Guard() { c->ld0_valid = false; }
    } ld0_guard{c};
    c->ld0_valid = false;
    {
        int prc = refresh_poison(c);
        if (prc) return prc;
        if (c->u_poison || !f_is_finite(c, f_inout, 1)) {
            for (int64_t k = 0; k < K; ++k)
                if (c->Nk[k] > 0.0) f_inout[k] = std::numeric_limits<double>::quiet_NaN();
            res.success = 1;
            res.max_delta = std::numeric_limits<double>::quiet_NaN();
            if (result) *result = res;
            return MBAR_OK;
        }
    }
    const int64_t rows = lse_rows(c);
    const int64_t batch = c->opt_sci_batch;
    if (!c->f_hist) HIPCHK(c, cache_malloc((void**)&c->f_hist, (size_t)256 * Kp * sizeof(double)));
    int rc = ensure_red(c, (size_t)rows + 8);
    if (rc) return rc;
    std::vector<double> hf((size_t)Kp, 0.0), ha((size_t)std::max(rows, Kp));
    for (int64_t k = 0; k < K; ++k) hf[k] = f_inout[k];
    build_aden(c, f_inout, ha.data(), std::max(rows, Kp));
    HIPCHK(c, hipMemcpyAsync(d_f(c), hf.data(), Kp * sizeof(double), hipMemcpyHostToDevice, c->stream));
    HIPCHK(c, hipMemcpyAsync(d_aden(c), ha.data(), std::max(rows, Kp) * sizeof(double), hipMemcpyHostToDevice, c->stream));
    HIPCHK(c, hipStreamSynchronize(c->stream));
    std::vector<double> hdelta(256);
    bool done = false;
    double last_delta = std::numeric_limits<double>::quiet_NaN();
    const bool fast = use_fast(c);
    const int nbk = (int)(rows / 16);
    const int64_t ntiles = (c->N + TS - 1) / TS;
    LaunchGeom g = fast ? lse_geometry(nbk, 1, c->num_cu, ntiles, c->opt_grid, lse_variant_for(c)) : LaunchGeom();
    g.balanced = c->opt_small_balanced ? 1 : 0;
    const bool merged = fast && g.variant == 4 && c->opt_sci_merged && c->nranks <= 1 && !c->comm && !stream_transport(c) &&
                        rows == Kp && batch % 2 == 0;
    if (fast) {
        rc = ensure(c, &c->part, &c->part_doubles, std::max((size_t)g.nwaves * (rows + 1), (size_t)2 * g.blocks * rows + g.blocks));
        if (rc) return rc;
        rc = ensure(c, &c->scratch, &c->scratch_doubles, ((size_t)g.nwaves / 32 + 16) * (rows + 1));
        if (rc) return rc;
    }
    auto prime_merged = [&]() -> int {
        HIPCHK(c, hipMemcpyAsync(c->scratch, hf.data(), rows * sizeof(double), hipMemcpyHostToDevice, c->stream));
        ScopedTimer t(c, MBAR_TIMER_LSE);
        HIPCHK(c, launch_lse(c->stream, nbk, 1, g, c->u, c->ld, c->N, d_aden(c), c->cw, nullptr, nullptr, nullptr, c->part,
                             c->part + (size_t)2 * g.blocks * rows));
        return MBAR_OK;
    };
    if (merged) {
        rc = prime_merged();
        if (rc) return rc;
    }
    int64_t it = 0;
    long long* sci_stamps = nullptr;
    if (merged && std::getenv("MBAR_DEBUG_STAMPS")) {
        if (!c->stamps) HIPCHK(c, hipMalloc((void**)&c->stamps, 65 * 16 * sizeof(long long)));
        HIPCHK(c, hipMemsetAsync(c->stamps, 0, 64 * 8 * sizeof(long long), c->stream));
        sci_stamps = c->stamps;
    }
    auto merged_args = [&](int64_t b) {
        SciLoopArgs q;
        q.Nk = d_Nk(c);
// ... 153 lines not shown
```

pymbar_amd/device.py:

```python
import ctypes as C

import numpy as np

from . import _lib


_dptr = _lib.ptr


class DeviceMatrix:

    def __init__(self, K, N_local, device=None):
        _lib.require_device()
        self._lib = _lib.load_library()
        self.K = int(K)
        self.N_local = int(N_local)
        self.device = _lib.default_device(device)
        self._ctx = C.c_void_p()
        rc = self._lib.mbar_ctx_create(C.byref(self._ctx), self.device, self.K, self.N_local)
        if rc != _lib.MBAR_OK:
            raise _lib.MbarHipError(rc, _lib.last_error(None))
        self._Nk = None
        self._version = 0
        self._wtag = None
# ... 231 lines not shown
            self._check(self._lib.mbar_ctx_set_objective_offset(self._ctx, None))
        else:
            f0 = np.ascontiguousarray(f0, dtype=np.float64)
            self._check(self._lib.mbar_ctx_set_objective_offset(self._ctx, _dptr(f0)))

    def lognum(self, f):
        f = np.ascontiguousarray(f, dtype=np.float64)
        out = np.empty(self.K, dtype=np.float64)
        self._check(self._lib.mbar_lognum(self._ctx, _dptr(f), _dptr(out)))
        return out

    def lognum_cached(self, f):
        f = np.ascontiguousarray(f, dtype=np.float64)
        if self._wtag is not None:
            return self.lognum(f)
        key = (self._version, f.tobytes())
        if self._lognum_cache is None or self._lognum_cache[0] != key:
            self._lognum_cache = (key, self.lognum(f))
        return self._lognum_cache[1].copy()

    def gram_w_cached(self, f):
        f = np.ascontiguousarray(f, dtype=np.float64)
        if self._wtag is not None:
            return self.gram_w(f)
        key = (self._version, f.tobytes())
        if self._gram_w_cache is None or self._gram_w_cache[0] != key:
            self._gram_w_cache = (key, self.gram_w(f))
        G, ws = self._gram_w_cache[1]
        return G.copy(), ws.copy()

    def extend(self, nrows):
        if self.nranks != 1:
            return None
        ctx = C.c_void_p()
        rc = self._lib.mbar_ctx_create_ext(C.byref(ctx), self._ctx, int(nrows))
        if rc != _lib.MBAR_OK:
            return None
        return ExtendedMatrix(self, ctx, int(nrows))

    def logden(self, f):
        f = np.ascontiguousarray(f, dtype=np.float64)
        out = np.empty(self.N_local, dtype=np.float64)
        self._check(self._lib.mbar_logden(self._ctx, _dptr(f), _dptr(out)))
        return out

    def logw_kn(self, f):
        f = np.ascontiguousarray(f, dtype=np.float64)
        from .utils import prefault

        out = prefault(np.empty((self.K, self.N_local), dtype=np.float64))
        self._check(self._lib.mbar_logw(self._ctx, _dptr(f), _dptr(out), self.N_local))
        return out

    def w_kn(self, f):
        from .utils import prefault

        f = np.ascontiguousarray(f, dtype=np.float64)
        out = prefault(np.empty((self.K, self.N_local), dtype=np.float64))
        self._check(self._lib.mbar_w(self._ctx, _dptr(f), _dptr(out), self.N_local))
        return out

    def gram_w(self, f):
        f = np.ascontiguousarray(f, dtype=np.float64)
        G = np.empty((self.K, self.K), dtype=np.float64)
        ws = np.empty(self.K, dtype=np.float64)
        self._check(self._lib.mbar_gram_w(self._ctx, _dptr(f), _dptr(G), _dptr(ws)))
        return G, ws

    def solve_adaptive(self, f, tol=1e-12, maxiter=10000, min_sc_iter=2, gamma=1.0, check_convergence=True,
                       history_rows=0):
        f = np.array(f, dtype=np.float64)
        res = _lib.SolveResult()
        hist = np.zeros((max(1, history_rows), 4), dtype=np.float64)
        self._check(self._lib.mbar_solve_adaptive(self._ctx, _dptr(f), tol, int(maxiter), int(min_sc_iter),
                                                  float(gamma), 1 if check_convergence else 0, _dptr(hist),
                                                  int(history_rows), C.byref(res)))
        out = {k: getattr(res, k) for k, _ in _lib.SolveResult._fields_ if not k.endswith("_")}
        out["success"] = bool(res.success)
        out["history"] = hist[: min(history_rows, res.iterations)]
        psum = np.empty(self.K, dtype=np.float64)
        out["psum"] = psum if self._lib.mbar_ctx_last_solve_psum(self._ctx, _dptr(psum)) == _lib.MBAR_OK else None
        return f, out

    def solve_sci(self, f, tol=1e-12, maxiter=10000, check_convergence=True):
        f = np.array(f, dtype=np.float64)
        res = _lib.SolveResult()
        self._check(self._lib.mbar_solve_sci(self._ctx, _dptr(f), tol, int(maxiter),
                                             1 if check_convergence else 0, C.byref(res)))
        out = {k: getattr(res, k) for k, _ in _lib.SolveResult._fields_ if not k.endswith("_")}
        out["success"] = bool(res.success)
        return f, out

    def timing(self):
        out = {}
        for name, which in (("lse", _lib.TIMER_LSE), ("gram", _lib.TIMER_GRAM), ("reduce", _lib.TIMER_REDUCE),
                            ("other", _lib.TIMER_OTHER), ("fused", _lib.TIMER_FUSED), ("newton", _lib.TIMER_NEWTON),
                            ("comm", _lib.TIMER_COMM)):
            ms = C.c_double(0.0)
            n = C.c_int64(0)
            self._check(self._lib.mbar_ctx_timing(self._ctx, which, C.byref(ms), C.byref(n)))
            out[name] = (ms.value, n.value)
        return out

    def timing_reset(self):
        self._check(self._lib.mbar_ctx_timing_reset(self._ctx))

    def mfma_f64_peak(self):
        t = C.c_double(0.0)
        self._check(self._lib.mbar_mfma_f64_peak(self._ctx, C.byref(t)))
        return t.value


class ExtendedMatrix:

    def __init__(self, base, ctx, nrows):
        self.base = base
        self._lib = base._lib
        self._ctx = ctx
        self.Kb = base.K
        self.K = base.K + nrows
        self.N_local = base.N_local
        self.nranks = 1

    def _check(self, rc):
        if rc != _lib.MBAR_OK:
            raise _lib.MbarHipError(rc, _lib.last_error(self._ctx))

    def close(self):
        if self._ctx:
            self._lib.mbar_ctx_destroy(self._ctx)
            self._ctx = C.c_void_p()

    def __enter__(self):
        return self

    def __exit__(self, *exc):
        self.close()

    def __del__(self):
        try:
            self.close()
        except Exception:
            pass

    def _ext_row(self, row, n=1):
        if row < self.Kb or row + n > self.K:
            raise ValueError("only the appended rows can be written")
        return int(row - self.Kb)

    def _src(self, row0, n):
        if row0 + n <= self.Kb:
            return self.base._ctx, int(row0)
        if row0 >= self.Kb:
            return self._ctx, int(row0 - self.Kb)
        raise ValueError("a source run straddles the resident and the appended rows")

    def upload_rows(self, row0, rows):
        rows = np.ascontiguousarray(np.atleast_2d(rows), dtype=np.float64)
        if rows.shape[1] != self.N_local:
            raise ValueError("rows must have N_local columns")
        self._check(self._lib.mbar_ctx_upload_rows(self._ctx, self._ext_row(row0, rows.shape[0]), rows.shape[0], _dptr(rows), rows.shape[1]))

    def copy_rows_from(self, src, dst_row0=0, src_row0=0, nrows=None):
        nrows = src.K - src_row0 if nrows is None else nrows
        if src is self.base and dst_row0 == 0 and src_row0 == 0 and nrows == self.Kb:
            return
# ... 99 lines not shown
```

Baseline: 294.6.

## Fold per-wave Gram partials in LDS and reduce partials in one launch

The fused and build-gram kernels (NB=8) now sum their four waves' Gram accumulators through LDS before writing. This leaves one Gram record per block instead of one per wave, cutting global partial-sum traffic. The two-level reduce2 is replaced by a single-launch kernel that chunks the parts per thread group and finishes in shared memory, with separate part counts for psum and Gram records. The changes add extra barriers and LDS reuse of the tile buffers at kernel exit. A debug entry point for inspecting one Gram sweep is also added.

```diff
diff --git a/include/mbar_hip.h b/include/mbar_hip.h
--- a/include/mbar_hip.h
+++ b/include/mbar_hip.h
@@ -116,6 +116,7 @@
                         int64_t min_sc_iter, double gamma, int check_convergence,
                         double* history, int64_t history_rows, mbar_solve_result* result);
 int mbar_ctx_last_solve_psum(mbar_ctx* ctx, double* psum);
+int mbar_ctx_debug_gram_sweep(mbar_ctx* ctx, const double* f, int build, double* psum, double* blocks, double* cmul);
 int mbar_solve_sci(mbar_ctx* ctx, double* f_inout, double tol, int64_t maxiter, int check_convergence,
                    mbar_solve_result* result);
 
diff --git a/pymbar_amd/_lib.py b/pymbar_amd/_lib.py
--- a/pymbar_amd/_lib.py
+++ b/pymbar_amd/_lib.py
@@ -119,6 +119,7 @@
     "mbar_solve_adaptive": (C.c_int, [_ctx, _dp, C.c_double, C.c_int64, C.c_int64, C.c_double, C.c_int,
                                       _dp, C.c_int64, C.POINTER(SolveResult)]),
     "mbar_ctx_last_solve_psum": (C.c_int, [_ctx, _dp]),
+    "mbar_ctx_debug_gram_sweep": (C.c_int, [_ctx, _dp, C.c_int, _dp, _dp, _dp]),
     "mbar_solve_sci": (C.c_int, [_ctx, _dp, C.c_double, C.c_int64, C.c_int, C.POINTER(SolveResult)]),
     "mbar_ctx_timing": (C.c_int, [_ctx, C.c_int, _dp, _ip]),
     "mbar_ctx_timing_reset": (C.c_int, [_ctx]),
diff --git a/pymbar_amd/csrc/mbar_capi.cpp b/pymbar_amd/csrc/mbar_capi.cpp
--- a/pymbar_amd/csrc/mbar_capi.cpp
+++ b/pymbar_amd/csrc/mbar_capi.cpp
@@ -132,7 +132,7 @@
         }
         {
             ScopedTimer t(c, MBAR_TIMER_REDUCE);
-            HIPCHK(c, launch_reduce2(c->stream, psum_part, (int64_t)rec, obj_part, nf, g.nwaves, c->scratch, c->red, c->red + rec));
+            HIPCHK(c, launch_reduce2(c->stream, psum_part, (int64_t)rec, g.nwaves, obj_part, nf, g.nwaves, c->red, c->red + rec));
         }
         return MBAR_OK;
     }
@@ -721,6 +721,14 @@
         c->opt_fused_general = value ? 1 : 0;
         (void)drop_graphs(c);
     }
+    else if (k == "gram_fold") {
+        c->opt_gram_fold = value ? 1 : 0;
+        (void)drop_graphs(c);
+    }
+    else if (k == "reduce_single") {
+        c->opt_reduce_single = value ? 1 : 0;
+        (void)drop_graphs(c);
+    }
     else if (k == "debug_download_p") c->opt_debug_download_p = value;
     else if (k == "direct_results") c->opt_direct_results = value;
     else if (k == "sci_merged") c->opt_sci_merged = value;
diff --git a/pymbar_amd/csrc/mbar_ctx.h b/pymbar_amd/csrc/mbar_ctx.h
--- a/pymbar_amd/csrc/mbar_ctx.h
+++ b/pymbar_amd/csrc/mbar_ctx.h
@@ -290,7 +290,7 @@
     bool P_valid = false;
     std::vector<double> P_a0;
     int64_t opt_grid = 0, opt_force_generic = 0, opt_check_finite = 1, opt_sci_batch = 16, opt_timing = 0, opt_graph = 1, opt_small = 1, opt_wide = 1;
-    int64_t opt_device_loop = 1, opt_adapt_batch = 8, opt_pmode = 1, opt_fused = 1, opt_quad = 1, opt_device_loop_wide = 1, opt_pcache = 1, opt_merge_select = 1, opt_sci_merged = 1, opt_wide_pmode = 1, opt_quad_trim = 1, opt_light_last = 1, opt_direct_results = 1, opt_debug_download_p = 0, opt_fused_general = 0;
+    int64_t opt_device_loop = 1, opt_adapt_batch = 8, opt_pmode = 1, opt_fused = 1, opt_quad = 1, opt_device_loop_wide = 1, opt_pcache = 1, opt_merge_select = 1, opt_sci_merged = 1, opt_wide_pmode = 1, opt_quad_trim = 1, opt_light_last = 1, opt_direct_results = 1, opt_debug_download_p = 0, opt_fused_general = 0, opt_gram_fold = 1, opt_reduce_single = 1;
     int64_t opt_small_balanced = 1, opt_sci_pingpong = 1, opt_host_pmode = 2, opt_rect_waves = 8, opt_newton_ldlt = 1;
 
     ncclComm_t comm = nullptr;
diff --git a/pymbar_amd/csrc/mbar_device.h b/pymbar_amd/csrc/mbar_device.h
--- a/pymbar_amd/csrc/mbar_device.h
+++ b/pymbar_amd/csrc/mbar_device.h
@@ -540,6 +540,34 @@
 constexpr double GRAM_NEG_HUGE = -2.9e303, LOGDEN_HUGE = 1e300;
 constexpr int FUSED_PSUM1_FROM_GRAM_NB = 8;
 
+constexpr int GRAM_FOLD_ROUND = 12;
+template <int NBLK>
+__device__ __forceinline__ void fold_gram_records(const v4d (&G)[NBLK], char* base0, int stride, int wave, int lane,
+                                                  double* __restrict__ rec) {
+    static_assert(NBLK % GRAM_FOLD_ROUND == 0, "whole rounds only");
+    typedef __attribute__((address_space(3))) double lds_double;
+    const uint32_t mine = (uint32_t)(uintptr_t)(__attribute__((address_space(3))) char*)(base0 + wave * stride) + (uint32_t)lane * 8u;
+    const double* all = reinterpret_cast<const double*>(base0);
+    const int ws = stride / 8;
+#pragma unroll
+    for (int rd = 0; rd < NBLK / GRAM_FOLD_ROUND; ++rd) {
+        if (rd) __syncthreads();
+#pragma unroll
+        for (int i = 0; i < GRAM_FOLD_ROUND; ++i)
+#pragma unroll
+            for (int r = 0; r < 4; ++r) {
+                uint32_t a = mine + (uint32_t)((i * 4 + r) * 512);
+                asm volatile("" : "+v"(a));
+                *reinterpret_cast<lds_double*>((uintptr_t)a) = G[rd * GRAM_FOLD_ROUND + i][r];
+            }
+        __syncthreads();
+        const double* q = all + (GRAM_FOLD_ROUND * wave) * 64 + lane;
+        double* o = rec + (rd * GRAM_FOLD_ROUND * 4 + GRAM_FOLD_ROUND * wave) * 64 + lane;
+#pragma unroll 4
+        for (int k = 0; k < GRAM_FOLD_ROUND; ++k) o[k * 64] = (q[k * 64] + q[k * 64 + ws]) + (q[k * 64 + 2 * ws] + q[k * 64 + 3 * ws]);
+    }
+}
+
 static inline int blocks_per_cu_for(size_t lds_bytes) {
     int b = (int)((160 * 1024) / lds_bytes);
     if (b < 1) b = 1;
diff --git a/pymbar_amd/csrc/mbar_internal.h b/pymbar_amd/csrc/mbar_internal.h
--- a/pymbar_amd/csrc/mbar_internal.h
+++ b/pymbar_amd/csrc/mbar_internal.h
@@ -67,6 +67,7 @@
     int waves;
     int nwaves;
     int psum_records;
+    int gram_records = 0;
     int variant;
     size_t lds_bytes;
     int live_blocks = 0;
@@ -161,8 +162,8 @@
 hipError_t launch_reduce_level1(hipStream_t s, const double* part, int64_t nparts, int64_t count, double* out,
                                 int64_t* nchunks);
 hipError_t launch_mfma_peak(hipStream_t s, int blocks, int iters, double* sink);
-hipError_t launch_reduce2(hipStream_t s, const double* partA, int64_t countA, const double* partB, int64_t countB,
-                          int64_t nparts, double* scratch, double* outA, double* outB);
+hipError_t launch_reduce2(hipStream_t s, const double* partA, int64_t countA, int64_t npartsA, const double* partB, int64_t countB,
+                          int64_t npartsB, double* outA, double* outB);
 
 struct LoopSrc {
     const double* p[8];
@@ -201,14 +202,14 @@
 hipError_t launch_psweep(hipStream_t s, int nb, int nf, const LaunchGeom& g, const double* P, int64_t ld, int64_t N,
                          const double* cmul, const double* cw, double* rinv0, double* rinv1, double* psum_part,
                          const LoopCtl& lc = LoopCtl());
-LaunchGeom fused_geometry(int nb, int num_cu, int64_t ntiles, int64_t grid_override, bool unit = false);
+LaunchGeom fused_geometry(int nb, int num_cu, int64_t ntiles, int64_t grid_override, bool unit = false, bool fold = false);
 hipError_t launch_fused(hipStream_t s, int nb, const LaunchGeom& g, const double* P, int64_t ld, int64_t N, const double* cmul,
                         const double* cw, const double* wsq, bool unit, double* rinv_base, double* gram_part, double* psum_part,
                         const LoopCtl& lc);
 LaunchGeom build_sweep_geometry(int nb, int num_cu, int64_t ntiles, int64_t grid_override);
 hipError_t launch_build_sweep(hipStream_t s, int nb, const LaunchGeom& g, const double* u, int64_t ld, int64_t N,
                               const double* aden, const double* cw, double* P, double* rinv_slot, double* psum_part);
-LaunchGeom build_gram_geometry(int nb, int num_cu, int64_t ntiles, int64_t grid_override);
+LaunchGeom build_gram_geometry(int nb, int num_cu, int64_t ntiles, int64_t grid_override, bool fold = false);
 hipError_t launch_build_gram(hipStream_t s, int nb, const LaunchGeom& g, const double* u, int64_t ld, int64_t N,
                              const double* aden, const double* wsq, bool general, double* P, double* rinv_slot, double* gram_part);
 
diff --git a/pymbar_amd/csrc/mbar_k_fused.hip b/pymbar_amd/csrc/mbar_k_fused.hip
--- a/pymbar_amd/csrc/mbar_k_fused.hip
+++ b/pymbar_amd/csrc/mbar_k_fused.hip
@@ -12,7 +12,7 @@
     const int rows = NB - 2 - r1;
     return NB + (NB * (I - r1) + rows - 1) / rows;
 }
-template <int NB, bool WIDE, bool UNIT>
+template <int NB, bool WIDE, bool UNIT, bool FOLD = false>
 __global__ void __launch_bounds__(256, 1)
 k_fused(const double* __restrict__ P, int64_t ld, int64_t N, int64_t ntiles, const double* __restrict__ cmul,
         const double* __restrict__ cw, const double* __restrict__ wsq, double* __restrict__ rinv0,
@@ -269,7 +269,12 @@
             if (lane < 16) psum_part[(gw * 2 + f) * ROWS + 16 * I + lane] = v;
         }
     }
-    {
+    if constexpr (FOLD) {
+        static_assert(!FOLD || (PINNED && NBLK % GRAM_FOLD_ROUND == 0), "the fold is laid out for the full panel");
+        wait_vm<0>();
+        static_assert(!FOLD || 2 * TILE_BYTES >= GRAM_FOLD_ROUND * 2048, "a wave's tile buffers hold its copy of a round");
+        fold_gram_records<NBLK>(G, smem, 2 * TILE_BYTES, wave, lane, gram_part + (int64_t)blockIdx.x * NBLK * 256);
+    } else {
         int b = 0;
 #pragma unroll
         for (int I = 0; I < NB; ++I)
@@ -289,7 +294,7 @@
 
 
 
-LaunchGeom fused_geometry(int nb, int num_cu, int64_t ntiles, int64_t grid_override, bool unit) {
+LaunchGeom fused_geometry(int nb, int num_cu, int64_t ntiles, int64_t grid_override, bool unit, bool fold) {
     LaunchGeom g;
     g.waves = 4;
     g.variant = 1;
@@ -300,7 +305,7 @@
         int64_t wantq = ntiles < 1 ? 1 : ntiles;
         g.blocks = (int)(wantq < capq ? wantq : capq);
         g.nwaves = g.blocks;
-        g.psum_records = g.nwaves;
+        g.psum_records = g.gram_records = g.nwaves;
         return g;
     }
     const size_t tile = (size_t)nb * 16 * TS * 8 + 1024;
@@ -321,6 +326,7 @@
     g.blocks = (int)(want < cap ? want : cap);
     g.nwaves = g.blocks * 4;
     g.psum_records = g.nwaves;
+    g.gram_records = fold && nb == 8 ? g.blocks : g.nwaves;
     return g;
 }
 template <int NB>
@@ -342,6 +348,14 @@
                                lc.ctl, lc.slot_stride);
         return hipGetLastError();
     };
+    if constexpr (NB == 8) {
+        if (g.gram_records != g.nwaves) {
+            if (g.gram_records != g.blocks) return hipErrorInvalidValue;
+            if (unit) return stage_offsets_wide(ld) ? go(k_fused<NB, true, true, true>) : go(k_fused<NB, false, true, true>);
+            return stage_offsets_wide(ld) ? go(k_fused<NB, true, false, true>) : go(k_fused<NB, false, false, true>);
+        }
+    }
+    if (g.gram_records != g.nwaves) return hipErrorInvalidValue;
     if (unit) return stage_offsets_wide(ld) ? go(k_fused<NB, true, true>) : go(k_fused<NB, false, true>);
     return stage_offsets_wide(ld) ? go(k_fused<NB, true, false>) : go(k_fused<NB, false, false>);
 }
diff --git a/pymbar_amd/csrc/mbar_k_pmode.hip b/pymbar_amd/csrc/mbar_k_pmode.hip
--- a/pymbar_amd/csrc/mbar_k_pmode.hip
+++ b/pymbar_amd/csrc/mbar_k_pmode.hip
@@ -160,7 +160,7 @@
     }
 }
 
-template <int NB, bool WIDE, bool GENERAL>
+template <int NB, bool WIDE, bool GENERAL, bool FOLD = false>
 __global__ void __launch_bounds__(256, 1)
 k_build_gram(const double* __restrict__ u, int64_t ld, int64_t N, int64_t ntiles, const double* __restrict__ aden,
              const double* __restrict__ wsq, double* __restrict__ P, double* __restrict__ rinv_slot, double* __restrict__ gram_part) {
@@ -316,10 +316,16 @@
         cur ^= 1;
     }
     if constexpr (PINNED) asm volatile("s_nop 15\n\ts_nop 15" ::: "memory");
-#pragma unroll
-    for (int b = 0; b < NBLK; ++b)
-#pragma unroll
-        for (int r = 0; r < 4; ++r) gram_part[((gw * NBLK + b) * 4 + r) * 64 + lane] = G[b][r];
+    if constexpr (FOLD) {
+        static_assert(!FOLD || (PINNED && 2 * TILE_BYTES >= GRAM_FOLD_ROUND * 2048), "a wave's tile buffers hold its copy of a round");
+        wait_vm<0>();
+        fold_gram_records<NBLK>(G, smem + EXP_TABLE_BYTES, 2 * TILE_BYTES, wave, lane, gram_part + (int64_t)blockIdx.x * NBLK * 256);
+    } else {
+#pragma unroll
+        for (int b = 0; b < NBLK; ++b)
+#pragma unroll
+            for (int r = 0; r < 4; ++r) gram_part[((gw * NBLK + b) * 4 + r) * 64 + lane] = G[b][r];
+    }
 }
 
 template <int NB, int NF>
@@ -541,8 +547,8 @@
     }
 }
 
-LaunchGeom build_gram_geometry(int nb, int num_cu, int64_t ntiles, int64_t grid_override) {
-    LaunchGeom g = fused_geometry(nb, num_cu, ntiles, grid_override);
+LaunchGeom build_gram_geometry(int nb, int num_cu, int64_t ntiles, int64_t grid_override, bool fold) {
+    LaunchGeom g = fused_geometry(nb, num_cu, ntiles, grid_override, false, fold);
     g.lds_bytes = (size_t)4 * 2 * ((size_t)nb * 16 * TS * 8 + TS * 8) + EXP_TABLE_BYTES;
     return g;
 }
@@ -559,6 +565,14 @@
         hipLaunchKernelGGL(kern, dim3(g.blocks), dim3(256), g.lds_bytes, s, u, ld, N, ntiles, aden, wsq, P, rinv_slot, gp);
         return hipGetLastError();
     };
+    if constexpr (NB == 8) {
+        if (g.gram_records != g.nwaves) {
+            if (g.gram_records != g.blocks) return hipErrorInvalidValue;
+            if (general) return stage_offsets_wide(ld) ? go(k_build_gram<NB, true, true, true>) : go(k_build_gram<NB, false, true, true>);
+            return stage_offsets_wide(ld) ? go(k_build_gram<NB, true, false, true>) : go(k_build_gram<NB, false, false, true>);
+        }
+    }
+    if (g.gram_records != g.nwaves) return hipErrorInvalidValue;
     if (general) return stage_offsets_wide(ld) ? go(k_build_gram<NB, true, true>) : go(k_build_gram<NB, false, true>);
     return stage_offsets_wide(ld) ? go(k_build_gram<NB, true, false>) : go(k_build_gram<NB, false, false>);
 }
diff --git a/pymbar_amd/csrc/mbar_k_solver.hip b/pymbar_amd/csrc/mbar_k_solver.hip
--- a/pymbar_amd/csrc/mbar_k_solver.hip
+++ b/pymbar_amd/csrc/mbar_k_solver.hip
@@ -2,6 +2,7 @@
 
 namespace mbar {
 
+constexpr int64_t REDUCE_CHUNK = 32;
 __global__ void __launch_bounds__(256)
 k_reduce(const double* __restrict__ part, int64_t nparts, int64_t count, int64_t chunk,
          double* __restrict__ out) {
@@ -304,22 +305,40 @@
 }
 
 
-__global__ void __launch_bounds__(256)
-k_reduce2(const double* __restrict__ partA, int64_t countA, const double* __restrict__ partB, int64_t countB,
-          int64_t nparts, int64_t chunk, double* __restrict__ outA, double* __restrict__ outB) {
-    const int64_t gxA = (countA + 255) / 256;
+__global__ void __launch_bounds__(1024)
+k_reduce2(const double* __restrict__ partA, int64_t countA, int64_t npartsA, const double* __restrict__ partB, int64_t countB,
+          int64_t npartsB, int log2e, double* __restrict__ outA, double* __restrict__ outB) {
+    extern __shared__ double red2[];
+    const int E = 1 << log2e;
+    const int64_t gxA = (countA + E - 1) >> log2e;
     const bool isB = (int64_t)blockIdx.x >= gxA;
     const double* part = isB ? partB : partA;
     const int64_t count = isB ? countB : countA;
+    const int64_t nparts = isB ? npartsB : npartsA;
     double* out = isB ? outB : outA;
-    const int64_t i = ((int64_t)blockIdx.x - (isB ? gxA : 0)) * blockDim.x + threadIdx.x;
-    if (i >= count) return;
-    const int64_t p0 = (int64_t)blockIdx.y * chunk;
-    const int64_t p1 = p0 + chunk < nparts ? p0 + chunk : nparts;
-    double s = 0.0;
+    const int e = threadIdx.x & (E - 1), j = threadIdx.x >> log2e, G = blockDim.x >> log2e;
+    const int64_t i = (((int64_t)blockIdx.x - (isB ? gxA : 0)) << log2e) + e;
+    const int64_t n1 = (nparts + REDUCE_CHUNK - 1) / REDUCE_CHUNK;
+    if (i < count) {
+        for (int64_t c = j; c < n1; c += G) {
+            const int64_t p0 = c * REDUCE_CHUNK;
+            const int64_t p1 = p0 + REDUCE_CHUNK < nparts ? p0 + REDUCE_CHUNK : nparts;
+            double s = 0.0;
 #pragma unroll 8
-    for (int64_t p = p0; p < p1; ++p) s += part[p * count + i];
-    out[(int64_t)blockIdx.y * count + i] = s;
+            for (int64_t p = p0; p < p1; ++p) s += part[p * count + i];
+            red2[c * E + e] = s;
+        }
+    }
+    __syncthreads();
+    if (j == 0 && i < count) {
+        double s = 0.0;
+        if (n1 == 1) {
+            s = red2[e];
+        } else {
+            for (int64_t c = 0; c < n1; ++c) s += red2[c * E + e];
+        }
+        out[i] = s;
+    }
 }
 
 
@@ -1243,7 +1262,7 @@
         hipLaunchKernelGGL(k_reduce, dim3(gx, 1), dim3(256), 0, s, part, nparts, count, nparts, out);
         return hipGetLastError();
     }
-    const int64_t chunk = 32;
+    const int64_t chunk = REDUCE_CHUNK;
     const int64_t n1 = (nparts + chunk - 1) / chunk;
     hipLaunchKernelGGL(k_reduce, dim3(gx, (unsigned)n1), dim3(256), 0, s, part, nparts, count, chunk, scratch);
     hipLaunchKernelGGL(k_reduce, dim3(gx, 1), dim3(256), 0, s, (const double*)scratch, n1, count, n1, out);
@@ -1454,19 +1473,20 @@
     return hipGetLastError();
 }
 
-hipError_t launch_reduce2(hipStream_t s, const double* partA, int64_t countA, const double* partB, int64_t countB,
-                          int64_t nparts, double* scratch, double* outA, double* outB) {
-    const unsigned gx = (unsigned)((countA + 255) / 256 + (countB + 255) / 256);
-    if (nparts <= 32) {
-        hipLaunchKernelGGL(k_reduce2, dim3(gx, 1), dim3(256), 0, s, partA, countA, partB, countB, nparts, nparts, outA, outB);
-        return hipGetLastError();
-    }
-    const int64_t chunk = 32;
-    const int64_t n1 = (nparts + chunk - 1) / chunk;
-    double* sA = scratch;
-    double* sB = scratch + n1 * countA;
-    hipLaunchKernelGGL(k_reduce2, dim3(gx, (unsigned)n1), dim3(256), 0, s, partA, countA, partB, countB, nparts, chunk, sA, sB);
-    hipLaunchKernelGGL(k_reduce2, dim3(gx, 1), dim3(256), 0, s, (const double*)sA, countA, (const double*)sB, countB, n1, n1,
+hipError_t launch_reduce2(hipStream_t s, const double* partA, int64_t countA, int64_t npartsA, const double* partB, int64_t countB,
+                          int64_t npartsB, double* outA, double* outB) {
+    const int64_t n1A = (npartsA + REDUCE_CHUNK - 1) / REDUCE_CHUNK, n1B = (npartsB + REDUCE_CHUNK - 1) / REDUCE_CHUNK;
+    const int64_t n1 = n1A > n1B ? n1A : n1B;
+    const int G = n1 < 1 ? 1 : (n1 > 32 ? 32 : (int)n1);
+    int log2e = 5;
+    while (G << (log2e + 1) <= 256) ++log2e;
+    while (log2e > 0 && ((size_t)(n1 < 1 ? 1 : n1) << log2e) * sizeof(double) > 48 * 1024) --log2e;
+    const size_t lds = ((size_t)(n1 < 1 ? 1 : n1) << log2e) * sizeof(double);
+    if (lds > 48 * 1024) return hipErrorInvalidValue;
+    const int64_t E = (int64_t)1 << log2e;
+    const unsigned gx = (unsigned)((countA + E - 1) / E + (countB + E - 1) / E);
+    if (gx == 0) return hipSuccess;
+    hipLaunchKernelGGL(k_reduce2, dim3(gx), dim3((unsigned)(G << log2e)), lds, s, partA, countA, npartsA, partB, countB, npartsB, log2e,
                        outA, outB);
     return hipGetLastError();
 }
diff --git a/pymbar_amd/csrc/mbar_loops.cpp b/pymbar_amd/csrc/mbar_loops.cpp
--- a/pymbar_amd/csrc/mbar_loops.cpp
+++ b/pymbar_amd/csrc/mbar_loops.cpp
@@ -373,7 +373,9 @@
     LaunchGeom& gp = p.gp;
     gg = wide ? gram_quad_geometry(nb, c->num_cu, ntiles, c->opt_grid) : gram_geometry(nb * 16, true, c->num_cu, ntiles, c->opt_grid);
     p.unit = !c->weighted && !c->opt_fused_general;
-    gl = fused ? fused_geometry(nb, c->num_cu, ntiles, c->opt_grid, p.unit)
+    bool fold = c->opt_gram_fold != 0;
+    if (const char* e = std::getenv("MBAR_GRAM_FOLD")) fold = std::atoi(e) != 0;
+    gl = fused ? fused_geometry(nb, c->num_cu, ntiles, c->opt_grid, p.unit, fold)
          : pmode ? psweep_geometry(nb, c->num_cu, ntiles, c->opt_grid)
                  : lse_geometry(nb, 2, c->num_cu, ntiles, c->opt_grid, lse_variant_for(c));
     if (wide) gg.live_blocks = gl.live_blocks = quad_live_blocks(c);
@@ -394,7 +396,7 @@
         light = light && l_ok;
     }
     p.light = light;
-    const LaunchGeom& gb = p.gb = fused ? build_gram_geometry(nb, c->num_cu, ntiles, c->opt_grid)
+    const LaunchGeom& gb = p.gb = fused ? build_gram_geometry(nb, c->num_cu, ntiles, c->opt_grid, fold)
                                         : build_sweep_geometry(nb, c->num_cu, ntiles, c->opt_grid);
     const size_t rec_g = p.rec_g = (size_t)nb * (nb + 1) / 2 * 256;
     const size_t rec_l = p.rec_l = (size_t)2 * Kp;
@@ -405,9 +407,12 @@
                      std::max(std::max((size_t)gg.nwaves * rec_g, (size_t)gl.nwaves * (rec_l + 2)), (size_t)gb.nwaves * Kp));
     if (!arc)
         arc = ensure(c, &c->scratch, &c->scratch_doubles,
-                     std::max(((size_t)std::max(gg.nwaves, gl.nwaves) / 32 + 1) * (rec_g + rec_l + 2), ((size_t)gb.nwaves / 32 + 1) * (Kp + rec_g)));
+                     std::max(((size_t)std::max(gg.nwaves, gl.nwaves) / 32 + 1) * (rec_g + rec_l + 2),
+                              ((size_t)std::max(gb.nwaves, gb.gram_records) / 32 + 1) * (Kp + rec_g)));
     if (!arc && c->weighted && !c->lden_eff) arc = fail(c, MBAR_ERR_STATE, "weighted context without its logden buffer");
-    if (!arc && fused) arc = ensure(c, &c->part_g, &c->part_g_doubles, (size_t)gl.nwaves * rec_g);
+    if (!arc && fused)
+        arc = ensure(c, &c->part_g, &c->part_g_doubles,
+                     (size_t)std::max(std::max(gl.gram_records, gb.gram_records), gg.nwaves) * rec_g);
     {
         bool ok = arc == MBAR_OK;
         const std::string local_err = c->error;
@@ -424,7 +429,8 @@
     p.batch = c->opt_adapt_batch;
     p.use_graph = c->opt_graph && !stream_transport(c);
     p.graph_sig = ((int64_t)gg.blocks << 40) ^ ((int64_t)gl.blocks << 20) ^ ((int64_t)p.m << 12) ^ (pmode ? 128 : 0) ^ (fused ? 256 : 0) ^
-                  (c->weighted ? 64 : 0) ^ (p.lc_slot.unclamped ? 512 : 0) ^ (p.merged ? 1024 : 0) ^ (light ? 2048 : 0) ^ (int64_t)nb;
+                  (c->weighted ? 64 : 0) ^ (p.lc_slot.unclamped ? 512 : 0) ^ (p.merged ? 1024 : 0) ^ (light ? 2048 : 0) ^ (int64_t)nb ^
+                  ((int64_t)(fused ? gl.gram_records : 0) << 24) ^ (c->opt_reduce_single ? 0 : 4096);
     p.an0.assign((size_t)Kp, 0.0);
     p.cm0.assign((size_t)Kp, 0.0);
     build_aden(c, f.data(), p.an0.data(), Kp);
@@ -447,6 +453,15 @@
 
 int start_classic(mbar_ctx* c, const DeviceLoopPlan&, const std::vector<double>& f, std::vector<double>& psum, mbar_solve_result&) {
     return eval_core(c, f.data(), 1, 0, c->logden[0], nullptr, psum.data(), nullptr, nullptr);
+}
+
+static hipError_t reduce_fused_records(mbar_ctx* c, const DeviceLoopPlan& p, const double* psum_part, const double* gram_part) {
+    if (c->opt_reduce_single)
+        return launch_reduce2(c->stream, psum_part, (int64_t)p.rec_l, p.gl.psum_records, gram_part, (int64_t)p.rec_g, p.gl.gram_records,
+                              c->red, c->red + p.off_gram);
+    hipError_t e = launch_reduce(c->stream, psum_part, p.gl.psum_records, (int64_t)p.rec_l, c->scratch, c->red);
+    if (e != hipSuccess) return e;
+    return launch_reduce(c->stream, gram_part, p.gl.gram_records, (int64_t)p.rec_g, c->scratch, c->red + p.off_gram);
 }
 
 int start_warm(mbar_ctx* c, const DeviceLoopPlan& p, const std::vector<double>&, std::vector<double>& psum, mbar_solve_result& res) {
@@ -462,8 +477,7 @@
         HIPCHK(c, launch_fused(c->stream, p.nb, p.gl, c->P, c->ld, c->N, d_aden(c), c->cw, c->weighted ? c->cwsq : c->cw, p.unit,
                                c->logden[0], c->part_g, c->part, p.lc_slot));
     }
-    HIPCHK(c, launch_reduce2(c->stream, c->part, (int64_t)p.rec_l, c->part_g, (int64_t)p.rec_g, p.gl.nwaves, c->scratch, c->red,
-                             c->red + p.off_gram));
+    HIPCHK(c, reduce_fused_records(c, p, c->part, c->part_g));
     int rc = allreduce_dev(c, c->red, (int64_t)(p.off_gram + p.rec_g), 0);
     if (rc) return rc;
     HIPCHK(c, hipMemcpyAsync(c->hred, c->red, (size_t)Kp * sizeof(double), hipMemcpyDeviceToHost, c->stream));
@@ -533,7 +547,7 @@
             HIPCHK(c, launch_build_sweep(c->stream, p.nb, p.gb, c->u, c->ld, c->N, d_aden(c), c->cw, c->P, c->logden[0], c->part));
     }
     if (p.fused) {
-        int rc = reduce_to_host(c, c->part_g, p.gb.nwaves, (int64_t)p.rec_g, p.off_gram);
+        int rc = reduce_to_host(c, c->part_g, p.gb.gram_records, (int64_t)p.rec_g, p.off_gram);
         if (rc) return rc;
         gram_row_sums(c->hred + p.off_gram, p.nb, K, psum.data());
     } else {
@@ -737,13 +751,12 @@
         {
             ScopedTimer sec(c, MBAR_TIMER_REDUCE, split);
             if (p.fused) {
-                HIPCHK(c, launch_reduce2(c->stream, psum_part, (int64_t)p.rec_l, gram_part, (int64_t)p.rec_g, p.gl.nwaves, c->scratch, c->red,
-                                         c->red + p.off_gram));
+                HIPCHK(c, reduce_fused_records(c, p, psum_part, gram_part));
                 ar_count = (int64_t)(p.off_gram + p.rec_g);
             } else if (p.pmode) {
                 HIPCHK(c, launch_reduce(c->stream, psum_part, p.gl.nwaves, (int64_t)p.rec_l, c->scratch, c->red));
             } else {
-                HIPCHK(c, launch_reduce2(c->stream, psum_part, (int64_t)p.rec_l, obj_part, 2, p.gl.nwaves, c->scratch, c->red, c->red + p.rec_l));
+                HIPCHK(c, launch_reduce2(c->stream, psum_part, (int64_t)p.rec_l, p.gl.nwaves, obj_part, 2, p.gl.nwaves, c->red, c->red + p.rec_l));
             }
         }
         if (stream_transport(c)) {
@@ -974,6 +987,38 @@
     return MBAR_OK;
 }
 
+int mbar_ctx_debug_gram_sweep(mbar_ctx* c, const double* f_in, int build, double* psum_out, double* blocks_out, double* cmul_out) {
+    if (!c || !f_in || !psum_out || !blocks_out || !cmul_out) return fail(c, MBAR_ERR_ARG, "NULL argument");
+    if (c->ext_base) return fail(c, MBAR_ERR_STATE, "mbar_ctx_debug_gram_sweep: an extension context holds rows only");
+    if (!c->have_Nk) return fail(c, MBAR_ERR_STATE, "mbar_ctx_set_Nk has not been called");
+    HIPCHK(c, hipSetDevice(c->device));
+    std::vector<double> f(f_in, f_in + c->K), psum((size_t)c->K, 0.0);
+    int rc = refresh_poison(c);
+    if (rc) return rc;
+    if (!device_loop_eligible(c) || c->u_poison || !f_is_finite(c, f.data(), 1) || c->Kp > 128)
+        return fail(c, MBAR_ERR_STATE, "mbar_ctx_debug_gram_sweep: the context does not run the device-resident loop up to 128 states");
+    c->ld0_valid = false;
+    c->last_psum.clear();
+    mbar_solve_result res;
+    std::memset(&res, 0, sizeof(res));
+    DeviceLoopPlan p;
+    const int64_t pcache = c->opt_pcache;
+    if (build) c->opt_pcache = 0;
+    rc = plan_device_loop(c, f, 0, nullptr, 0, p);
+    c->opt_pcache = pcache;
+    if (rc) return rc;
+    if (!p.fused || p.wide) return fail(c, MBAR_ERR_STATE, "mbar_ctx_debug_gram_sweep: the fused loop is switched off");
+    if (!build && !p.warm) return fail(c, MBAR_ERR_STATE, "mbar_ctx_debug_gram_sweep: no resident probability matrix within reach of f");
+    rc = build ? start_build_narrow(c, p, f, psum, res) : start_warm(c, p, f, psum, res);
+    if (rc) return rc;
+    HIPCHK(c, hipMemcpyAsync(blocks_out, c->red + p.off_gram, p.rec_g * sizeof(double), hipMemcpyDeviceToHost, c->stream));
+    rc = sync_stream(c);
+    if (rc) return rc;
+    std::copy(psum.begin(), psum.end(), psum_out);
+    for (int64_t k = 0; k < c->Kp; ++k) cmul_out[k] = build ? 1.0 : p.cm0[(size_t)k];
+    return MBAR_OK;
+}
+
 int mbar_ctx_last_solve_psum(mbar_ctx* c, double* psum_out) {
     if (!c || !psum_out) return fail(c, MBAR_ERR_ARG, "NULL argument");
     if ((int64_t)c->last_psum.size() != c->K) return fail(c, MBAR_ERR_STATE, "no adaptive solve has left its per-state sums on this context");
diff --git a/pymbar_amd/device.py b/pymbar_amd/device.py
--- a/pymbar_amd/device.py
+++ b/pymbar_amd/device.py
@@ -337,6 +337,15 @@
         out["psum"] = psum if self._lib.mbar_ctx_last_solve_psum(self._ctx, _dptr(psum)) == _lib.MBAR_OK else None
         return f, out
 
+    def debug_gram_sweep(self, f, build=False):
+        f = np.ascontiguousarray(f, dtype=np.float64)
+        nb = (self.K + 15) // 16
+        psum = np.empty(self.K, dtype=np.float64)
+        blocks = np.empty((nb * (nb + 1) // 2, 16, 16), dtype=np.float64)
+        cmul = np.empty(16 * nb, dtype=np.float64)
+        self._check(self._lib.mbar_ctx_debug_gram_sweep(self._ctx, _dptr(f), 1 if build else 0, _dptr(psum), _dptr(blocks), _dptr(cmul)))
+        return psum, blocks, cmul
+
     def solve_sci(self, f, tol=1e-12, maxiter=10000, check_convergence=True):
         f = np.array(f, dtype=np.float64)
         res = _lib.SolveResult()
```

Result: no change. 294.6 (-0.0%).
